# jacobstern/volume-viz

Measured on AMD Instinct MI355X. Metric: Msamples/s (rays x steps), 1024^3 f32 volume @1080p, higher is better.
Workload: dtype f32

## Files before the change

### include/volviz.h

```cpp
#ifndef VOLVIZ_H
#define VOLVIZ_H

#include <stddef.h>
#include <stdint.h>
#include <stdbool.h>

#ifdef __cplusplus
extern "C" {
#endif

#ifndef SLICE_NONE
#define SLICE_NONE      -1
#define SLICE_PLANE      0
#define SLICE_PLANE_CUT  1
#endif
#ifndef TRANSFER_PRESET_DEFAULT
#define TRANSFER_PRESET_DEFAULT -1
#define TRANSFER_PRESET_ENGINE   0
#define TRANSFER_PRESET_MRI      1
#endif

struct slice_params {
    int   type;
    float params[6];
// ... 120 lines not shown
int  vv_render_projection(vv_context *ctx, int width, int height,
                          const struct slice_params *slice,
                          const struct camera_params *camera,
                          const vv_ray_source *rays,
                          const vv_render_options *opts,
                          int mode,
                          uint8_t *rgba_out, uint8_t *index_out, uint32_t *stat_out, int out_on_device, void *stream);

int  vv_slice(vv_context *ctx, float *buffer, size_t height, size_t width,
              float dx, float dy, float dz, int orientation,
              const float scale[3], int legacy, int filter,
              int out_on_device, void *stream);
int  vv_slice_advanced(vv_context *ctx, float *buffer, size_t height, size_t width,
                       const float trans[16] ,
                       const float scale[3], int filter,
                       int out_on_device, void *stream);

typedef enum { VV_SLAB_MAX = 0, VV_SLAB_MIN = 1, VV_SLAB_MEAN = 2 } vv_slab_mode;
#define VV_SLAB_MAX_SAMPLES 1024
typedef struct vv_slab { int mode; int samples; float thickness; } vv_slab;
int  vv_slice_slab(vv_context *ctx, float *buffer, int32_t *aux , size_t height, size_t width,
                   float dx, float dy, float dz, int orientation, const float scale[3], int filter,
                   const vv_slab *slab, int out_on_device, void *stream);
int  vv_slice_advanced_slab(vv_context *ctx, float *buffer, int32_t *aux , size_t height, size_t width,
                            const float trans[16], const float scale[3], int filter,
                            const vv_slab *slab, int out_on_device, void *stream);

typedef struct vv_histogram {
    unsigned long long counts[256];
    unsigned long long voxels;
    unsigned long long nan_voxels;
    float vmin, vmax;
} vv_histogram;
int  vv_volume_histogram(vv_context *ctx, const int box_lo[3], const int box_hi[3],
                         vv_histogram *out, int out_on_device, void *stream);
int  vv_histogram_indices(vv_context *ctx, const uint8_t *index, size_t n,
                          unsigned long long counts[256], int on_device, void *stream);

int  vv_first_pass(vv_context *ctx, int img_w, int img_h, const struct camera_params *camera,
                   const vv_ray_source *rays, uint8_t *front_rgba, uint8_t *back_rgba,
                   int out_on_device, void *stream);

int  vv_cut_plane_canonical(int orientation, float displace, float point[3], float normal[3]);
int  vv_cut_plane_from_euler(float dx, float dy, float dz, float theta, float phi, float psi, float point[3], float normal[3]);
int  vv_cut_plane_to_slice_params(int slice_type, const float point[3], const float normal[3],
                                  int flip_cross_section, struct slice_params *out);

int  vv_camera_orbit_drag(const float position[3], int dx, int dy, float out_position[3], float out_look[3]);
int  vv_camera_zoom(const float position[3], const float look[3], int delta, float out_position[3]);
int  vv_cut_plane_from_drag(const float position[3], const float look[3], const float up[3], float aspect,
                            const float press[2], const float release[2],
                            float point[3], float normal[3], float plane_up[3], float plane_right[3]);
int  vv_cut_plane_drag(float point[3], const float plane_up[3], const float plane_right[3],
                       int dx, int dy, int width, int height);

int  vv_slice_to_bgra(const float *slice, size_t height, size_t width, uint8_t *bgra);

int  vv_slice_matrix(float dx, float dy, float dz, float theta, float phi, float psi,
                     float out[16]);

int  vv_generate_ellipsoids(vv_context *ctx, uint8_t *out, int out_on_device,
                            int nx, int ny, int nz, int n,
                            const float *centers , const float *axes ,
                            const uint8_t *colors , void *stream);
int  vv_draw_ellipsoid(vv_context *ctx, uint8_t *vol, int vol_on_device,
                       int nx, int ny, int nz, const float center[3], const float axes[3],
                       uint8_t color, void *stream);
int  vv_generate_default_brain(vv_context *ctx, uint8_t *out, int out_on_device,
                               int nx, int ny, int nz, void *stream);
int  vv_promote_u8_to_f32(vv_context *ctx, const uint8_t *dev_in, float *dev_out,
                          size_t n, void *stream);
int  vv_generate_noise_u8(vv_context *ctx, uint8_t *dev_out, int nx, int ny, int nz,
                          uint32_t seed, void *stream);

typedef enum { VV_TF_ENGINE = 0, VV_TF_HEAD = 1, VV_TF_MRI = 2 } vv_tf_preset;
int  vv_transfer_preset(int preset, float tf_out[1024]);

int  vv_dataset_preset(const char *path, int *tf_preset, float scale[3]);

int  vv_t3d_read_header(const char *path, int header, int *nx, int *ny, int *nz);
int  vv_t3d_read (const char *path, int header, uint8_t *dst, size_t capacity);
int  vv_t3d_write(const char *path, int header, const uint8_t *src, int nx, int ny, int nz);

enum { VV_LAYOUT_BRICKED = 1, VV_LAYOUT_ZPAIR = 2, VV_LAYOUT_ZFAST = 4, VV_LAYOUT_POLICY = 256 };
int  vv_prepare_layouts(vv_context *ctx, int which, void *stream);
int  vv_set_layout_policy(vv_context *ctx, unsigned long long budget_bytes , int build_in_render );
int  vv_layout_state(const vv_context *ctx, unsigned long long out[8]);
int  vv_device_bytes(const vv_context *ctx, unsigned long long out[4]);

float              vv_last_frame_ms(const vv_context *ctx);
int                vv_set_frame_timing(vv_context *ctx, int on);
unsigned long long vv_last_sample_count(vv_context *ctx);
int                vv_debug_last_launch(vv_context *ctx, int out[8]);
int                vv_debug_screen_rect(int width, int height, const struct camera_params *cam, const vv_ray_source *rays, double out[4]);
int                vv_debug_counters(vv_context *ctx, unsigned long long out[16]);
int                vv_reread_env(vv_context *ctx);
int                vv_volume_dims(const vv_context *ctx, int dims[3], int *voxel_type);

#ifdef __cplusplus
}
#endif
#endif
```

### volume-viz_amd/csrc/vv_api.cpp

```cpp
#include "../../include/volviz.h"
#include "vv_kernels.h"
#include "vv_gate.h"

#include <cassert>
#include <hip/hip_runtime.h>
#include <climits>
#include <cmath>
#include <cstdio>
#include <cstdlib>
#include <cstring>
#include <string>
#include <algorithm>
#include <vector>

using namespace vv;

struct vv_knobs {
    int tile_log2w = -1, xcd_band = -1, unroll = -1, lds_reserve = -1, lds_reserve_phong = -1;
    int bricked = -1, zpair = -1, zfast = -1, force_big = 0;
    int block_w = -1, tail = -1, rect = -1, lpt = -1, lpt_run = -1, phong_bricks = -1;
    int hist_blocks = -1;
    static int geti(const char *name, int dflt) { const char *e = getenv(name); return e ? atoi(e) : dflt; }
    void read()
    {
        tile_log2w = geti("VV_TILE_LOG2W", -1); xcd_band = geti("VV_XCD_BAND", -1); unroll = geti("VV_UNROLL", -1);
        lds_reserve = geti("VV_LDS_RESERVE", -1); lds_reserve_phong = geti("VV_LDS_RESERVE_PHONG", -1);
        bricked = geti("VV_BRICKED", -1); zpair = geti("VV_ZPAIR", -1);
        block_w = geti("VV_BLOCK_W", -1); tail = geti("VV_TAIL", -1);
        zfast = geti("VV_ZFAST", -1); force_big = getenv("VV_FORCE_BIG") != nullptr;
        rect = geti("VV_RECT", -1); lpt = geti("VV_LPT", -1); lpt_run = geti("VV_LPT_RUN", -1); phong_bricks = geti("VV_PHONG_BRICKS", -1);
        hist_blocks = geti("VV_HIST_BLOCKS", -1);
    }
};

enum { CP_BRICKS = 0, CP_ZPAIR = 1, CP_ZFAST = 2, CP_XPAIR = 3, CP_N = 4 };
struct layout_copy {
    void *ptr = nullptr; size_t bytes = 0;
    bool valid = false, failed = false;
    unsigned long long last_used = 0;
    uint32_t row = 0; uint64_t slab = 0;
};

struct vv_context {
    int device = 0;
    vv_knobs knobs;
    hipStream_t stream = nullptr;
    hipEvent_t ev0 = nullptr, ev1 = nullptr;
    hipEvent_t ev_count = nullptr;
    bool timed = false, time_frames = true;
    void *d_vol = nullptr; size_t vol_bytes = 0; int vtype = VV_VOXEL_U8; int nx = 0, ny = 0, nz = 0;
    size_t row_pitch = 0, slice_pitch = 0, alloc_bytes = 0;
    layout_copy copies[CP_N];
    size_t layout_budget_bytes = 0; bool build_in_render = true;
    unsigned long long frame_no = 0;
    unsigned long long builds_in_render = 0;
    float last_density = 1e9f;
    float4 *d_tf = nullptr; bool tf_gray = false; bool have_tf = false;
    bool tf_alpha_unit = false;
    float *d_rad = nullptr; size_t rad_cap = 0;
    uint32_t *d_order = nullptr; size_t order_cap = 0;
    uint8_t *d_frame = nullptr; size_t frame_cap = 0;
    uint8_t *d_index = nullptr; size_t index_cap = 0;
    uint8_t *d_hit = nullptr; size_t hit_cap = 0;
    uint8_t *d_stat = nullptr; size_t stat_cap = 0;
    float4 *d_tf_arg = nullptr;
    uint8_t *d_img = nullptr; size_t img_cap = 0;
    float *d_slice = nullptr; size_t slice_cap = 0;
    float *d_gen = nullptr; size_t gen_cap = 0;
    struct view_key_t { float cam[8]; const void *front, *back; int img_w, img_h, W, H; } view_key;
    bool view_key_valid = false, view_est_ok = false; float view_side[3] = {0, 0, 0}, view_px_cube = 0.f;
    std::vector<uint8_t> row_buf;
    int last_launch[8] = {0, 0, 0, 0, 0, 0, 0, 0};
    unsigned long long *d_counter = nullptr;
    unsigned long long *d_hist = nullptr;
    int n_cu = 0;
    bool counter_valid = false;
    hipStream_t copy_stream = nullptr, promo_stream = nullptr;
    void *pin[2] = {nullptr, nullptr}; hipEvent_t pin_ev[2] = {nullptr, nullptr}; int pin_next = 0;
    hipEvent_t src_ev[2] = {nullptr, nullptr}; int src_last = -1;
    uint8_t *d_stage[2] = {nullptr, nullptr};
    bool streaming = false;
    std::string err;
};

static std::string g_err;

static const size_t kHistResultOffset = kHistAccWords * sizeof(unsigned long long);
static const size_t kHistScratchBytes = kHistResultOffset + sizeof(vv_histogram);
static_assert(sizeof(vv_histogram) == 2072 && sizeof(unsigned long long) == 8, "vv_histogram layout (include/volviz.h)");

static int fail(vv_context *c, int code, const std::string &msg)
{
    if (c) c->err = msg; else g_err = msg;
    return code;
}
#define HIPCHK(c, expr) do { hipError_t e_ = (expr); if (e_ != hipSuccess) \
    return fail((c), VV_ERR_DEVICE, std::string(#expr) + ": " + hipGetErrorString(e_)); } while (0)

static inline hipStream_t pick_stream(const vv_context *c, void *stream)
{
    if (!stream) return c->stream;
    if (stream == VV_STREAM_DEFAULT_ASYNC) return (hipStream_t)0;
    return (hipStream_t)stream;
}

static void drop_copies(vv_context *c)
{
    for (layout_copy &cp : c->copies) {
        if (cp.ptr) (void)hipFree(cp.ptr);
        cp = layout_copy();
    }
    c->builds_in_render = 0;
    c->view_key_valid = false;
}

static int ensure(vv_context *c, void **p, size_t *cap, size_t need)
{
    if (*cap >= need && *p) return VV_OK;
    if (*p) { HIPCHK(c, hipFree(*p)); *p = nullptr; *cap = 0; }
    HIPCHK(c, hipMalloc(p, need));
    *cap = need;
    return VV_OK;
}

static int finalize_layout(vv_context *c, hipStream_t st);
static int camera_basis(vv_context *c, FrameParams &P, const camera_params *cam, const vv_ray_source *rays, int W, int H);
typedef vv_context::view_key_t vv_view_key;

static bool image_source_has_hint(const vv_ray_source *r)
{
    if (r->mode != VV_RAYS_IMAGES) return false;
    const float l2 = r->look[0] * r->look[0] + r->look[1] * r->look[1] + r->look[2] * r->look[2];
    const float cx = r->look[1] * r->up[2] - r->look[2] * r->up[1], cy = r->look[2] * r->up[0] - r->look[0] * r->up[2], cz = r->look[0] * r->up[1] - r->look[1] * r->up[0];
    return std::isfinite(l2) && l2 > 0.f && std::isfinite(cx + cy + cz) && (cx * cx + cy * cy + cz * cz) > 0.f;
}
static int clamp_row(long long t, int n) { return (int)(t < 0 ? 0 : (t > n - 1 ? n - 1 : t)); }
static vv_view_key view_key_of(const camera_params *cam, const vv_ray_source *r, int W, int H)
{
    vv_view_key k;
    memset(&k, 0, sizeof k);
    memcpy(k.cam, cam, sizeof(float) * 8);
    k.front = r->front; k.back = r->back; k.img_w = r->img_w; k.img_h = r->img_h; k.W = W; k.H = H;
    return k;
}
static bool estimate_view_from_images(const uint8_t *front, const uint8_t *back, int img_w, int img_h, int W, int H, float side[3], float *px_cube)
{
    if (!front || !back || img_w < 1 || img_h < 1 || W < 8 || H < 1) return false;
    const int y = H / 2;
    const int ty = clamp_row((long long)floorf((float)y / (float)H * (float)img_h), img_h);
    const uint8_t *fr = front + (size_t)ty * img_w * 4, *br = back + (size_t)ty * img_w * 4;
    auto texel = [&](int x) { return clamp_row((long long)floorf((float)x / (float)W * (float)img_w), img_w); };
    auto hit = [&](int x) { const int t = texel(x) * 4; return fr[t] != br[t] || fr[t + 1] != br[t + 1] || fr[t + 2] != br[t + 2]; };
    int xl = -1, xr = -1;
    for (int x = 0; x <= W - 2; ++x) if (hit(x)) { xl = x; break; }
    if (xl < 0) return false;
    for (int x = W - 2; x >= xl; --x) if (hit(x)) { xr = x; break; }
    if (xr - xl < 8) return false;
    const int a = (xl + xr) / 2 - (xr - xl) / 8, b = (xl + xr) / 2 + (xr - xl) / 8;
    float d[3], len2 = 0.f;
    for (int k = 0; k < 3; ++k) {
        const int ta = texel(a) * 4 + k, tb = texel(b) * 4 + k;
        d[k] = (((float)fr[tb] + (float)br[tb]) - ((float)fr[ta] + (float)br[ta])) / (2.f * 255.f);
        len2 += d[k] * d[k];
    }
    if (!(len2 > 0.f)) return false;
    const float len = sqrtf(len2);
    side[0] = d[0] / len; side[1] = d[1] / len; side[2] = d[2] / len;
    *px_cube = len / (float)(b - a);
    return true;
}

static size_t layout_budget(const vv_context *c)
{
    if (c->layout_budget_bytes) return c->layout_budget_bytes;
    return std::max<size_t>((size_t)8 << 30, c->alloc_bytes / 2 * 5);
}
static size_t copy_bytes(const vv_context *c, int k) { return c->copies[k].valid ? c->copies[k].bytes : 0; }
static void copy_drop(vv_context *c, int k)
{
    layout_copy &cp = c->copies[k];
    if (cp.ptr) (void)hipFree(cp.ptr);
    cp.ptr = nullptr; cp.valid = false; cp.bytes = 0;
}
static bool make_room(vv_context *c, size_t need, unsigned keep)
{
    const size_t budget = layout_budget(c);
    if (need > budget) return false;
    for (;;) {
        size_t used = 0;
        for (int k = 0; k < CP_N; ++k) used += copy_bytes(c, k);
        if (used + need <= budget) return true;
        int victim = -1;
        for (int k = 0; k < CP_N; ++k)
            if (c->copies[k].valid && !(keep & (1u << k)) && (victim < 0 || c->copies[k].last_used < c->copies[victim].last_used)) victim = k;
        if (victim < 0) return false;
        copy_drop(c, victim);
    }
}

static bool copy_refused(vv_context *c, int k)
{
    if (k != CP_ZPAIR) c->copies[k].failed = true;
    return false;
}

template <class Build>
static bool build_copy(vv_context *c, int k, size_t bytes, size_t pad, size_t zero_from, unsigned keep, hipStream_t st, Build build)
{
    layout_copy &cp = c->copies[k];
    size_t free_b = 0, total_b = 0;
    if (make_room(c, bytes, keep | (1u << k)) && hipMemGetInfo(&free_b, &total_b) == hipSuccess && free_b >= bytes + (512ull << 20) &&
        hipMalloc(&cp.ptr, bytes + pad) == hipSuccess) {
        if (hipMemsetAsync((char *)cp.ptr + zero_from, 0, bytes + pad - zero_from, st) == hipSuccess) {
            build(cp.ptr);
            if (hipGetLastError() == hipSuccess && hipStreamSynchronize(st) == hipSuccess) { cp.bytes = bytes; cp.valid = true; return true; }
        }
        (void)hipFree(cp.ptr);
    }
    (void)hipGetLastError();
    cp.ptr = nullptr;
    return copy_refused(c, k);
}

static bool ensure_bricks(vv_context *c, hipStream_t st)
{
    layout_copy &cp = c->copies[CP_BRICKS];
    if (cp.valid || cp.failed) return cp.valid;
    uint32_t sy = 0, sz64 = 0;
    const size_t bytes = brick_copy_bytes(c->vtype, c->nx, c->ny, c->nz, &sy, &sz64);
    if (sz64 >= (1u << 24) || sy >= (1u << 24)) return copy_refused(c, CP_BRICKS);
    cp.row = sy; cp.slab = sz64;
    return build_copy(c, CP_BRICKS, bytes, 16, bytes, 0, st, [&](void *p) {
        launch_build_bricks(c->vtype, c->d_vol, c->row_pitch, c->slice_pitch, p, c->nx, c->ny, c->nz, st); });
}

static bool ensure_zpair(vv_context *c, hipStream_t st)
{
    layout_copy &cp = c->copies[CP_ZPAIR];
    if (cp.valid) return true;
    uint32_t rb = 0, sb = 0;
    const size_t bytes = zpair_copy_bytes(c->vtype, c->nx, c->ny, c->nz, &rb, &sb);
    if ((size_t)(c->ny + 1) * ((size_t)c->nx + 1) * 8 >= (1ull << 32) || ((size_t)c->nx + 1) * 8 >= (1u << 24) ||
        (c->vtype == VV_VOXEL_U8 && bytes >= (1ull << 32)))
        return copy_refused(c, CP_ZPAIR);
    cp.row = rb; cp.slab = sb;
    return build_copy(c, CP_ZPAIR, bytes, 32, bytes, 0, st, [&](void *p) {
        launch_build_zpair(c->vtype, c->d_vol, c->row_pitch, c->slice_pitch, p, c->nx, c->ny, c->nz, st); });
}

static bool ensure_zfast(vv_context *c, hipStream_t st)
{
    layout_copy &cp = c->copies[CP_ZFAST];
    if (cp.valid || cp.failed) return cp.valid;
    const size_t vsz = c->vtype == VV_VOXEL_F32 ? 4 : 1;
    size_t row = (size_t)c->nz * vsz;
    if (row % 1024 == 0) row += 32;
    else if (vsz == 1) row = (row + 3) & ~(size_t)3;
    size_t rows = (size_t)c->ny;
    if (row % 1024 == 32 && (rows * row) % 4096 == 0) rows += 1;
    const size_t slice = rows * row, bytes = slice * ((size_t)c->nx + 1) + row + 16;
    if (c->ny > 65535 || (c->nz + 31) / 32 > 65535 || row >= (1u << 24) || slice >= (1ull << 32))
        return copy_refused(c, CP_ZFAST);
    cp.row = (uint32_t)row; cp.slab = slice;
    return build_copy(c, CP_ZFAST, bytes, 0, 0, 0, st, [&](void *p) {
        launch_build_zfast(c->vtype, c->d_vol, (uint32_t)c->row_pitch, (uint64_t)c->slice_pitch, p, (uint32_t)row, (uint64_t)slice, c->nx, c->ny, c->nz, st); });
}

static bool ensure_xpair(vv_context *c, hipStream_t st)
{
    layout_copy &cp = c->copies[CP_XPAIR];
    if (cp.valid || cp.failed) return cp.valid;
    if (!ensure_zfast(c, st)) return false;
    uint32_t rb = 0, sb = 0;
    const size_t bytes = zpair_copy_bytes(c->vtype, c->nz, c->ny, c->nx, &rb, &sb);
    if ((size_t)(c->ny + 1) * ((size_t)c->nz + 1) * 8 >= (1ull << 32) || ((size_t)c->nz + 1) * 8 >= (1u << 24) ||
        (c->vtype == VV_VOXEL_U8 && bytes >= (1ull << 32)))
        return copy_refused(c, CP_XPAIR);
    cp.row = rb; cp.slab = sb;
    const layout_copy &zf = c->copies[CP_ZFAST];
    return build_copy(c, CP_XPAIR, bytes, 32, bytes, 1u << CP_ZFAST, st, [&](void *p) {
        launch_build_xpair(c->vtype, zf.ptr, zf.row, zf.slab, p, c->nx, c->ny, c->nz, st); });
}

static bool (*const ensure_copy[CP_N])(vv_context *, hipStream_t) = {ensure_bricks, ensure_zpair, ensure_zfast, ensure_xpair};

static bool take_copy(vv_context *c, int k, hipStream_t st)
{
    if (!(c->build_in_render ? ensure_copy[k](c, st) : c->copies[k].valid)) return false;
    c->copies[k].last_used = c->frame_no;
    return true;
}

extern "C" {

const char *vv_last_error(const vv_context *ctx) { return ctx ? ctx->err.c_str() : g_err.c_str(); }

int vv_init(int device, vv_context **out)
{
    if (!out) return fail(nullptr, VV_ERR_INVALID, "vv_init: out_ctx is NULL");
    *out = nullptr;
    int count = 0;
    hipError_t e = hipGetDeviceCount(&count);
    if (e != hipSuccess || count == 0)
        return fail(nullptr, VV_ERR_DEVICE, "vv_init: no HIP device available (this library has no CPU path)");
    if (device < 0) { if (hipGetDevice(&device) != hipSuccess) device = 0; }
    if (device >= count) return fail(nullptr, VV_ERR_INVALID, "vv_init: device index out of range");
    vv_context *c = new vv_context();
    c->device = device;
    c->knobs.read();
    if (hipSetDevice(device) != hipSuccess || hipStreamCreate(&c->stream) != hipSuccess ||
        hipEventCreate(&c->ev0) != hipSuccess || hipEventCreate(&c->ev1) != hipSuccess || hipEventCreateWithFlags(&c->ev_count, hipEventDisableTiming) != hipSuccess ||
        hipMalloc((void **)&c->d_counter, 16 * sizeof(unsigned long long)) != hipSuccess ||
        hipMalloc((void **)&c->d_hist, kHistScratchBytes) != hipSuccess ||
        hipDeviceGetAttribute(&c->n_cu, hipDeviceAttributeMultiprocessorCount, device) != hipSuccess ||
        hipMalloc((void **)&c->d_tf, 256 * sizeof(float4)) != hipSuccess) {
        delete c;
        return fail(nullptr, VV_ERR_DEVICE, "vv_init: device set-up failed");
    }
    *out = c;
    return VV_OK;
}

int vv_shutdown(vv_context *c)
{
    if (!c) return VV_OK;
    hipSetDevice(c->device);
    hipStreamSynchronize(c->stream);
    if (c->d_vol) hipFree(c->d_vol);
    drop_copies(c);
    if (c->d_tf) hipFree(c->d_tf);
    if (c->d_rad) hipFree(c->d_rad);
    if (c->d_order) hipFree(c->d_order);
    if (c->d_frame) hipFree(c->d_frame);
    if (c->d_index) hipFree(c->d_index);
    if (c->d_hit) hipFree(c->d_hit);
    if (c->d_stat) hipFree(c->d_stat);
    if (c->d_tf_arg) hipFree(c->d_tf_arg);
    if (c->d_img) hipFree(c->d_img);
    if (c->d_slice) hipFree(c->d_slice);
    if (c->d_gen) hipFree(c->d_gen);
    if (c->d_counter) hipFree(c->d_counter);
    if (c->d_hist) hipFree(c->d_hist);
    for (int i = 0; i < 2; ++i) {
        if (c->pin[i]) hipHostFree(c->pin[i]);
        if (c->pin_ev[i]) hipEventDestroy(c->pin_ev[i]);
        if (c->src_ev[i]) hipEventDestroy(c->src_ev[i]);
        if (c->d_stage[i]) hipFree(c->d_stage[i]);
    }
    if (c->copy_stream) hipStreamDestroy(c->copy_stream);
    if (c->promo_stream) hipStreamDestroy(c->promo_stream);
    if (c->ev0) hipEventDestroy(c->ev0);
    if (c->ev1) hipEventDestroy(c->ev1);
    if (c->ev_count) hipEventDestroy(c->ev_count);
    if (c->stream) hipStreamDestroy(c->stream);
    delete c;
    return VV_OK;
}

int vv_set_transfer_function(vv_context *c, const float tf[1024])
{
    if (!c || !tf) return fail(c, VV_ERR_INVALID, "vv_set_transfer_function: NULL argument");
    HIPCHK(c, hipSetDevice(c->device));
    for (int i = 0; i < 1024; ++i)
        if (!std::isfinite(tf[i])) return fail(c, VV_ERR_INVALID, "vv_set_transfer_function: table entries must be finite");
    bool gray = true, unit = true;
    for (int i = 0; i < 256; ++i)
        if (!(tf[4*i] == tf[4*i+1] && tf[4*i] == tf[4*i+2])) { gray = false; break; }
    for (int i = 0; i < 256; ++i)
        if (!(tf[4*i+3] >= 0.f && tf[4*i+3] <= 1.f)) { unit = false; break; }
    HIPCHK(c, hipMemcpy(c->d_tf, tf, 1024 * sizeof(float), hipMemcpyHostToDevice));
    c->tf_gray = gray; c->tf_alpha_unit = unit; c->have_tf = true;
    return VV_OK;
}

static int install_volume(vv_context *c, const void *src, bool src_on_device, int vtype,
                          int nx, int ny, int nz, const float tf[1024], hipStream_t s)
{
    if (!c || !src) return fail(c, VV_ERR_INVALID, "load_volume: NULL argument");
    if (nx < 1 || ny < 1 || nz < 1) return fail(c, VV_ERR_INVALID, "load_volume: dims must be >= 1");
    if (vtype != VV_VOXEL_U8 && vtype != VV_VOXEL_F32) return fail(c, VV_ERR_INVALID, "load_volume: bad voxel type");
    const size_t vsz = vtype == VV_VOXEL_F32 ? 4 : 1;
    const size_t bytes = (size_t)nx * ny * nz * vsz;
    if ((size_t)nx * ny * vsz > 0xFFFFFFF0ull)
        return fail(c, VV_ERR_INVALID, "load_volume: one slice must stay below 4 GiB");
    if ((size_t)nx * vsz >= (1u << 24) || nx >= (1 << 24) || ny >= (1 << 24) || nz >= (1 << 24))
        return fail(c, VV_ERR_INVALID, "load_volume: a volume row must be below 16 MiB and each dimension below 2^24");
    HIPCHK(c, hipSetDevice(c->device));
    c->knobs.read();
    const size_t pad = (size_t)nx * ny * vsz + 2 * (size_t)nx * vsz + 4096;
    drop_copies(c);
    if (c->d_vol) { HIPCHK(c, hipFree(c->d_vol)); c->d_vol = nullptr; }
    HIPCHK(c, hipMalloc(&c->d_vol, bytes + pad));
    hipStream_t st = pick_stream(c, s);
    HIPCHK(c, hipMemsetAsync((char *)c->d_vol + bytes, 0, pad, st));
    if (src_on_device) HIPCHK(c, hipMemcpyAsync(c->d_vol, src, bytes, hipMemcpyDeviceToDevice, st));
    else { HIPCHK(c, hipMemcpyAsync(c->d_vol, src, bytes, hipMemcpyHostToDevice, st)); }
    c->vol_bytes = bytes; c->vtype = vtype; c->nx = nx; c->ny = ny; c->nz = nz;
    c->row_pitch = (size_t)nx * vsz; c->slice_pitch = c->row_pitch * ny; c->alloc_bytes = bytes + pad;
    { int rc = finalize_layout(c, st); if (rc) return rc; }
    if (!src_on_device || !s) HIPCHK(c, hipStreamSynchronize(st));
    if (tf) return vv_set_transfer_function(c, tf);
    return VV_OK;
}

int vv_load_volume_u8(vv_context *c, const uint8_t *texels, size_t size, int nx, int ny, int nz, const float tf[1024])
{
    if (size != (size_t)nx * ny * nz) return fail(c, VV_ERR_INVALID, "vv_load_volume_u8: size != nx*ny*nz");
    return install_volume(c, texels, false, VV_VOXEL_U8, nx, ny, nz, tf, nullptr);
}
int vv_load_volume_f32(vv_context *c, const float *texels, size_t size, int nx, int ny, int nz, const float tf[1024])
{
    if (size != (size_t)nx * ny * nz * 4) return fail(c, VV_ERR_INVALID, "vv_load_volume_f32: size != nx*ny*nz*4 bytes");
    return install_volume(c, texels, false, VV_VOXEL_F32, nx, ny, nz, tf, nullptr);
}
int vv_load_volume_device(vv_context *c, const void *dev, int vtype, int nx, int ny, int nz, const float tf[1024], void *stream)
{
    return install_volume(c, dev, true, vtype, nx, ny, nz, tf, (hipStream_t)stream);
}

int vv_prepare_layouts(vv_context *c, int which, void *stream)
{
    if (!c) return fail(nullptr, VV_ERR_INVALID, "vv_prepare_layouts: NULL context");
    if (!c->d_vol) return fail(c, VV_ERR_NO_VOLUME, "vv_prepare_layouts: no volume loaded");
    if (which & ~(VV_LAYOUT_BRICKED | VV_LAYOUT_ZPAIR | VV_LAYOUT_ZFAST | VV_LAYOUT_POLICY)) return fail(c, VV_ERR_INVALID, "vv_prepare_layouts: unknown layout bit");
    HIPCHK(c, hipSetDevice(c->device));
    hipStream_t st = pick_stream(c, stream);
    const bool pair_ok = c->vtype == VV_VOXEL_U8 || c->vol_bytes <= (512ull << 20);
    if (which & VV_LAYOUT_POLICY) {
        if ((size_t)c->nx * c->ny * c->nz >= (1ull << 21)) which |= VV_LAYOUT_BRICKED | VV_LAYOUT_ZFAST;
        if (pair_ok) which |= VV_LAYOUT_ZPAIR;
    }
    int built = 0;
    if (which & VV_LAYOUT_BRICKED) c->copies[CP_BRICKS].failed = false;
    if (which & VV_LAYOUT_ZFAST) c->copies[CP_ZFAST].failed = c->copies[CP_XPAIR].failed = false;
    auto prepare = [&](int k) {
        if (!ensure_copy[k](c, st)) return false;
        c->copies[k].last_used = ++c->frame_no;
        return true;
    };
    if ((which & VV_LAYOUT_BRICKED) && prepare(CP_BRICKS)) built |= VV_LAYOUT_BRICKED;
    if ((which & VV_LAYOUT_ZFAST) && prepare(CP_ZFAST)) {
        built |= VV_LAYOUT_ZFAST;
        if (pair_ok) prepare(CP_XPAIR);
    }
    if ((which & VV_LAYOUT_ZPAIR) && prepare(CP_ZPAIR)) built |= VV_LAYOUT_ZPAIR;
    return built;
}

int vv_reread_env(vv_context *c)
{
    if (!c) return VV_ERR_INVALID;
    c->knobs.read();
    return VV_OK;
}

int vv_set_layout_policy(vv_context *c, unsigned long long budget_bytes, int build_in_render)
{
    if (!c) return fail(nullptr, VV_ERR_INVALID, "vv_set_layout_policy: NULL context");
    c->layout_budget_bytes = (size_t)budget_bytes;
    c->build_in_render = build_in_render != 0;
    return VV_OK;
}

int vv_layout_state(const vv_context *c, unsigned long long out[8])
{
    if (!c || !out) return VV_ERR_INVALID;
    out[0] = c->d_vol ? c->alloc_bytes : 0;
    for (int k = 0; k < CP_N; ++k) out[1 + k] = copy_bytes(c, k);
    out[5] = c->d_vol ? layout_budget(c) : c->layout_budget_bytes;
    out[6] = c->builds_in_render;
    out[7] = c->build_in_render ? 1 : 0;
    return VV_OK;
}

int vv_device_bytes(const vv_context *c, unsigned long long out[4])
{
    if (!c || !out) return VV_ERR_INVALID;
    out[0] = c->d_vol ? c->alloc_bytes : 0;
    out[1] = copy_bytes(c, CP_BRICKS);
    out[2] = copy_bytes(c, CP_ZPAIR) + copy_bytes(c, CP_ZFAST) + copy_bytes(c, CP_XPAIR);
    out[3] = c->rad_cap + c->frame_cap + c->index_cap + c->hit_cap + c->stat_cap + (c->d_tf_arg ? 4096 : 0) + c->img_cap + c->slice_cap + 4096 + 8 * sizeof(unsigned long long) + kHistScratchBytes;
    return VV_OK;
}

int vv_debug_counters(vv_context *c, unsigned long long out[16])
{
    if (!c || !out || !c->counter_valid) return VV_ERR_INVALID;
    if (hipEventSynchronize(c->ev_count) != hipSuccess) return VV_ERR_DEVICE;
    if (hipMemcpy(out, c->d_counter, 16 * sizeof(unsigned long long), hipMemcpyDeviceToHost) != hipSuccess) return VV_ERR_DEVICE;
    return VV_OK;
}

static const size_t kStageBytes = 64u << 20;

int vv_load_volume_stream_begin(vv_context *c, int vtype, int nx, int ny, int nz, const float tf[1024])
{
    if (!c) return fail(nullptr, VV_ERR_INVALID, "stream_begin: NULL context");
    if (nx < 1 || ny < 1 || nz < 1 || (vtype != VV_VOXEL_U8 && vtype != VV_VOXEL_F32))
        return fail(c, VV_ERR_INVALID, "stream_begin: bad dims / voxel type");
    const size_t vsz = vtype == VV_VOXEL_F32 ? 4 : 1;
    if ((size_t)nx * ny * vsz > 0xFFFFFFF0ull) return fail(c, VV_ERR_INVALID, "stream_begin: one slice must stay below 4 GiB");
    if ((size_t)nx * vsz >= (1u << 24) || ny >= (1 << 24) || nz >= (1 << 24))
        return fail(c, VV_ERR_INVALID, "stream_begin: a volume row must be below 16 MiB and each dimension below 2^24");
    HIPCHK(c, hipSetDevice(c->device));
    c->knobs.read();
    const size_t bytes = (size_t)nx * ny * nz * vsz, pad = (size_t)nx * ny * vsz + 2 * (size_t)nx * vsz + 4096;
    drop_copies(c);
    if (c->d_vol) { HIPCHK(c, hipFree(c->d_vol)); c->d_vol = nullptr; }
    HIPCHK(c, hipMalloc(&c->d_vol, bytes + pad));
    if (!c->copy_stream) HIPCHK(c, hipStreamCreate(&c->copy_stream));
    if (!c->promo_stream) HIPCHK(c, hipStreamCreate(&c->promo_stream));
    HIPCHK(c, hipMemsetAsync((char *)c->d_vol + bytes, 0, pad, c->copy_stream));
    c->src_last = -1;
    c->vol_bytes = bytes; c->vtype = vtype; c->nx = nx; c->ny = ny; c->nz = nz;
    c->row_pitch = (size_t)nx * vsz; c->slice_pitch = c->row_pitch * ny; c->alloc_bytes = bytes + pad;
    c->streaming = true;
    if (tf) return vv_set_transfer_function(c, tf);
    return VV_OK;
}

int vv_load_volume_stream_slices_async(vv_context *c, const void *src, int src_type, int z0, int nslices)
{
    if (!c || !c->streaming) return fail(c, VV_ERR_INVALID, "stream_slices: no stream_begin");
    if (!src || z0 < 0 || nslices < 1 || z0 + nslices > c->nz) return fail(c, VV_ERR_INVALID, "stream_slices: bad slice range");
    if (src_type != c->vtype && !(src_type == VV_VOXEL_U8 && c->vtype == VV_VOXEL_F32))
        return fail(c, VV_ERR_INVALID, "stream_slices: source type must match the volume (or be u8 for an f32 volume)");
    HIPCHK(c, hipSetDevice(c->device));
    const size_t ssz = src_type == VV_VOXEL_F32 ? 4 : 1, dsz = c->vtype == VV_VOXEL_F32 ? 4 : 1;
    const size_t slice_vox = (size_t)c->nx * c->ny;
    const bool promote = src_type != c->vtype;
    hipPointerAttribute_t attr;
    bool pinned = hipPointerGetAttributes(&attr, src) == hipSuccess && attr.type == hipMemoryTypeHost;
    (void)hipGetLastError();
    size_t total_vox = slice_vox * (size_t)nslices, done = 0;
    const size_t piece_vox_max = ((kStageBytes / ssz) / 16) * 16;
    while (done < total_vox) {
        const size_t nv = std::min(piece_vox_max, total_vox - done);
        const int b = c->pin_next; c->pin_next ^= 1;
        if (!c->pin_ev[b]) HIPCHK(c, hipEventCreate(&c->pin_ev[b]));
        if (!c->src_ev[b]) HIPCHK(c, hipEventCreate(&c->src_ev[b]));
        HIPCHK(c, hipEventSynchronize(c->pin_ev[b]));
        const char *hsrc = (const char *)src + done * ssz;
        if (!pinned) {
            if (!c->pin[b]) HIPCHK(c, hipHostMalloc(&c->pin[b], kStageBytes, hipHostMallocDefault));
            memcpy(c->pin[b], hsrc, nv * ssz);
            hsrc = (const char *)c->pin[b];
        }
        char *dst = (char *)c->d_vol + ((size_t)z0 * slice_vox + done) * dsz;
        if (!promote) {
            HIPCHK(c, hipMemcpyAsync(dst, hsrc, nv * ssz, hipMemcpyHostToDevice, c->copy_stream));
            HIPCHK(c, hipEventRecord(c->src_ev[b], c->copy_stream));
            HIPCHK(c, hipEventRecord(c->pin_ev[b], c->copy_stream));
        } else {
            if (!c->d_stage[b]) HIPCHK(c, hipMalloc((void **)&c->d_stage[b], kStageBytes));
// ... 73 lines not shown
        return rc ? rc : r3;
    }
    return VV_OK;
}

int vv_volume_dims(const vv_context *c, int dims[3], int *vtype)
{
    if (!c || !c->d_vol) return VV_ERR_NO_VOLUME;
    if (dims) { dims[0] = c->nx; dims[1] = c->ny; dims[2] = c->nz; }
    if (vtype) *vtype = c->vtype;
    return VV_OK;
}

static int finalize_layout(vv_context *c, hipStream_t st)
{
    size_t pad_bytes = 32;
    if (const char *e = getenv("VV_PITCH_PAD")) { int t = atoi(e); if (t <= 0) return VV_OK; if (t >= 16 && t <= 4096 && t % 16 == 0) pad_bytes = (size_t)t; }
    const size_t dense_row = c->row_pitch;
    if (dense_row % 1024 != 0 && !getenv("VV_PITCH_FORCE")) return VV_OK;
    if (dense_row % 16 != 0) return VV_OK;
    const size_t row = dense_row + pad_bytes;
    size_t rows = (size_t)c->ny;
    if ((rows * row) % 4096 == 0) rows += 1;
    if (const char *e = getenv("VV_PITCH_ROWS")) { int t = atoi(e); if (t >= 0 && t <= 64) rows = (size_t)c->ny + (size_t)t; }
    const size_t slice = rows * row;
    if (slice > 0xFFFFFFF0ull || row >= (1u << 24)) return VV_OK;
    const size_t bytes = slice * (size_t)c->nz, pad = slice + 2 * row + 4096;
    size_t free_b = 0, total_b = 0;
    void *nv = nullptr;
    if (hipMemGetInfo(&free_b, &total_b) != hipSuccess || free_b < bytes + pad + (512ull << 20) ||
        hipMalloc(&nv, bytes + pad) != hipSuccess) { (void)hipGetLastError(); return VV_OK; }
    HIPCHK(c, hipMemsetAsync(nv, 0, bytes + pad, st));
    launch_repitch(c->d_vol, nv, dense_row, (size_t)c->ny, (size_t)c->nz, row, slice, st);
    HIPCHK(c, hipGetLastError());
    HIPCHK(c, hipStreamSynchronize(st));
    HIPCHK(c, hipFree(c->d_vol));
    c->d_vol = nv; c->row_pitch = row; c->slice_pitch = slice; c->alloc_bytes = bytes + pad;
    return VV_OK;
}

static VolumeView view_of(const vv_context *c, MarchBuild b)
{
    VolumeView V = {};
    V.data = c->d_vol; V.nx = c->nx; V.ny = c->ny; V.nz = c->nz;
    V.row_bytes = (uint32_t)c->row_pitch;
    V.slice_bytes = (uint32_t)c->slice_pitch;
    V.big = c->slice_pitch * (size_t)c->nz > (1ull << 32) || V.slice_bytes >= (1u << 24) || c->knobs.force_big;
    const layout_copy *cp = c->copies;
    if (b == MB_BRICKED || b == MB_BRICKED_CACHED) { V.bricks = cp[CP_BRICKS].ptr; V.b_sy = cp[CP_BRICKS].row; V.b_sz64 = (uint32_t)cp[CP_BRICKS].slab; }
    if (b == MB_ZFAST || b == MB_XPAIR) { V.zfast = cp[CP_ZFAST].ptr; V.zf_row_bytes = cp[CP_ZFAST].row; V.zf_slice_bytes = cp[CP_ZFAST].slab; }
    const layout_copy &pc = cp[b == MB_XPAIR ? CP_XPAIR : CP_ZPAIR];
    if (b == MB_ZPAIR || b == MB_XPAIR) { V.zpair = pc.ptr; V.zp_row_bytes = pc.row; V.zp_slab_bytes = (uint32_t)pc.slab; }
    return V;
}

static inline float vlen_h(float x, float y, float z) { return sqrtf(x * x + y * y + z * z); }

static int camera_basis(vv_context *c, FrameParams &P, const camera_params *cam, const vv_ray_source *rays, int W, int H)
{
    float lx = rays->look[0], ly = rays->look[1], lz = rays->look[2];
    float ll = vlen_h(lx, ly, lz);
    if (!(ll > 0.f)) return fail(c, VV_ERR_INVALID, "vv_render: look vector is zero");
    lx /= ll; ly /= ll; lz /= ll;
    float ux = rays->up[0], uy = rays->up[1], uz = rays->up[2];
    float sx = ly * uz - lz * uy, sy = lz * ux - lx * uz, sz = lx * uy - ly * ux;
    float sl = vlen_h(sx, sy, sz);
    if (!(sl > 0.f)) return fail(c, VV_ERR_INVALID, "vv_render: up vector is parallel to look");
    sx /= sl; sy /= sl; sz /= sl;
    float vx = sy * lz - sz * ly, vy = sz * lx - sx * lz, vz = sx * ly - sy * lx;
    float vl = vlen_h(vx, vy, vz);
    vx /= vl; vy /= vl; vz /= vl;
    P.look[0] = lx; P.look[1] = ly; P.look[2] = lz;
    P.side[0] = sx; P.side[1] = sy; P.side[2] = sz;
    P.up[0] = vx; P.up[1] = vy; P.up[2] = vz;
    float aspect = rays->aspect > 0.f ? rays->aspect : (float)W / (float)H;
    float th = (float)tan((double)cam->fovY * M_PI / 360.0);
    P.tan_half_x = th * aspect; P.tan_half_y = th;
    return VV_OK;
}


}

static bool choose_launch(vv_context *c, MarchArgs &A, const camera_params *cam, const vv_ray_source *rays, const shading_params *shading,
                          bool have_basis, float density, int H, hipStream_t st)
{
    FrameParams &P = A.P;
    A.V_type = c->vtype;
    A.strips.tile_log2w = 3;
    if (have_basis) {
        const float ax = fabsf(P.side[0]) , ay = fabsf(P.side[1]), az = fabsf(P.side[2]);
        if (ax >= 0.97f * sqrtf(ax * ax + ay * ay + az * az)) A.strips.tile_log2w = 5;
    }
    const vv_knobs &K = c->knobs;
    if ((rays->mode == VV_RAYS_ANALYTIC || image_source_has_hint(rays)) && have_basis && H > 0) {
        const float dist = vlen_h(cam->origin[0], cam->origin[1], cam->origin[2]);
        const float vpw = cbrtf(((float)c->nx / (2.f * P.scale[0])) * ((float)c->ny / (2.f * P.scale[1])) * ((float)c->nz / (2.f * P.scale[2])));
        const float px_vox = 2.f * P.tan_half_y * dist / (float)H * vpw;
        const float step_vox = fmaxf(P.step[0] * c->nx, fmaxf(P.step[1] * c->ny, P.step[2] * c->nz));
        if (std::isfinite(px_vox) && std::isfinite(step_vox) && px_vox > 0.f && step_vox > 0.f) density = step_vox * px_vox * px_vox;
    }
    bool use_zfast = false;
    if (have_basis && A.strips.tile_log2w == 3) {
        const float ax = fabsf(P.side[0]) , ay = fabsf(P.side[1]), az = fabsf(P.side[2]);
        use_zfast = az >= 0.97f * sqrtf(ax * ax + ay * ay + az * az) && (size_t)c->nx * c->ny * c->nz >= (1ull << 21);
        if (K.zfast >= 0) use_zfast = K.zfast != 0;
    }
    const bool phong_bricks_fit = K.phong_bricks > 0 || (density > 3.5f && density <= 8.f && c->vol_bytes > (2ull << 30) && c->vol_bytes <= (8ull << 30));
    const bool phong_bricks = phong_bricks_fit && shading->phongShading && c->vol_bytes > (1ull << 30) && c->vtype == VV_VOXEL_F32 && K.bricked != 0 && K.phong_bricks != 0 &&
                              (c->copies[CP_BRICKS].valid || (c->build_in_render && !c->copies[CP_BRICKS].failed));
    if (phong_bricks && K.zfast < 0) use_zfast = false;
    ++c->frame_no;
    auto copies_valid = [c] { int n = 0; for (const layout_copy &cp : c->copies) n += cp.valid; return n; };
    const int valid_before = copies_valid();
    if (use_zfast) use_zfast = take_copy(c, CP_ZFAST, st);
    if (use_zfast) A.strips.tile_log2w = 5;
    if (K.tile_log2w >= 3 && K.tile_log2w <= 5 && !use_zfast) A.strips.tile_log2w = K.tile_log2w;
    A.strips.xcd_band = 1;
    if (K.xcd_band >= 0 && K.xcd_band <= 64) A.strips.xcd_band = K.xcd_band;
    const bool beyond_caches = c->vol_bytes > (1ull << 30);
    const int big_reserve = density > 3.5f ? 76000 : (density > 1.8f ? 49000 : 36000);
    A.unroll = (A.strips.tile_log2w == 5 || beyond_caches) ? 3 : 2;
    A.lds_reserve = !beyond_caches ? 36000 : (A.strips.tile_log2w == 5 ? big_reserve : 155000);
    A.strips.blk_log2w = 5;
    A.strips.tail_batch = K.tail == 0 ? 0 : 1;
    const int rows_px_8 = A.strips.n_strips * 8;
    int block_w = A.strips.tile_log2w == 3 ? 16 : ((A.strips.tile_log2w == 5 && c->vol_bytes >= (1ull << 30) && density > 3.5f) ? 64 : 32);
    if (K.block_w >= 8 && K.block_w <= 128 && (K.block_w & (K.block_w - 1)) == 0) block_w = K.block_w;
    {
        int lw = 3; while ((1 << lw) < block_w) ++lw;
        const int h = 256 >> lw;
        if (lw != 5 && lw >= A.strips.tile_log2w && h >= (64 >> A.strips.tile_log2w)) {
            A.strips.blk_log2w = lw;
            if (A.strips.strips_per_band < (1 << 26)) {
                const int band_px = A.strips.strips_per_band * 8, spb = (band_px + h - 1) / h;
                A.strips.n_strips = (rows_px_8 / band_px) * spb; A.strips.strips_per_band = spb;
            } else A.strips.n_strips = (rows_px_8 + h - 1) / h;
        }
    }
    const bool k_unroll = K.unroll >= 1 && K.unroll <= 3, k_reserve = K.lds_reserve >= 0 && K.lds_reserve <= 155 * 1024;
    if (k_unroll) A.unroll = K.unroll;
    if (k_reserve) A.lds_reserve = K.lds_reserve;
    bool use_bricks = (A.strips.tile_log2w == 3 || phong_bricks) && (size_t)c->nx * c->ny * c->nz >= (1ull << 21);
    if (K.bricked >= 0) use_bricks = K.bricked != 0;
    if (use_zfast) use_bricks = false;
    if (use_bricks) use_bricks = take_copy(c, CP_BRICKS, st);
    if (use_bricks) {
        if (!k_unroll) A.unroll = 2;
        if (!k_reserve) A.lds_reserve = beyond_caches ? big_reserve : 36000;
    }
    bool use_zpair = !use_bricks && A.strips.tile_log2w == 5 && !shading->phongShading &&
                     (c->vtype == VV_VOXEL_U8 || c->vol_bytes <= (512ull << 20));
    if (K.zpair >= 0) use_zpair = K.zpair != 0 && !use_bricks;
    if (use_zfast) use_zpair = false;
    if (use_zpair) use_zpair = take_copy(c, CP_ZPAIR, st);
    const bool use_xpair = use_zfast && !shading->phongShading && K.zpair != 0 && (c->vtype == VV_VOXEL_U8 || c->vol_bytes <= (512ull << 20)) &&
                           take_copy(c, CP_XPAIR, st);
    const int valid_after = copies_valid();
    if (valid_after > valid_before) c->builds_in_render += valid_after - valid_before;
    A.build = use_xpair ? MB_XPAIR : use_zfast ? MB_ZFAST : use_bricks ? (beyond_caches ? MB_BRICKED : MB_BRICKED_CACHED) : use_zpair ? MB_ZPAIR :
              (view_of(c, MB_LINEAR).big || (shading->phongShading && beyond_caches)) ? MB_LINEAR_BIG : MB_LINEAR;
    A.V = view_of(c, A.build);
    A.lds_reserve_phong = c->vol_bytes > (8ull << 30) ? 40000 : ((beyond_caches && density > 3.5f && !use_bricks) ? 30000 : 13000);
    if (K.lds_reserve_phong >= 0 && K.lds_reserve_phong <= 146 * 1024) A.lds_reserve_phong = K.lds_reserve_phong;
    c->last_density = density;
    return beyond_caches;
}

static bool screen_rect(const MarchArgs &A, int W, int H, double *xmin, double *xmax, double *ymin, double *ymax)
{
    const FrameParams &P = A.P;
    double lo[2] = {INFINITY, INFINITY}, hi[2] = {-INFINITY, -INFINITY}, dmin = INFINITY, ext = 0.0;
    for (int a = 0; a < 3; ++a) ext = std::max(ext, (double)fabsf(P.cam_pos[a]) + (double)P.scale[a]);
    for (int k = 0; k < 8; ++k) {
        const double v[3] = {((k & 1) ? P.scale[0] : -P.scale[0]) - (double)P.cam_pos[0], ((k & 2) ? P.scale[1] : -P.scale[1]) - (double)P.cam_pos[1],
                             ((k & 4) ? P.scale[2] : -P.scale[2]) - (double)P.cam_pos[2]};
        const double depth = v[0] * P.look[0] + v[1] * P.look[1] + v[2] * P.look[2];
        if (!(depth > 1e-3 * ext)) return false;
        dmin = std::min(dmin, depth);
        const double sx = (v[0] * P.side[0] + v[1] * P.side[1] + v[2] * P.side[2]) / depth, sy = (v[0] * P.up[0] + v[1] * P.up[1] + v[2] * P.up[2]) / depth;
        const double px = (sx / P.tan_half_x + 1.0) * 0.5 * W - 0.5, py = (sy / P.tan_half_y + 1.0) * 0.5 * H - 0.5;
        lo[0] = std::min(lo[0], px); hi[0] = std::max(hi[0], px); lo[1] = std::min(lo[1], py); hi[1] = std::max(hi[1], py);
    }
    const double ang = 1e-4 * ext / dmin;
    const double mx = 1.0 + ang / (2.0 * P.tan_half_x / W), my = 1.0 + ang / (2.0 * P.tan_half_y / H);
    if (!std::isfinite(lo[0] + hi[0] + lo[1] + hi[1] + mx + my) || mx > W || my > H) return false;
    *xmin = lo[0] - mx; *xmax = hi[0] + mx; *ymin = lo[1] - my; *ymax = hi[1] + my;
    return true;
}

static void launch_build(FrameKind kind, const MarchArgs &A, hipStream_t st) { assert(A.build < MB_COUNT); kLaunch[frame_row(kind)][A.build](A, st); }

struct FrameImage {
    void *host;
    size_t px_bytes;
    uint8_t **scratch; size_t *cap;
    unsigned align;
    const char *misaligned;
    uint8_t *dev;
};

struct Frame {
    MarchArgs A;
    FrameKind kind; int W, H; hipStream_t st;
    bool have_basis; float density;
    bool beyond_caches;
    bool rect_limits; PixelRect fill_rect;
    bool whole;
    FrameImage img[4];
};

static int check_frame_args(vv_context *c, int W, int H, const slice_params *slice, const camera_params *cam, const vv_ray_source *rays)
{
    if (W < 1 || H < 1) return fail(c, VV_ERR_INVALID, "vv_render: width/height must be >= 1");
    if (!c->d_vol || !c->have_tf) return fail(c, VV_ERR_NO_VOLUME, "vv_render: no volume / transfer function loaded");
    if (slice->type != SLICE_NONE && slice->type != SLICE_PLANE && slice->type != SLICE_PLANE_CUT)
        return fail(c, VV_ERR_INVALID, "vv_render: slice type must be SLICE_NONE/PLANE/PLANE_CUT");
    if (rays->mode == VV_RAYS_IMAGES && (!rays->front || !rays->back || rays->img_w < 1 || rays->img_h < 1))
        return fail(c, VV_ERR_INVALID, "vv_render: image ray source needs front/back images");
    if (rays->mode != VV_RAYS_IMAGES && rays->mode != VV_RAYS_ANALYTIC)
        return fail(c, VV_ERR_INVALID, "vv_render: bad ray source mode");
    for (int a = 0; a < 3; ++a)
        if (!(cam->scale[a] > 0.f) || !std::isfinite(cam->scale[a]))
            return fail(c, VV_ERR_INVALID, "vv_render: camera scale must be finite and > 0");
    return VV_OK;
}

static int frame_params(vv_context *c, Frame &F, const slice_params *slice, const camera_params *cam, const vv_ray_source *rays, const vv_render_options *opts)
{
    MarchArgs &A = F.A;
    FrameParams &P = A.P;
    const int W = F.W, H = F.H;
    const bool reducer = F.kind != FRAME_COMPOSITE;
    P.W = W; P.H = H;
    P.nbx = W / kSlab + ((W % kSlab) ? 1 : 0);
    P.nby = H / kSlab + ((H % kSlab) ? 1 : 0);
    P.conflict_x = (W >= 2 && W - 1 == (P.nbx - 1) * kSlab);
    P.conflict_y = (H >= 2 && H - 1 == (P.nby - 1) * kSlab);
    int rb = 0, re = P.nby;
    int s_count = 1, s_index = 0, s_band = 4;
    P.step[0] = 1.f / (float)c->nx; P.step[1] = 1.f / (float)c->ny; P.step[2] = 1.f / (float)c->nz;
    P.ert_thr = .95f; P.ert_true = 0; P.alpha_unit = c->tf_alpha_unit;
    A.tex8 = true; A.instr = false;
    if (opts) {
        if (opts->step[0] > 0.f || opts->step[1] > 0.f || opts->step[2] > 0.f) {
// ... 164 lines not shown
}

static int tile_order(vv_context *c, Frame &F, const vv_ray_source *rays)
{
    MarchArgs &A = F.A;
    const int W = F.W, H = F.H;
    const bool beyond_caches = F.beyond_caches;
    A.strips.order = nullptr; A.order_out = nullptr;
    const int wr = A.strips.wr, ns = A.strips.s1 - A.strips.s0;
    A.strips.order_run = wr > 0 ? (wr + (wr + 15) / 16 - 1) / ((wr + 15) / 16) : 1;
    if (c->knobs.lpt_run > 0 && c->knobs.lpt_run <= 256) A.strips.order_run = c->knobs.lpt_run;
    const int units = wr > 0 ? order_units(A.strips) : 0;
    const bool want = c->knobs.lpt > 0 ? true : (A.strips.tile_log2w == 5 && !beyond_caches && (long long)wr * ns >= 1024);
    if (c->knobs.lpt != 0 && want && !A.phong && rays->mode == VV_RAYS_ANALYTIC && W >= 2 && H >= 2 && units >= 8 && units <= 1024 && (long long)(wr + 1) * (ns + 1) <= 24576) {
        const int rc = ensure(c, (void **)&c->d_order, &c->order_cap, std::max((size_t)order_words(A.strips), (size_t)65536) * sizeof(uint32_t));
        if (rc) return rc;
        A.strips.order = c->d_order; A.order_out = c->d_order;
    } else A.strips.order_run = 1;
    return VV_OK;
}

static int stage_images(vv_context *c, Frame &F, int out_on_device)
{
    const size_t npx = (size_t)F.W * F.H;
    for (FrameImage &im : F.img) {
        im.dev = (uint8_t *)im.host;
        if (out_on_device || !im.host) continue;
        int rc = ensure(c, (void **)im.scratch, im.cap, npx * im.px_bytes);
        if (rc) return rc;
        im.dev = *im.scratch;
        if (!F.whole) HIPCHK(c, hipMemcpyAsync(im.dev, im.host, npx * im.px_bytes, hipMemcpyHostToDevice, F.st));
    }
    for (const FrameImage &im : F.img)
        if (((uintptr_t)im.dev & (im.align - 1)) != 0) return fail(c, VV_ERR_INVALID, im.misaligned);
    return VV_OK;
}

static void launch_kernels(Frame &F)
{
    MarchArgs &A = F.A;
    hipStream_t st = F.st;
    if (A.phong) {
        if (A.fill_outside) { A.rad_out = nullptr; launch_rad(A, st); }
        launch_build(F.kind, A, st);
    } else if (A.strips.n_strips > 0) {
        if (F.W >= 2 && F.H >= 2) launch_rad(A, st);
        if (F.kind != FRAME_COMPOSITE && F.rect_limits) launch_fill(A, F.fill_rect, st);
        launch_build(F.kind, A, st);
    }
}

static int read_back(vv_context *c, const Frame &F, int out_on_device, void *stream)
{
    const size_t W = (size_t)F.W, H = (size_t)F.H;
    if (!out_on_device) {
        for (const FrameImage &im : F.img) {
            if (!im.host) continue;
            const size_t pitch = W * im.px_bytes;
            if (F.whole) HIPCHK(c, hipMemcpy2DAsync(im.host, pitch, im.dev, pitch, (W - 1) * im.px_bytes, H - 1, hipMemcpyDeviceToHost, F.st));
            else HIPCHK(c, hipMemcpyAsync(im.host, im.dev, pitch * H, hipMemcpyDeviceToHost, F.st));
        }
        HIPCHK(c, hipStreamSynchronize(F.st));
    } else if (!stream) {
        HIPCHK(c, hipStreamSynchronize(F.st));
    }
    return VV_OK;
}

static int render_frame(vv_context *c, int W, int H, const slice_params *slice, const camera_params *cam,
                        const shading_params *shading, const vv_ray_source *rays, const vv_render_options *opts,
                        uint8_t *rgba_out, uint8_t *index_out, float *hit_out, uint32_t *stat_out, FrameKind kind, int level, int out_on_device, void *stream)
{
    int rc = check_frame_args(c, W, H, slice, cam, rays);
    if (rc) return rc;
    HIPCHK(c, hipSetDevice(c->device));
    Frame F;
    memset(&F, 0, sizeof F);
    F.kind = kind; F.W = W; F.H = H; F.st = pick_stream(c, stream);
    MarchArgs &A = F.A;
    const FrameParams &P = A.P;
    hipStream_t st = F.st;
    if ((rc = frame_params(c, F, slice, cam, rays, opts)) != VV_OK) return rc;
    if ((rc = view_knowledge(c, F, cam, rays, stream)) != VV_OK) return rc;
    F.beyond_caches = choose_launch(c, A, cam, rays, shading, F.have_basis, F.density, H, st);
    F.density = c->last_density;
    A.gray = c->tf_gray; A.phong = shading->phongShading;
    tiles_under_rect(c, F, rays);
    A.tf = c->d_tf; A.fill_tf = kind == FRAME_ISO ? nullptr : A.tf;
    if ((rc = ensure(c, (void **)&c->d_rad, &c->rad_cap, (size_t)P.nbx * P.nby * sizeof(float))) != VV_OK) return rc;
    if ((rc = tile_order(c, F, rays)) != VV_OK) return rc;
    A.rad = c->d_rad; A.rad_out = c->d_rad;
    A.counter = c->d_counter;

    F.whole = P.count <= 1 && P.rb == 0 && P.re == P.nby && W >= 2 && H >= 2;
    const FrameImage images[4] = {
        {rgba_out,  4,  &c->d_frame, &c->frame_cap, 4,  "vv_render: output buffer must be 4-byte aligned", nullptr},
        {index_out, 1,  &c->d_index, &c->index_cap, 1,  "", nullptr},
        {hit_out,   16, &c->d_hit,   &c->hit_cap,   16, "vv_render_iso: a device hit_out must be 16-byte aligned", nullptr},
        {stat_out,  8,  &c->d_stat,  &c->stat_cap,  8,  "vv_render_projection: a device stat_out must be 8-byte aligned", nullptr},
    };
    memcpy(F.img, images, sizeof images);
    if ((rc = stage_images(c, F, out_on_device)) != VV_OK) return rc;
    A.pixels = (uint32_t *)F.img[0].dev; A.index = F.img[1].dev; A.hit = (float4 *)F.img[2].dev; A.stat = (uint2 *)F.img[3].dev;
    A.proj_mode = kind == FRAME_PROJ ? level : 0;
    if (kind == FRAME_ISO) {
        A.iso.level = level;
        const int dims[3] = {c->nx, c->ny, c->nz};
        for (int a = 0; a < 3; ++a) { A.iso.n[a] = (float)dims[a]; A.iso.h[a] = 1.0f / (float)dims[a]; }
    }

    if (A.instr) HIPCHK(c, hipMemsetAsync(c->d_counter, 0, 16 * sizeof(unsigned long long), st));
#ifdef VV_TIMELINE
    { const char *e = getenv("VV_TIMELINE_PTR"); A.I.timeline = e ? (unsigned long long *)strtoull(e, nullptr, 0) : nullptr; }
#endif
    c->counter_valid = A.instr;
    {
        static const int layout_code[] = {0, 1, 2, 2, 3, 4, 5};
        const int v[8] = {A.strips.tile_log2w, A.strips.blk_log2w, A.unroll, A.phong ? A.lds_reserve_phong : A.lds_reserve, layout_code[A.build],
                          F.have_basis ? 1 : 0, (int)fminf(F.density * 1000.f, 2e9f), kind != FRAME_COMPOSITE ? (int)kind : (A.phong ? 1 : 0)};
        memcpy(c->last_launch, v, sizeof v);
    }
    if (c->time_frames) HIPCHK(c, hipEventRecord(c->ev0, st));
    launch_kernels(F);
    if (c->time_frames) HIPCHK(c, hipEventRecord(c->ev1, st));
    if (A.instr) HIPCHK(c, hipEventRecord(c->ev_count, st));
    HIPCHK(c, hipGetLastError());
    c->timed = c->time_frames;
    return read_back(c, F, out_on_device, stream);
}

static shading_params unshaded()
{
    shading_params s;
    memset(&s, 0, sizeof s);
    s.transferPreset = -1; s.phongShading = false;
    return s;
}

extern "C" {

int vv_render(vv_context *c, int W, int H, const slice_params *slice, const camera_params *cam,
              const shading_params *shading, const vv_ray_source *rays, const vv_render_options *opts,
              uint8_t *rgba_out, int out_on_device, void *stream)
{
    if (!c) return fail(nullptr, VV_ERR_INVALID, "vv_render: NULL context");
    if (!slice || !cam || !shading || !rays || !rgba_out) return fail(c, VV_ERR_INVALID, "vv_render: NULL argument");
    return render_frame(c, W, H, slice, cam, shading, rays, opts, rgba_out, nullptr, nullptr, nullptr, FRAME_COMPOSITE, 0, out_on_device, stream);
}

int vv_render_mip(vv_context *c, int W, int H, const slice_params *slice, const camera_params *cam,
                  const vv_ray_source *rays, const vv_render_options *opts,
                  uint8_t *rgba_out, uint8_t *index_out, int out_on_device, void *stream)
{
    if (!c) return fail(nullptr, VV_ERR_INVALID, "vv_render_mip: NULL context");
    if (!slice || !cam || !rays) return fail(c, VV_ERR_INVALID, "vv_render_mip: NULL argument");
    if (!rgba_out && !index_out) return fail(c, VV_ERR_INVALID, "vv_render_mip: rgba_out and index_out are both NULL");
    const shading_params none = unshaded();
    return render_frame(c, W, H, slice, cam, &none, rays, opts, rgba_out, index_out, nullptr, nullptr, FRAME_MIP, 0, out_on_device, stream);
}

int vv_render_iso(vv_context *c, int W, int H, const slice_params *slice, const camera_params *cam,
                  const vv_ray_source *rays, const vv_render_options *opts, int level,
                  uint8_t *rgba_out, uint8_t *index_out, float *hit_out, int out_on_device, void *stream)
{
    if (!c) return fail(nullptr, VV_ERR_INVALID, "vv_render_iso: NULL context");
    if (!slice || !cam || !rays) return fail(c, VV_ERR_INVALID, "vv_render_iso: NULL argument");
    if (!rgba_out && !index_out && !hit_out) return fail(c, VV_ERR_INVALID, "vv_render_iso: rgba_out, index_out and hit_out are all NULL");
// ... 418 lines not shown
```

### volume-viz_amd/csrc/vv_aux.hip

```cpp
#include <atomic>
#include "vv_device.h"
#include "vv_kernels.h"
#include <cstdlib>

namespace vv {

__device__ __forceinline__ void vv_wave_lds_order()
{
    __builtin_amdgcn_fence(__ATOMIC_RELEASE, "wavefront");
    __builtin_amdgcn_wave_barrier();
    __builtin_amdgcn_fence(__ATOMIC_ACQUIRE, "wavefront");
}


template <int VOXEL, bool TEX8>
__global__ __launch_bounds__(256) void slice_kernel(SliceArgs A)
{
#pragma clang fp contract(off)
    const size_t i = threadIdx.x + (size_t)blockIdx.x * 16;
    const size_t j = threadIdx.y + (size_t)blockIdx.y * 16;
    if (!(j < A.height && i < A.width)) return;
    const size_t offset = j * A.height + i;
    if (offset >= A.height * A.width) return;
    if (i >= A.height && j + 1 < A.height) return;
// ... 531 lines not shown
void launch_promote_u8_f32(const uint8_t *in, float *out, size_t n, hipStream_t s)
{
    size_t blocks = (n / 4 + 255) / 256;
    if (blocks > 256 * 32) blocks = 256 * 32;
    if (blocks == 0) blocks = 1;
    hipLaunchKernelGGL(promote_kernel, dim3((unsigned)blocks), dim3(256), 0, s, in, out, n);
}

size_t brick_copy_bytes(int vtype, int nx, int ny, int nz, uint32_t *sy, uint32_t *sz64)
{
    const size_t brick = vtype == VV_VOXEL_F32 ? BrickGeom<VV_VOXEL_F32>::brick : BrickGeom<VV_VOXEL_U8>::brick;
    const size_t bxv = vtype == VV_VOXEL_F32 ? BrickGeom<VV_VOXEL_F32>::bx : BrickGeom<VV_VOXEL_U8>::bx;
    const bool xcol = vtype == VV_VOXEL_F32 && BrickGeom<VV_VOXEL_F32>::halo == 0;
    const size_t bzv = vtype == VV_VOXEL_F32 ? BrickGeom<VV_VOXEL_F32>::bz : BrickGeom<VV_VOXEL_U8>::bz;
    const size_t nbx = xcol ? (size_t)nx / bxv + 1 : ((size_t)nx + bxv - 1) / bxv, nby = (size_t)ny / 4 + 1, nbz = (size_t)nz / bzv + 1;
    size_t row = nbx * brick;
    size_t pad = (vtype == VV_VOXEL_F32 && row % 4096 == 0) ? (BrickGeom<VV_VOXEL_F32>::brick % 128 == 0 ? 128 : 64) : 0;
    if (const char *e = getenv("VV_BRICK_PAD")) { int t = atoi(e); if (t >= 0 && t <= 4096 && t % 64 == 0) pad = (size_t)t; }
    if (nx >= (1 << 20)) { if (sy) *sy = 0xFFFFFFFFu; if (sz64) *sz64 = 0xFFFFFFFFu; return ~(size_t)0 >> 1; }
    row += pad;
    const size_t layer = nby * row;
    if (sy) *sy = (uint32_t)row;
    if (sz64) *sz64 = (uint32_t)(layer >> 6);
    return nbz * layer;
}

template <typename T, int E, int BX, int BZ, int BRICK_ELEMS>
__global__ __launch_bounds__(256) void brick_kernel(const T *__restrict__ in, size_t row_pitch, size_t slice_pitch, T *__restrict__ out,
                                                    int nx, int ny, int nz, size_t nbx, size_t nby, size_t total,
                                                    size_t brow , size_t blayer )
{
    for (size_t t = blockIdx.x * (size_t)blockDim.x + threadIdx.x; t < total; t += (size_t)gridDim.x * blockDim.x) {
        constexpr int R = 4 * BZ;
        const int e = (int)(t % E), r = (int)((t / E) % R);
        const size_t b = t / (E * R);
        const size_t bx = b % nbx, by = (b / nbx) % nby, bz = b / (nbx * nby);
        const int x = min((int)bx * BX + e, nx - 1), y = min((int)by * 4 + (r & 3), ny - 1), z = min((int)bz * BZ + (r >> 2), nz - 1);
        out[bz * blayer + by * brow + bx * (size_t)BRICK_ELEMS + (size_t)(r * E + e)] =
            e <= BX ? ((const T *)((const char *)in + (size_t)z * slice_pitch + (size_t)y * row_pitch))[x] : T(0);
    }
}

void launch_build_bricks(int vtype, const void *linear, size_t row_pitch, size_t slice_pitch, void *bricks, int nx, int ny, int nz, hipStream_t s)
{
    constexpr int FBX = BrickGeom<VV_VOXEL_F32>::bx;
    const size_t bxv = vtype == VV_VOXEL_F32 ? FBX : 4;
    constexpr int FH = BrickGeom<VV_VOXEL_F32>::halo;
    const bool xcol = vtype == VV_VOXEL_F32 && FH == 0;
    constexpr int FBZ = BrickGeom<VV_VOXEL_F32>::bz;
    const size_t bzv = vtype == VV_VOXEL_F32 ? FBZ : 4;
    const size_t nbx = xcol ? (size_t)nx / bxv + 1 : ((size_t)nx + bxv - 1) / bxv, nby = (size_t)ny / 4 + 1, nbz = (size_t)nz / bzv + 1;
    const size_t per_brick = vtype == VV_VOXEL_F32 ? 4 * FBZ * (FBX + FH) : 128;
    const size_t total = nbx * nby * nbz * per_brick;
    uint32_t sy = 0, sz64 = 0;
    brick_copy_bytes(vtype, nx, ny, nz, &sy, &sz64);
    const size_t esz = vtype == VV_VOXEL_F32 ? 4 : 1, brow = sy / esz, blayer = ((size_t)sz64 << 6) / esz;
    size_t blocks = (total + 255) / 256;
    if (blocks > 256 * 64) blocks = 256 * 64;
    if (vtype == VV_VOXEL_F32)
        hipLaunchKernelGGL((brick_kernel<float, FBX + FH, FBX, FBZ, BrickGeom<VV_VOXEL_F32>::brick / 4>), dim3((unsigned)blocks), dim3(256), 0, s, (const float *)linear, row_pitch, slice_pitch, (float *)bricks, nx, ny, nz, nbx, nby, total, brow, blayer);
    else
        hipLaunchKernelGGL((brick_kernel<uint8_t, 8, 4, 4, 128>), dim3((unsigned)blocks), dim3(256), 0, s, (const uint8_t *)linear, row_pitch, slice_pitch, (uint8_t *)bricks, nx, ny, nz, nbx, nby, total, brow, blayer);
}

__global__ __launch_bounds__(256) void repitch_kernel(const uint4 *__restrict__ in, char *__restrict__ out, size_t row16, size_t ny,
                                                      size_t row_pitch, size_t slice_pitch, size_t total)
{
    for (size_t t = blockIdx.x * (size_t)blockDim.x + threadIdx.x; t < total; t += (size_t)gridDim.x * blockDim.x) {
        const size_t x = t % row16, r = t / row16, y = r % ny, z = r / ny;
        *(uint4 *)(out + z * slice_pitch + y * row_pitch + x * 16) = in[t];
    }
}

void launch_repitch(const void *dense, void *pitched, size_t row_bytes, size_t ny, size_t nz,
                    size_t row_pitch, size_t slice_pitch, hipStream_t s)
{
    const size_t row16 = row_bytes / 16, total = row16 * ny * nz;
    size_t blocks = (total + 255) / 256;
    if (blocks > 256 * 64) blocks = 256 * 64;
    if (blocks == 0) return;
    hipLaunchKernelGGL(repitch_kernel, dim3((unsigned)blocks), dim3(256), 0, s, (const uint4 *)dense, (char *)pitched, row16, ny, row_pitch, slice_pitch, total);
}

size_t zpair_copy_bytes(int vtype, int nx, int ny, int nz, uint32_t *row_bytes, uint32_t *slab_bytes)
{
    const size_t rec = vtype == VV_VOXEL_F32 ? 8 : 2;
    size_t row = (((size_t)nx + 1) * rec + 3) & ~(size_t)3;
    if (const char *e = getenv("VV_ZPAIR_PAD")) { int t = atoi(e); if (t > 0 && t <= 4096 && t % 8 == 0) row += (size_t)t; }
    const size_t slab = ((size_t)ny + 1) * row;
    if (row_bytes) *row_bytes = (uint32_t)row;
    if (slab_bytes) *slab_bytes = (uint32_t)slab;
    return slab * (size_t)nz;
}

template <typename T, typename T2>
__global__ __launch_bounds__(256) void zpair_kernel(const T *__restrict__ in, size_t row_pitch, size_t slice_pitch, T2 *__restrict__ out,
                                                    int nx, int ny, int nz, size_t row_recs, size_t total)
{
    const size_t ry = (size_t)ny + 1;
    for (size_t t = blockIdx.x * (size_t)blockDim.x + threadIdx.x; t < total; t += (size_t)gridDim.x * blockDim.x) {
        const int x = min((int)(t % row_recs), nx - 1);
        const size_t row = t / row_recs;
        const int y = min((int)(row % ry), ny - 1), z = (int)(row / ry);
        const char *rowp = (const char *)in + (size_t)y * row_pitch;
        T2 r;
        r.x = ((const T *)(rowp + (size_t)z * slice_pitch))[x];
        r.y = ((const T *)(rowp + (size_t)min(z + 1, nz - 1) * slice_pitch))[x];
        out[t] = r;
    }
}

void launch_build_zpair(int vtype, const void *linear, size_t row_pitch, size_t slice_pitch, void *zpair, int nx, int ny, int nz, hipStream_t s)
{
    uint32_t rb = 0, sb = 0;
    zpair_copy_bytes(vtype, nx, ny, nz, &rb, &sb);
    const size_t row_recs = rb / (vtype == VV_VOXEL_F32 ? 8 : 2);
    const size_t total = row_recs * ((size_t)ny + 1) * (size_t)nz;
    size_t blocks = (total + 255) / 256;
    if (blocks > 256 * 64) blocks = 256 * 64;
    if (vtype == VV_VOXEL_F32)
        hipLaunchKernelGGL((zpair_kernel<float, float2>), dim3((unsigned)blocks), dim3(256), 0, s, (const float *)linear, row_pitch, slice_pitch, (float2 *)zpair, nx, ny, nz, row_recs, total);
    else
        hipLaunchKernelGGL((zpair_kernel<uint8_t, uchar2>), dim3((unsigned)blocks), dim3(256), 0, s, (const uint8_t *)linear, row_pitch, slice_pitch, (uchar2 *)zpair, nx, ny, nz, row_recs, total);
}

template <typename T>
__global__ __launch_bounds__(256) void zfast_kernel(const T *__restrict__ in, uint32_t row_pitch, uint64_t slice_pitch, T *__restrict__ out,
                                                    uint32_t zf_row_bytes, uint64_t zf_slice_bytes, int nx, int ny, int nz)
{
    __shared__ T tile[32][33];
    const int tx = threadIdx.x & 31, ty = threadIdx.x >> 5;
    const int x0 = blockIdx.x * 32, z0 = blockIdx.y * 32, y = blockIdx.z;
    for (int r = ty; r < 32; r += 8) {
        const int z = z0 + r, x = x0 + tx;
        tile[r][tx] = (z < nz && x < nx) ? ((const T *)((const char *)in + (uint64_t)z * slice_pitch + (uint64_t)y * row_pitch))[x] : T(0);
    }
    __syncthreads();
    for (int r = ty; r < 32; r += 8) {
        const int x = x0 + r, z = z0 + tx;
        if (x < nx && z < nz) ((T *)((char *)out + (uint64_t)x * zf_slice_bytes + (uint64_t)y * zf_row_bytes))[z] = tile[tx][r];
    }
}

void launch_build_zfast(int vtype, const void *vol, uint32_t row_pitch, uint64_t slice_pitch, void *out, uint32_t zf_row_bytes, uint64_t zf_slice_bytes, int nx, int ny, int nz, hipStream_t s)
{
    if (ny > 65535 || (nz + 31) / 32 > 65535) return;
    const dim3 grid((unsigned)((nx + 31) / 32), (unsigned)((nz + 31) / 32), (unsigned)ny);
    if (vtype == VV_VOXEL_F32)
        hipLaunchKernelGGL(zfast_kernel<float>, grid, dim3(256), 0, s, (const float *)vol, row_pitch, slice_pitch, (float *)out, zf_row_bytes, zf_slice_bytes, nx, ny, nz);
    else
        hipLaunchKernelGGL(zfast_kernel<uint8_t>, grid, dim3(256), 0, s, (const uint8_t *)vol, row_pitch, slice_pitch, (uint8_t *)out, zf_row_bytes, zf_slice_bytes, nx, ny, nz);
}

template <typename T, typename T2>
__global__ __launch_bounds__(256) void xpair_kernel(const T *__restrict__ zf, uint32_t zf_row_bytes, uint64_t zf_slice_bytes, T2 *__restrict__ out,
                                                    int nx, int ny, int nz, size_t row_recs, size_t total)
{
    const size_t ry = (size_t)ny + 1;
    for (size_t t = blockIdx.x * (size_t)blockDim.x + threadIdx.x; t < total; t += (size_t)gridDim.x * blockDim.x) {
        const int z = min((int)(t % row_recs), nz - 1);
        const size_t row = t / row_recs;
        const int y = min((int)(row % ry), ny - 1), x = (int)(row / ry);
        const char *rowp = (const char *)zf + (size_t)y * zf_row_bytes;
        T2 r;
        r.x = ((const T *)(rowp + (size_t)x * zf_slice_bytes))[z];
        r.y = ((const T *)(rowp + (size_t)min(x + 1, nx - 1) * zf_slice_bytes))[z];
// ... 52 lines not shown
```

### volume-viz_amd/csrc/vv_device.h

```cpp
#pragma once
#include <hip/hip_runtime.h>
#include <stdint.h>
#include "../../include/volviz.h"

namespace vv {

constexpr int   kCacheDepth = 32;
constexpr float kChunkSteps = 30.f;
constexpr int   kSlab = 14;
constexpr int   kBlock = 16;
constexpr float kSqrt3 = 1.73205081f;
constexpr float kEps = 1e-6f;

struct f3 { float x, y, z; };
__device__ __forceinline__ f3 mk3(float x, float y, float z) { return f3{x, y, z}; }

struct VolumeView {
    const void *data;
    int nx, ny, nz;
    uint32_t row_bytes;
    uint32_t slice_bytes;
    int big;
    const void *bricks;
    uint32_t b_sy;
    uint32_t b_sz64;
    const void *zpair;
    uint32_t zp_row_bytes;
    uint32_t zp_slab_bytes;
    const void *zfast;
    uint32_t zf_row_bytes;
    uint64_t zf_slice_bytes;
};
template <int VOXEL> struct BrickGeom;
#ifndef VV_BRICK_XLOG2
#define VV_BRICK_XLOG2 2
#endif
#ifndef VV_BRICK_HALO
#define VV_BRICK_HALO 1
#endif
#ifndef VV_BRICK_ZLOG2
#define VV_BRICK_ZLOG2 2
#endif
#ifndef VV_BRICK_X7
#define VV_BRICK_X7 0
#endif
#ifndef VV_BRICK_EXTRA
#define VV_BRICK_EXTRA 0
#endif
#if VV_BRICK_X7
template <> struct BrickGeom<VV_VOXEL_F32> { static constexpr uint32_t xlog2 = 0, bx = 7, halo = 1, row = 32,
                                             zlog2 = VV_BRICK_ZLOG2, bz = 1u << zlog2, rows = 4 * bz, brick = rows * row + VV_BRICK_EXTRA; };
#else
template <> struct BrickGeom<VV_VOXEL_F32> { static constexpr uint32_t xlog2 = VV_BRICK_XLOG2, bx = 1u << xlog2, halo = VV_BRICK_HALO, row = (bx + halo) * 4,
                                             zlog2 = VV_BRICK_ZLOG2, bz = 1u << zlog2, rows = 4 * bz, brick = rows * row; };
#endif
template <int VOXEL>
__device__ __forceinline__ uint32_t brick_x_offset(uint32_t ix)
{
    using G = BrickGeom<VOXEL>;
    if constexpr (VOXEL == VV_VOXEL_F32 && G::bx == 7) {
        const uint32_t q = (uint32_t)((float)ix * 0.142857149f);
        return __umul24(q, G::brick - 28u) + (ix << 2);
    } else if constexpr (VOXEL == VV_VOXEL_F32) {
        return __umul24(ix >> G::xlog2, G::brick) + ((ix & (G::bx - 1u)) << 2);
    } else {
        return (ix >> 2) * G::brick;
    }
}
template <> struct BrickGeom<VV_VOXEL_U8>  { static constexpr uint32_t xlog2 = 2, bx = 4, halo = 1, row = 8, zlog2 = 2, bz = 4, rows = 16, brick = 128; };
enum { LAYOUT_LINEAR = 0, LAYOUT_LINEAR_BIG = 1, LAYOUT_BRICKED = 2, LAYOUT_ZPAIR = 3, LAYOUT_ZFAST = 4 };

struct FrameParams {
    int W, H;
    int nbx, nby;
    int conflict_x, conflict_y;
    int rb, re, band, count, index;
    int slice_type;
    float slice_point[3], slice_normal[3];
    float cam_pos[3], scale[3], inv_scale[3];
    float step[3];
    float tan_fov_x, tan_fov_y;
    float ert_thr;
    int   ert_true;
    int   alpha_unit;
    int   max_chunks;
    int   safe_div;
    int ray_mode, quantize8;
    const uint8_t *front_img, *back_img; int img_w, img_h;
    float side[3], up[3], look[3];
    float tan_half_x, tan_half_y;
};

__device__ __forceinline__ int wave_min_i(int v) { for (int o = 32; o > 0; o >>= 1) v = min(v, __shfl_xor(v, o)); return v; }
__device__ __forceinline__ int wave_max_i(int v) { for (int o = 32; o > 0; o >>= 1) v = max(v, __shfl_xor(v, o)); return v; }

#pragma clang fp contract(off)
__device__ __forceinline__ float vlen3(float x, float y, float z)
{
#pragma clang fp contract(off)
    return sqrtf(x * x + y * y + z * z);
}
__device__ __forceinline__ float dot3s(f3 a, f3 b)
{
#pragma clang fp contract(off)
    return a.x * b.x + a.y * b.y + a.z * b.z;
}

__device__ __forceinline__ void ray_endpoints(const FrameParams &P, int x, int y, f3 &front, f3 &back)
{
#pragma clang fp contract(off)
    if (P.ray_mode == VV_RAYS_IMAGES) {
        float u = (float)x / (float)P.W, v = (float)y / (float)P.H;
        int tx = (int)floorf(u * (float)P.img_w), ty = (int)floorf(v * (float)P.img_h);
        tx = max(0, min(tx, P.img_w - 1)); ty = max(0, min(ty, P.img_h - 1));
        const size_t t = (size_t)ty * P.img_w + tx;
        const uint32_t f = ((const uint32_t *)P.front_img)[t], b = ((const uint32_t *)P.back_img)[t];
        front = mk3((float)(f & 255u) / 255.f, (float)((f >> 8) & 255u) / 255.f, (float)((f >> 16) & 255u) / 255.f);
        back  = mk3((float)(b & 255u) / 255.f, (float)((b >> 8) & 255u) / 255.f, (float)((b >> 16) & 255u) / 255.f);
        return;
    }
    float ndx = (2.0f * ((float)x + 0.5f)) / (float)P.W - 1.0f;
    float ndy = (2.0f * ((float)y + 0.5f)) / (float)P.H - 1.0f;
    float sx = ndx * P.tan_half_x, sy = ndy * P.tan_half_y;
    float d[3], o[3] = {P.cam_pos[0], P.cam_pos[1], P.cam_pos[2]};
    for (int a = 0; a < 3; a++) d[a] = (P.side[a] * sx + P.up[a] * sy) + P.look[a];
    float tmin = -INFINITY, tmax = INFINITY;
    bool miss = false;
    for (int a = 0; a < 3; a++) {
        float s = P.scale[a];
        if (d[a] != 0.0f) {
            float t1 = (-s - o[a]) / d[a], t2 = (s - o[a]) / d[a];
            tmin = fmaxf(tmin, fminf(t1, t2)); tmax = fminf(tmax, fmaxf(t1, t2));
        } else if (o[a] < -s || o[a] > s) miss = true;
    }
    front = mk3(0.f, 0.f, 0.f); back = mk3(0.f, 0.f, 0.f);
    if (miss || !(tmin <= tmax) || !(tmax > 0.0f)) return;
    back = mk3((o[0] + d[0] * tmax) * 0.5f + 0.5f, (o[1] + d[1] * tmax) * 0.5f + 0.5f,
               (o[2] + d[2] * tmax) * 0.5f + 0.5f);
    if (tmin > 0.0f)
        front = mk3((o[0] + d[0] * tmin) * 0.5f + 0.5f, (o[1] + d[1] * tmin) * 0.5f + 0.5f,
                    (o[2] + d[2] * tmin) * 0.5f + 0.5f);
    if (P.quantize8) {
        float *p[6] = {&front.x, &front.y, &front.z, &back.x, &back.y, &back.z};
        for (int i = 0; i < 6; i++) {
            float c = fmaxf(0.f, fminf(*p[i], 1.f));
            *p[i] = floorf(c * 255.0f + 0.5f) / 255.f;
        }
    }
}

__device__ __host__ __forceinline__ int slab_lo(int b) { int v = b * kSlab - 1; return v < 0 ? 0 : v; }
__device__ __host__ __forceinline__ int slab_up(int b, int n) { int v = (b + 1) * kSlab + 1; return v > n - 1 ? n - 1 : v; }
// ... 20 lines not shown
    f3 cam = mk3(P.cam_pos[0], P.cam_pos[1], P.cam_pos[2]);
    float dx = back.x - front.x, dy = back.y - front.y, dz = back.z - front.z;
    float length = vlen3(dx, dy, dz);
    f3 ray = mk3(dx / length, dy / length, dz / length);
    f3 pos = front;
    {
        f3 l = mk3(ray.x * -1.f, ray.y * -1.f, ray.z * -1.f);
        f3 l0p0 = mk3(front.x - cam.x, front.y - cam.y, front.z - cam.z);
        float b = dot3s(l, l0p0);
        float c = dot3s(l0p0, l0p0) - rad * rad;
        float disc = b * b - c;
        if (disc >= 0.f) {
            float t = b * -1.f - sqrtf(disc);
            if (t >= -kEps) pos = mk3(pos.x - ray.x * t, pos.y - ray.y * t, pos.z - ray.z * t);
        }
    }
    float upper = fminf(kSqrt3, vlen3(back.x - pos.x, back.y - pos.y, back.z - pos.z));
    r.origin = pos; r.dir = ray;
    r.sdir = mk3(ray.x * P.step[0], ray.y * P.step[1], ray.z * P.step[2]);
    r.sstep = vlen3(r.sdir.x, r.sdir.y, r.sdir.z);
    r.dist0 = 0.f; r.cut_return = false;
    if (P.slice_type == SLICE_PLANE_CUT) {
        f3 p0 = mk3(P.slice_point[0], P.slice_point[1], P.slice_point[2]);
        f3 n  = mk3(P.slice_normal[0], P.slice_normal[1], P.slice_normal[2]);
        f3 bk = mk3(pos.x + ray.x * upper, pos.y + ray.y * upper, pos.z + ray.z * upper);
        float sf = dot3s(n, mk3(pos.x - p0.x, pos.y - p0.y, pos.z - p0.z));
        float sb = dot3s(n, mk3(bk.x - p0.x, bk.y - p0.y, bk.z - p0.z));
        if (sf <= kEps && sb <= kEps) {
            r.cut_return = true;
        } else {
            float denom = dot3s(n, ray);
            bool hit = false;
            if (denom > kEps) {
                float t = dot3s(mk3(p0.x - pos.x, p0.y - pos.y, p0.z - pos.z), n) / denom;
                if (t >= 0.f) { r.dist0 = t; hit = true; }
            }
            if (!hit) {
                f3 nr = mk3(ray.x * -1.f, ray.y * -1.f, ray.z * -1.f);
                float den2 = dot3s(n, nr);
                if (den2 > kEps) {
                    float t = dot3s(mk3(p0.x - bk.x, p0.y - bk.y, p0.z - bk.z), n) / den2;
                    if (t >= 0.f) upper -= t;
                }
            }
        }
    }
    r.upper = upper;
}

__device__ __forceinline__ int chunk_count(float dist, float upper, float sstep)
{
#pragma clang fp contract(off)
    if (!(dist < upper)) return 0;
    float est = (upper - dist) / sstep;
    int n = est >= 30.f ? 30 : (est > 0.f ? (int)est : 0);
    while (n < 30 && !((float)(n + 1) * sstep + dist > upper)) ++n;
    while (n > 0 && ((float)n * sstep + dist > upper)) --n;
    if (sstep != sstep) n = 30;
    return n;
}
#pragma clang fp contract(fast)

typedef float  __attribute__((ext_vector_type(2), aligned(4))) float2u;
typedef unsigned short __attribute__((aligned(1))) ushort_u;

template <bool TEX8>
__device__ __forceinline__ float axis_coord(float x, float n, float nm1, uint32_t &i)
{
    float xb = __builtin_fmaf(x, n, -0.5f);
    xb = __builtin_amdgcn_fmed3f(xb, 0.0f, nm1);
    i = (uint32_t)xb;
    float a = __builtin_amdgcn_fractf(xb);
    if (TEX8) {
        const float magic = 49152.0f;
        float t = a + magic;
        a = t - magic;
    }
    return a;
}

template <int VOXEL> struct Corners;
template <> struct Corners<VV_VOXEL_F32> { float2u a, b, c, d; float wx, wy, wz; };
template <> struct Corners<VV_VOXEL_U8>  { uint32_t a0, a1, b0, b1, c0, c1, d0, d1, sh; float wx, wy, wz; };

template <int VOXEL>
__device__ __forceinline__ void load_rows(const char *b00, uint32_t row_bytes, uint32_t slice_bytes, uint32_t ix,
                                          uint32_t yz, Corners<VOXEL> &C)
{
    const char *b10 = b00 + row_bytes;
    const char *b01 = b00 + slice_bytes;
    const char *b11 = b01 + row_bytes;
    if constexpr (VOXEL == VV_VOXEL_F32) {
        const uint32_t off = ix * 4u + yz;
        C.a = *(const float2u *)(b00 + off); C.b = *(const float2u *)(b10 + off);
        C.c = *(const float2u *)(b01 + off); C.d = *(const float2u *)(b11 + off);
    } else {
        const uint32_t off = (ix & ~3u) + yz;
        C.sh = ix & 3u;
        C.a0 = *(const uint32_t *)(b00 + off); C.a1 = *(const uint32_t *)(b00 + off + 4);
        C.b0 = *(const uint32_t *)(b10 + off); C.b1 = *(const uint32_t *)(b10 + off + 4);
        C.c0 = *(const uint32_t *)(b01 + off); C.c1 = *(const uint32_t *)(b01 + off + 4);
        C.d0 = *(const uint32_t *)(b11 + off); C.d1 = *(const uint32_t *)(b11 + off + 4);
    }
}

template <int VOXEL, bool TEX8, int LAYOUT = LAYOUT_LINEAR>
__device__ __forceinline__ void fetch_corners(const VolumeView &V, float px, float py, float pz, Corners<VOXEL> &C)
{
    uint32_t ix, iy, iz;
    C.wx = axis_coord<TEX8>(px, (float)V.nx, (float)(V.nx - 1), ix);
    C.wy = axis_coord<TEX8>(py, (float)V.ny, (float)(V.ny - 1), iy);
    C.wz = axis_coord<TEX8>(pz, (float)V.nz, (float)(V.nz - 1), iz);
    if constexpr (LAYOUT == LAYOUT_LINEAR) {
        load_rows<VOXEL>((const char *)V.data, V.row_bytes, V.slice_bytes, ix,
                         __umul24(iy, V.row_bytes) + __umul24(iz, V.slice_bytes), C);
    } else if constexpr (LAYOUT == LAYOUT_LINEAR_BIG) {
        const uint32_t vsz = VOXEL == VV_VOXEL_F32 ? 4u : 1u;
        const char *zb = (const char *)V.data + (uint64_t)iz * V.slice_bytes + (__umul24(iy, V.row_bytes) + ix * vsz);
        if constexpr (VOXEL == VV_VOXEL_F32) load_rows<VOXEL>(zb, V.row_bytes, V.slice_bytes, 0u, 0u, C);
        else {
            const char *zr = (const char *)V.data + (uint64_t)iz * V.slice_bytes;
            load_rows<VOXEL>(zr, V.row_bytes, V.slice_bytes, ix, __umul24(iy, V.row_bytes), C);
        }
    } else if constexpr (LAYOUT == LAYOUT_ZFAST) {
        const char *xb = (const char *)V.zfast + (uint64_t)ix * V.zf_slice_bytes;
        if constexpr (VOXEL == VV_VOXEL_F32) {
            Corners<VOXEL> T;
            load_rows<VOXEL>(xb + (__umul24(iy, V.zf_row_bytes) + iz * 4u), V.zf_row_bytes, (uint32_t)V.zf_slice_bytes, 0u, 0u, T);
            C.a.x = T.a.x; C.a.y = T.c.x; C.b.x = T.b.x; C.b.y = T.d.x;
            C.c.x = T.a.y; C.c.y = T.c.y; C.d.x = T.b.y; C.d.y = T.d.y;
        } else {
            load_rows<VOXEL>(xb, V.zf_row_bytes, (uint32_t)V.zf_slice_bytes, iz, __umul24(iy, V.zf_row_bytes), C);
        }
    } else {
        using G = BrickGeom<VOXEL>;
        const uint32_t ya = iy & 3u, za = iz & (G::bz - 1u);
        const uint32_t oy0 = __umul24(iy >> 2, V.b_sy) + __umul24(ya, G::row);
        const uint32_t oy1 = oy0 + (ya == 3u ? V.b_sy - 3u * G::row : G::row);
        const uint32_t m0  = __umul24(iz >> G::zlog2, V.b_sz64);
        const uint32_t m1  = m0 + (za == G::bz - 1u ? V.b_sz64 : 0u);
        const uint32_t zi0 = __umul24(za, 4u * G::row), zi1 = za == G::bz - 1u ? 0u : zi0 + 4u * G::row;
        const char *L0 = (const char *)V.bricks + ((uint64_t)m0 << 6);
        const char *L1 = (const char *)V.bricks + ((uint64_t)m1 << 6);
        if constexpr (VOXEL == VV_VOXEL_F32) {
            const uint32_t ox = brick_x_offset<VOXEL>(ix);
            const uint32_t o0 = ox + oy0, o1 = ox + oy1;
            if constexpr (G::halo != 0) {
                C.a = *(const float2u *)(L0 + (o0 + zi0)); C.b = *(const float2u *)(L0 + (o1 + zi0));
                C.c = *(const float2u *)(L1 + (o0 + zi1)); C.d = *(const float2u *)(L1 + (o1 + zi1));
            } else {
                const uint32_t dx = (ix & (G::bx - 1u)) == G::bx - 1u ? G::brick - (G::bx - 1u) * 4u : 4u;
                const char *pa = L0 + (o0 + zi0), *pb = L0 + (o1 + zi0), *pc = L1 + (o0 + zi1), *pd = L1 + (o1 + zi1);
                const float a0 = *(const float *)pa, b0 = *(const float *)pb, c0 = *(const float *)pc, d0 = *(const float *)pd;
                const float a1 = *(const float *)(pa + dx), b1 = *(const float *)(pb + dx), c1 = *(const float *)(pc + dx), d1 = *(const float *)(pd + dx);
                C.a = {a0, a1}; C.b = {b0, b1}; C.c = {c0, c1}; C.d = {d0, d1};
            }
        } else {
            const uint32_t ox = (ix >> 2) * G::brick;
            const uint32_t o0 = ox + oy0, o1 = ox + oy1;
            C.sh = ix & 3u;
            const uint2 ra = *(const uint2 *)(L0 + (o0 + zi0)), rb = *(const uint2 *)(L0 + (o1 + zi0));
            const uint2 rc = *(const uint2 *)(L1 + (o0 + zi1)), rd = *(const uint2 *)(L1 + (o1 + zi1));
            C.a0 = ra.x; C.a1 = ra.y; C.b0 = rb.x; C.b1 = rb.y; C.c0 = rc.x; C.c1 = rc.y; C.d0 = rd.x; C.d1 = rd.y;
        }
    }
}

typedef float __attribute__((ext_vector_type(4), aligned(8))) float4u;
typedef float __attribute__((ext_vector_type(2))) float2v;
struct CornersZ { float wx, c000, c001, c100, c101, wy, c010, c011, c110, c111, wz; };

template <bool TEX8>
__device__ __forceinline__ void fetch_corners_zpair(const VolumeView &V, float px, float py, float pz, CornersZ &C)
{
    uint32_t ix, iy, iz;
    C.wx = axis_coord<TEX8>(px, (float)V.nx, (float)(V.nx - 1), ix);
    C.wy = axis_coord<TEX8>(py, (float)V.ny, (float)(V.ny - 1), iy);
    C.wz = axis_coord<TEX8>(pz, (float)V.nz, (float)(V.nz - 1), iz);
#ifdef VV_XPAIR
    const char *zb = (const char *)V.zpair + (uint64_t)ix * V.zp_slab_bytes;
    const uint32_t off = __umul24(iy, V.zp_row_bytes) + (iz << 3);
    const float4u r0 = *(const float4u *)(zb + off);
    const float4u r1 = *(const float4u *)(zb + off + V.zp_row_bytes);
    C.c000 = r0.x; C.c100 = r0.y; C.c001 = r0.z; C.c101 = r0.w;
    C.c010 = r1.x; C.c110 = r1.y; C.c011 = r1.z; C.c111 = r1.w;
#else
    const char *zb = (const char *)V.zpair + (uint64_t)iz * V.zp_slab_bytes;
    const uint32_t off = __umul24(iy, V.zp_row_bytes) + (ix << 3);
    const float4u r0 = *(const float4u *)(zb + off);
    const float4u r1 = *(const float4u *)(zb + off + V.zp_row_bytes);
    C.c000 = r0.x; C.c001 = r0.y; C.c100 = r0.z; C.c101 = r0.w;
    C.c010 = r1.x; C.c011 = r1.y; C.c110 = r1.z; C.c111 = r1.w;
#endif
}

struct CornersZ8 { float wx; uint32_t r0; float wy; uint32_t r1; float wz; };
typedef uint32_t __attribute__((aligned(2))) uint32_a2;

template <bool TEX8>
__device__ __forceinline__ void fetch_corners_zpair(const VolumeView &V, float px, float py, float pz, CornersZ8 &C)
{
    uint32_t ix, iy, iz;
    C.wx = axis_coord<TEX8>(px, (float)V.nx, (float)(V.nx - 1), ix);
    C.wy = axis_coord<TEX8>(py, (float)V.ny, (float)(V.ny - 1), iy);
    C.wz = axis_coord<TEX8>(pz, (float)V.nz, (float)(V.nz - 1), iz);
    const char *b0 = (const char *)V.zpair, *b1 = b0 + V.zp_row_bytes;
#ifdef VV_XPAIR
    const uint32_t off = ix * V.zp_slab_bytes + __umul24(iy, V.zp_row_bytes) + (iz << 1);
#else
    const uint32_t off = iz * V.zp_slab_bytes + __umul24(iy, V.zp_row_bytes) + (ix << 1);
#endif
    C.r0 = *(const uint32_a2 *)(b0 + off);
    C.r1 = *(const uint32_a2 *)(b1 + off);
}

__device__ __forceinline__ float finish_corners(const CornersZ8 &C)
{
#ifdef VV_XPAIR
    const float c000 = (float)(C.r0 & 0xffu), c100 = (float)((C.r0 >> 8) & 0xffu), c001 = (float)((C.r0 >> 16) & 0xffu), c101 = (float)(C.r0 >> 24);
    const float c010 = (float)(C.r1 & 0xffu), c110 = (float)((C.r1 >> 8) & 0xffu), c011 = (float)((C.r1 >> 16) & 0xffu), c111 = (float)(C.r1 >> 24);
#else
    const float c000 = (float)(C.r0 & 0xffu), c001 = (float)((C.r0 >> 8) & 0xffu), c100 = (float)((C.r0 >> 16) & 0xffu), c101 = (float)(C.r0 >> 24);
    const float c010 = (float)(C.r1 & 0xffu), c011 = (float)((C.r1 >> 8) & 0xffu), c110 = (float)((C.r1 >> 16) & 0xffu), c111 = (float)(C.r1 >> 24);
#endif
    const float c00 = __builtin_fmaf(C.wx, c100 - c000, c000);
    const float c10 = __builtin_fmaf(C.wx, c110 - c010, c010);
    const float c01 = __builtin_fmaf(C.wx, c101 - c001, c001);
    const float c11 = __builtin_fmaf(C.wx, c111 - c011, c011);
    const float c0 = __builtin_fmaf(C.wy, c10 - c00, c00);
    const float c1 = __builtin_fmaf(C.wy, c11 - c01, c01);
    return __builtin_fmaf(C.wz, c1 - c0, c0);
}

__device__ __forceinline__ float finish_corners(const CornersZ &C)
{
    const float2v lo0 = {C.c000, C.c001}, hi0 = {C.c100, C.c101}, lo1 = {C.c010, C.c011}, hi1 = {C.c110, C.c111};
    const float2v wx = {C.wx, C.wx}, wy = {C.wy, C.wy};
    const float2v cy0 = __builtin_elementwise_fma(wx, hi0 - lo0, lo0);
    const float2v cy1 = __builtin_elementwise_fma(wx, hi1 - lo1, lo1);
    const float2v cz  = __builtin_elementwise_fma(wy, cy1 - cy0, cy0);
    return __builtin_fmaf(C.wz, cz.y - cz.x, cz.x);
}

template <int VOXEL>
__device__ __forceinline__ float finish_corners(const Corners<VOXEL> &C)
{
    float c000, c100, c010, c110, c001, c101, c011, c111;
    if constexpr (VOXEL == VV_VOXEL_F32) {
        c000 = C.a.x; c100 = C.a.y; c010 = C.b.x; c110 = C.b.y; c001 = C.c.x; c101 = C.c.y; c011 = C.d.x; c111 = C.d.y;
    } else {
        const uint32_t a = __builtin_amdgcn_alignbyte(C.a1, C.a0, C.sh), b = __builtin_amdgcn_alignbyte(C.b1, C.b0, C.sh);
        const uint32_t c = __builtin_amdgcn_alignbyte(C.c1, C.c0, C.sh), d = __builtin_amdgcn_alignbyte(C.d1, C.d0, C.sh);
#ifdef VV_ZFAST
        c000 = (float)(a & 0xffu); c001 = (float)((a >> 8) & 0xffu); c010 = (float)(b & 0xffu); c011 = (float)((b >> 8) & 0xffu);
        c100 = (float)(c & 0xffu); c101 = (float)((c >> 8) & 0xffu); c110 = (float)(d & 0xffu); c111 = (float)((d >> 8) & 0xffu);
#else
        c000 = (float)(a & 0xffu); c100 = (float)((a >> 8) & 0xffu); c010 = (float)(b & 0xffu); c110 = (float)((b >> 8) & 0xffu);
        c001 = (float)(c & 0xffu); c101 = (float)((c >> 8) & 0xffu); c011 = (float)(d & 0xffu); c111 = (float)((d >> 8) & 0xffu);
#endif
    }
    float c00 = __builtin_fmaf(C.wx, c100 - c000, c000);
    float c10 = __builtin_fmaf(C.wx, c110 - c010, c010);
    float c01 = __builtin_fmaf(C.wx, c101 - c001, c001);
    float c11 = __builtin_fmaf(C.wx, c111 - c011, c011);
    float c0 = __builtin_fmaf(C.wy, c10 - c00, c00);
    float c1 = __builtin_fmaf(C.wy, c11 - c01, c01);
    return __builtin_fmaf(C.wz, c1 - c0, c0);
}

template <int VOXEL, bool TEX8, bool BIG = false>
__device__ __forceinline__ float tex3d_raw(const VolumeView &V, float px, float py, float pz)
{
    Corners<VOXEL> C;
    fetch_corners<VOXEL, TEX8, BIG ? LAYOUT_LINEAR_BIG : LAYOUT_LINEAR>(V, px, py, pz, C);
    return finish_corners<VOXEL>(C);
}

__device__ __forceinline__ bool bounds_check(float x, float y, float z)
{
    uint32_t m = max(max(__float_as_uint(x), __float_as_uint(y)), __float_as_uint(z));
    return m < 0x3F800000u;
}

template <int VOXEL> __device__ __forceinline__ float corner_value(const Corners<VOXEL> &C) { return finish_corners<VOXEL>(C); }
template <int VOXEL> __device__ __forceinline__ float corner_value(const CornersZ &C) { return finish_corners(C); }
template <int VOXEL> __device__ __forceinline__ float corner_value(const CornersZ8 &C) { return finish_corners(C); }

template <int VOXEL>
__device__ __forceinline__ uint32_t index_of(float L)
{
    float s = (VOXEL == VV_VOXEL_F32) ? L * 255.0f : L;
    return min((uint32_t)s, 255u);
}
template <int VOXEL, class CT>
__device__ __forceinline__ uint32_t classify_raw(const CT &C)
{
    return index_of<VOXEL>(corner_value<VOXEL>(C));
}
template <int VOXEL, class CT>
__device__ __forceinline__ uint32_t classify_index(const CT &C, float px, float py, float pz)
{
    uint32_t idx = index_of<VOXEL>(corner_value<VOXEL>(C));
    return bounds_check(px, py, pz) ? idx : 0u;
}
template <int VOXEL, bool TEX8, bool BIG = false>
__device__ __forceinline__ uint32_t sample_index(const VolumeView &V, float px, float py, float pz)
{
    Corners<VOXEL> C;
    fetch_corners<VOXEL, TEX8, BIG ? LAYOUT_LINEAR_BIG : LAYOUT_LINEAR>(V, px, py, pz, C);
    return classify_index<VOXEL>(C, px, py, pz);
}

__device__ __forceinline__ uint32_t pack_rgba(float r, float g, float b, float a)
{
    uint32_t R = (uint32_t)(fmaxf(0.f, fminf(r, 1.f)) * 255.0f);
    uint32_t G = (uint32_t)(fmaxf(0.f, fminf(g, 1.f)) * 255.0f);
    uint32_t B = (uint32_t)(fmaxf(0.f, fminf(b, 1.f)) * 255.0f);
    uint32_t A = (uint32_t)(fmaxf(0.f, fminf(a, 1.f)) * 255.0f);
    return R | (G << 8) | (B << 16) | (A << 24);
}

__device__ __forceinline__ float ph_div_core(float n, float d)
{
    const float y0 = __builtin_amdgcn_rcpf(d);
    const float e = __builtin_fmaf(-d, y0, 1.0f);
    const float y = __builtin_fmaf(e, y0, y0);
    const float q0 = n * y;
    const float r0 = __builtin_fmaf(-d, q0, n);
    const float q1 = __builtin_fmaf(r0, y, q0);
    const float r1 = __builtin_fmaf(-d, q1, n);
    return __builtin_fmaf(r1, y, q1);
}
__device__ __forceinline__ float ph_sqrt_core(float x)
{
    const float s0 = __builtin_amdgcn_sqrtf(x);
    const float sm = __uint_as_float(__float_as_uint(s0) - 1u), sp = __uint_as_float(__float_as_uint(s0) + 1u);
    const float t1 = __builtin_fmaf(-sm, s0, x);
    float s = (0.f >= t1) ? sm : s0;
    const float t2 = __builtin_fmaf(-sp, s0, x);
    s = (0.f < t2) ? sp : s;
    return s;
}

struct InstrArgs {
    uint32_t *bricks;
    uint32_t *lines;
    uint64_t  line_bits;
    int       lines_all;
    unsigned long long *pairs;
    uint32_t  pairs_log2;
#ifdef VV_TIMELINE
    unsigned long long *timeline;
#endif
};
__device__ __forceinline__ void mark_line_range(const InstrArgs &I, uint64_t off, uint32_t bytes)
{
    for (uint64_t l = off >> 7; l <= (off + bytes - 1u) >> 7; ++l) {
        if (I.lines && l < I.line_bits) {
            const uint32_t bit = 1u << (l & 31);
            if (!(I.lines[l >> 5] & bit)) atomicOr(&I.lines[l >> 5], bit);
        }
        if (I.pairs) {
            const unsigned long long key = ((unsigned long long)(blockIdx.x + 1u) << 36) | (l & 0xFFFFFFFFFull);
            const unsigned long long mask = (1ull << I.pairs_log2) - 1ull;
            unsigned long long h = (key * 0x9E3779B97F4A7C15ull) >> (64u - I.pairs_log2);
            for (int probe = 0; probe < (1 << 14); ++probe, h = (h + 1ull) & mask) {
                const unsigned long long seen = I.pairs[h];
                if (seen == key) break;
                if (seen == 0ull) { const unsigned long long old = atomicCAS(&I.pairs[h], 0ull, key); if (old == 0ull || old == key) break; }
            }
        }
    }
}

// ... 33 lines not shown
```

### volume-viz_amd/csrc/vv_kernels.h

```cpp
#pragma once
#include <hip/hip_runtime.h>
#include "vv_device.h"
#include "vv_tiles.h"

namespace vv {

struct PixelRect { int x0, x1, y0, y1; };

struct SlabMap  { int r0, band, band_stride, n_regular;
                  int gx0, wg, gs0, gs1; };

#define VV_FOR_EACH_BUILD(X, K) X(K, MB_LINEAR) X(K, MB_LINEAR_BIG) X(K, MB_BRICKED) X(K, MB_BRICKED_CACHED) X(K, MB_ZPAIR) X(K, MB_ZFAST) X(K, MB_XPAIR)
#define VV_X(K, B) B,
enum MarchBuild : uint8_t { VV_FOR_EACH_BUILD(VV_X, ) MB_COUNT };
#undef VV_X

enum FrameKind { FRAME_COMPOSITE = 0, FRAME_MIP = 2, FRAME_ISO = 3, FRAME_PROJ = 4 };
#define VV_FOR_EACH_KIND(X) X(FRAME_COMPOSITE) X(FRAME_MIP) X(FRAME_ISO) X(FRAME_PROJ)
#define VV_X(K) K,
constexpr FrameKind kFrameKinds[] = { VV_FOR_EACH_KIND(VV_X) };
#undef VV_X
constexpr int kFrameKindCount = sizeof(kFrameKinds) / sizeof(kFrameKinds[0]);
constexpr int frame_row(FrameKind k) { int r = 0; while (r < kFrameKindCount - 1 && kFrameKinds[r] != k) ++r; return r; }

struct IsoParams { int level; float h[3]; float n[3]; };

struct MarchArgs {
    FrameParams P;
    VolumeView  V;
    int V_type;
    bool tex8, gray, phong, instr;
    MarchBuild build;
    int lds_reserve;
    int unroll;
    int lds_reserve_phong;
    StripMap strips;
    PixelRect rect;
    bool fill_outside;
    uint32_t *order_out;
    SlabMap slabs;
    const float4 *tf;
    const float *rad;
    float *rad_out;
    const float4 *fill_tf;
    uint32_t *pixels;
    uint8_t *index;
    float4 *hit;
    IsoParams iso;
    uint2 *stat;
    int proj_mode;
    unsigned long long *counter;
    InstrArgs I;
};

template <int KIND, MarchBuild B> void launch_frame(const MarchArgs &a, hipStream_t s);
#define VV_X(K, B) template <> void launch_frame<K, B>(const MarchArgs &, hipStream_t);
#define VV_ROW(K) VV_FOR_EACH_BUILD(VV_X, K)
VV_FOR_EACH_KIND(VV_ROW)
#undef VV_ROW
#undef VV_X
using MarchLauncher = void (*)(const MarchArgs &, hipStream_t);
#define VV_X(K, B) launch_frame<K, B>,
#define VV_ROW(K) { VV_FOR_EACH_BUILD(VV_X, K) },
constexpr MarchLauncher kLaunch[][MB_COUNT] = { VV_FOR_EACH_KIND(VV_ROW) };
#undef VV_ROW
#undef VV_X
static_assert(sizeof(kLaunch) == sizeof(MarchLauncher) * kFrameKindCount * MB_COUNT, "one launcher per frame kind and build");
void launch_rad(const MarchArgs &a, hipStream_t s);
constexpr int kMipTableBytes = 4096;
void launch_fill(const MarchArgs &a, const PixelRect &rect, hipStream_t s);
void launch_mip_classify(const uint8_t *index, size_t n, const float4 *tf, uint32_t *pixels, hipStream_t s);
void launch_build_xpair(int vtype, const void *zfast, uint32_t zf_row_bytes, uint64_t zf_slice_bytes, void *xpair, int nx, int ny, int nz, hipStream_t s);
void launch_build_zfast(int vtype, const void *vol, uint32_t row_pitch, uint64_t slice_pitch, void *out, uint32_t zf_row_bytes, uint64_t zf_slice_bytes, int nx, int ny, int nz, hipStream_t s);
size_t zpair_copy_bytes(int vtype, int nx, int ny, int nz, uint32_t *row_bytes, uint32_t *slab_bytes);
void launch_build_zpair(int vtype, const void *linear, size_t row_pitch, size_t slice_pitch, void *zpair, int nx, int ny, int nz, hipStream_t s);
void launch_repitch(const void *dense, void *pitched, size_t row_bytes , size_t ny, size_t nz,
                    size_t row_pitch, size_t slice_pitch, hipStream_t s);
size_t brick_copy_bytes(int vtype, int nx, int ny, int nz, uint32_t *sy, uint32_t *sz64);
void launch_build_bricks(int vtype, const void *linear, size_t row_pitch, size_t slice_pitch, void *bricks, int nx, int ny, int nz, hipStream_t s);
struct SliceArgs {
    VolumeView V; int V_type; bool tex8;
    float *buffer; size_t height, width;
    float dx, dy, dz; int orientation; int legacy;
    float scale[3];
    float trans[16]; int advanced;
};
void launch_slice(const SliceArgs &a, hipStream_t s);
struct SlabArgs {
    VolumeView V; int V_type; bool tex8;
    float *buffer; int32_t *aux; size_t height, width;
    float dx, dy, dz; int orientation;
    float scale[3];
    float trans[16]; int advanced;
    int mode, samples; float thickness;
};
void launch_slab(const SlabArgs &a, hipStream_t s);
struct HistRuns {
    const void *data0; int vtype; int tight;
    uint64_t run_voxels, row_step, slice_step;
    uint32_t rps, n_slices;
};
constexpr int kHistAccNan = 256, kHistAccKeys = 257, kHistAccWords = 258;
void launch_hist(const HistRuns &r, int n_cu, int max_blocks , unsigned long long *acc, hipStream_t s);
void launch_hist_finish(const unsigned long long *acc, int vtype, unsigned long long voxels, vv_histogram *out, unsigned long long *counts ,
                        hipStream_t s);
void launch_first_pass(const FrameParams &P, uint32_t *front, uint32_t *back, hipStream_t s);

size_t generate_scratch_floats(int nx, int ny, int nz, int n);
void launch_generate_ellipsoids(uint8_t *out, int nx, int ny, int nz, int n,
                                const float *centers, const float *axes, const uint8_t *colors,
                                int in_place, float *scratch , hipStream_t s);
void launch_promote_u8_f32(const uint8_t *in, float *out, size_t n, hipStream_t s);
void launch_noise_u8(uint8_t *out, int nx, int ny, int nz, uint32_t seed, hipStream_t s);

constexpr int kMaxEllipsoids = 64;

}
```

### volume-viz_amd/csrc/vv_layout.h

```cpp
#pragma once
#include <type_traits>
#include "vv_device.h"
#include "vv_kernels.h"

#if defined(VV_ZPAIR) && defined(VV_XPAIR)
#define VV_BIG_NS xpair
constexpr vv::MarchBuild kBuild = vv::MB_XPAIR;
constexpr int kLayout = vv::LAYOUT_ZPAIR;
#elif defined(VV_ZPAIR)
#define VV_BIG_NS zpair
constexpr vv::MarchBuild kBuild = vv::MB_ZPAIR;
constexpr int kLayout = vv::LAYOUT_ZPAIR;
#elif defined(VV_BRICKED) && defined(VV_BRICKED_CACHED)
#define VV_BIG_NS brickc
constexpr vv::MarchBuild kBuild = vv::MB_BRICKED_CACHED;
constexpr int kLayout = vv::LAYOUT_BRICKED;
#elif defined(VV_BRICKED)
#define VV_BIG_NS brick
constexpr vv::MarchBuild kBuild = vv::MB_BRICKED;
constexpr int kLayout = vv::LAYOUT_BRICKED;
#elif defined(VV_ZFAST)
#define VV_BIG_NS zfast
constexpr vv::MarchBuild kBuild = vv::MB_ZFAST;
constexpr int kLayout = vv::LAYOUT_ZFAST;
#elif defined(VV_BIG_VOLUME)
#define VV_BIG_NS big
constexpr vv::MarchBuild kBuild = vv::MB_LINEAR_BIG;
constexpr int kLayout = vv::LAYOUT_LINEAR_BIG;
#else
#define VV_BIG_NS small
#define VV_BUILD_LINEAR
constexpr vv::MarchBuild kBuild = vv::MB_LINEAR;
constexpr int kLayout = vv::LAYOUT_LINEAR;
#endif

namespace vv {
namespace VV_BIG_NS {

template <int VOXEL> struct CornerSel { using type = Corners<VOXEL>; };
#ifdef VV_ZPAIR
template <> struct CornerSel<VV_VOXEL_F32> { using type = CornersZ; };
template <> struct CornerSel<VV_VOXEL_U8>  { using type = CornersZ8; };
#endif
template <int VOXEL, bool TEX8, class CT>
__device__ __forceinline__ void fetch_any(const VolumeView &V, float px, float py, float pz, CT &C)
{
#ifdef VV_ZPAIR
    fetch_corners_zpair<TEX8>(V, px, py, pz, C);
#else
    fetch_corners<VOXEL, TEX8, kLayout>(V, px, py, pz, C);
#endif
}

template <int VOXEL, bool TEX8>
__device__ __noinline__ void mark_sample_lines(const InstrArgs &I, const VolumeView &V, float px, float py, float pz)
{
    uint32_t ix, iy, iz;
    (void)axis_coord<TEX8>(px, (float)V.nx, (float)(V.nx - 1), ix);
    (void)axis_coord<TEX8>(py, (float)V.ny, (float)(V.ny - 1), iy);
    (void)axis_coord<TEX8>(pz, (float)V.nz, (float)(V.nz - 1), iz);
    constexpr bool F = VOXEL == VV_VOXEL_F32;
#if defined(VV_ZPAIR)
    const uint32_t rec = F ? 8u : 2u, bytes = F ? 16u : 4u;
#ifdef VV_XPAIR
    const uint64_t off = (uint64_t)ix * V.zp_slab_bytes + (uint64_t)iy * V.zp_row_bytes + (uint64_t)iz * rec;
#else
    const uint64_t off = (uint64_t)iz * V.zp_slab_bytes + (uint64_t)iy * V.zp_row_bytes + (uint64_t)ix * rec;
#endif
    mark_line_range(I, off, bytes); mark_line_range(I, off + V.zp_row_bytes, bytes);
#else
    if constexpr (kLayout == LAYOUT_LINEAR || kLayout == LAYOUT_LINEAR_BIG) {
        const uint64_t o = (uint64_t)iz * V.slice_bytes + (uint64_t)iy * V.row_bytes + (F ? ix * 4u : (ix & ~3u));
        mark_line_range(I, o, 8); mark_line_range(I, o + V.row_bytes, 8);
        mark_line_range(I, o + V.slice_bytes, 8); mark_line_range(I, o + V.slice_bytes + V.row_bytes, 8);
    } else if constexpr (kLayout == LAYOUT_ZFAST) {
        const uint64_t o = (uint64_t)ix * V.zf_slice_bytes + (uint64_t)iy * V.zf_row_bytes + (F ? iz * 4u : (iz & ~3u));
        mark_line_range(I, o, 8); mark_line_range(I, o + V.zf_row_bytes, 8);
        mark_line_range(I, o + V.zf_slice_bytes, 8); mark_line_range(I, o + V.zf_slice_bytes + V.zf_row_bytes, 8);
    } else {
        using G = BrickGeom<VOXEL>;
        uint64_t a[4];
        brick_offsets<VOXEL>(V, ix, iy, iz, a);
        if constexpr (F && G::halo == 0) {
            const uint32_t dx = (ix & (G::bx - 1u)) == G::bx - 1u ? G::brick - (G::bx - 1u) * 4u : 4u;
            for (int k = 0; k < 4; ++k) { mark_line_range(I, a[k], 4); mark_line_range(I, a[k] + dx, 4); }
        } else {
            for (int k = 0; k < 4; ++k) mark_line_range(I, a[k], 8);
        }
    }
#endif
}

template <int VOXEL, bool TEX8>
__device__ __forceinline__ void instrument_sample(const InstrArgs &I, const VolumeView &V, float tx, float ty, float tz, bool live, unsigned long long &executed)
{
    const bool inv = bounds_check(tx, ty, tz);
    if (live) {
        executed++;
        if (I.bricks && inv) mark_bricks(I.bricks, V, tx, ty, tz);
    }
    if ((I.lines || I.pairs) && (I.lines_all || (live && inv))) mark_sample_lines<VOXEL, TEX8>(I, V, tx, ty, tz);
}

__device__ __forceinline__ void flush_counters(unsigned long long *__restrict__ counter, unsigned long long executed, unsigned long long slots)
{
    const bool first = (threadIdx.x & 63) == 0;
    for (int o = 32; o > 0; o >>= 1) executed += __shfl_down(executed, o);
    if (first && executed) atomicAdd(counter, executed);
    if (first && slots) atomicAdd(counter + 1, slots);
    if (kLayout == LAYOUT_BRICKED && first && executed) atomicAdd(counter + 2, 1ull);
    if (kLayout == LAYOUT_ZPAIR && first && executed) atomicAdd(counter + 3, 1ull);
}

template <int N> using int_c = std::integral_constant<int, N>;
template <class F> static void with_bool(bool b, F &&f) { if (b) f(std::true_type{}); else f(std::false_type{}); }
template <class F> static void for_sampler(const MarchArgs &a, F &&f)
{
    with_bool(a.instr, [&](auto instr) { with_bool(a.V_type == VV_VOXEL_F32, [&](auto f32) { with_bool(a.tex8, [&](auto tex8) {
        f(int_c<decltype(f32)::value ? VV_VOXEL_F32 : VV_VOXEL_U8>{}, tex8, instr);
    }); }); });
}
template <class F> static void for_unroll(const MarchArgs &a, F &&f) { if (a.unroll == 3) f(int_c<3>{}); else f(int_c<2>{}); }
template <class F> static void for_variant(const MarchArgs &a, F &&f)
{
    for_sampler(a, [&](auto VOXEL, auto TEX8, auto INSTR) { for_unroll(a, [&](auto U) { f(VOXEL, TEX8, INSTR, U); }); });
}

static inline size_t reducer_lds(const MarchArgs &a) { return (size_t)a.lds_reserve + kMipTableBytes; }

}
}
```

### volume-viz_amd/csrc/vv_raymarch.hip

```cpp
#include "vv_device.h"
#include "vv_kernels.h"

#include "vv_layout.h"

namespace vv {
namespace VV_BIG_NS {

__device__ __forceinline__ int point_life_class(const FrameParams &P, const StripMap &M, int gx, int gy)
{
    const float x = (float)((M.tx0 + gx) << M.blk_log2w) - 0.5f, y = (float)strip_row(M, M.s0 + gy) - 0.5f;
    const float sx = ((2.0f * (x + 0.5f)) / (float)P.W - 1.0f) * P.tan_half_x, sy = ((2.0f * (y + 0.5f)) / (float)P.H - 1.0f) * P.tan_half_y;
    float tmin = 0.f, tmax = INFINITY, d2 = 0.f, s2 = 0.f;
    bool miss = false;
    for (int a = 0; a < 3; a++) {
        const float d = P.side[a] * sx + P.up[a] * sy + P.look[a], o = P.cam_pos[a], sc = P.scale[a];
        d2 += d * d; s2 += sc * sc;
        if (d != 0.0f) { const float t1 = (-sc - o) / d, t2 = (sc - o) / d; tmin = fmaxf(tmin, fminf(t1, t2)); tmax = fminf(tmax, fmaxf(t1, t2)); }
        else if (o < -sc || o > sc) miss = true;
    }
    float len = (miss || !(tmin <= tmax)) ? 0.f : (tmax - tmin) * sqrtf(d2);
    const float cls = len / (2.0f * sqrtf(s2)) * 64.f;
    const int k = cls >= 63.f ? 63 : (cls > 0.f ? (int)cls : 0);
    return 63 - k;
}

constexpr int kMaxUnits = 1024, kMaxPoints = 24576;
__global__ __launch_bounds__(256) void rad_kernel(FrameParams P, float *__restrict__ rad, PixelRect R, uint32_t *__restrict__ pixels,
                                                  StripMap M, uint32_t *__restrict__ order)
{
    if (order && blockIdx.x == gridDim.x - 1) {
        __shared__ uint32_t w[kMaxUnits];
        __shared__ uint8_t pts[kMaxPoints];
        const int cols = M.wr, rows = M.s1 - M.s0, run = M.order_run, nseg = order_units_per_row(M), U = order_units(M), n = cols * rows;
        for (int i = threadIdx.x; i < U; i += 256) w[i] = 0;
        for (int i = threadIdx.x; i < order_words(M); i += 256) order[i] = ~0u;
        __syncthreads();
        {
            const int gw = cols + 1, np = gw * (rows + 1);
            for (int i = threadIdx.x; i < np; i += 256) pts[i] = (uint8_t)point_life_class(P, M, i % gw, i / gw);
            __syncthreads();
            for (int t = threadIdx.x; t < n; t += 256) {
                const int tx = t % cols, ty = t / cols;
                const int c = min(min((int)pts[ty * gw + tx], (int)pts[ty * gw + tx + 1]), min((int)pts[(ty + 1) * gw + tx], (int)pts[(ty + 1) * gw + tx + 1]));
                atomicAdd(&w[ty * nseg + tx / run], 64u - (uint32_t)c);
            }
        }
        __syncthreads();
        for (int u = threadIdx.x; u < U; u += 256) {
            const uint32_t wu = w[u];
            int rank = 0;
            for (int v = 0; v < U; ++v) { const uint32_t wv = w[v]; rank += (wv > wu || (wv == wu && v < u)) ? 1 : 0; }
            const int c = rank & 7, r = rank >> 3, xcd = (r & 1) ? 7 - c : c;
            const int row = u / nseg, x0 = (u % nseg) * run, size = min(run, cols - x0);
            uint32_t *dst = order + order_slot(M, r, xcd, 0);
            for (int i = 0; i < size; ++i) dst[i] = (uint32_t)(row * cols + x0 + i);
        }
        return;
    }
    const int slab = blockIdx.x * 4 + (threadIdx.x >> 6), lane = threadIdx.x & 63;
    if (slab >= P.nbx * P.nby) return;
    const int bx = slab % P.nbx, by = slab / P.nbx;
    if (!row_owned(P, by * kSlab) && !(P.conflict_y && by == P.nby - 1)) return;
    const int sx0 = bx * kSlab, sy0 = by * kSlab;
    const bool meets = sx0 < R.x1 && sx0 + kSlab > R.x0 && sy0 < R.y1 && sy0 + kSlab > R.y0;
    const bool inside = sx0 >= R.x0 && sx0 + kSlab <= R.x1 && sy0 >= R.y0 && sy0 + kSlab <= R.y1;
    if (!inside && row_owned(P, sy0)) {
#pragma unroll
        for (int q = 0; q < 4; ++q) {
            const int t = lane + 64 * q, tx = t % kSlab, ty = t / kSlab;
            const int x = sx0 + tx, y = sy0 + ty;
            if (t < kSlab * kSlab && x <= P.W - 2 && y <= P.H - 2 && !(x >= R.x0 && x < R.x1 && y >= R.y0 && y < R.y1)) pixels[(size_t)y * P.W + x] = 0u;
        }
    }
    if (!rad || (!meets && !(P.conflict_x && bx == P.nbx - 1) && !(P.conflict_y && by == P.nby - 1))) return;
    const int lox = slab_lo(bx), upx = slab_up(bx, P.W) - 1, loy = slab_lo(by), upy = slab_up(by, P.H) - 1;
    float m = 0.f;
#pragma unroll
    for (int q = 0; q < 4; ++q) {
        const int t = lane + 64 * q, tx = t & 15, ty = t >> 4;
        int x = bx * kSlab + tx - 1, y = by * kSlab + ty - 1;
        x = max(lox, min(x, upx));
        y = max(loy, min(y, upy));
// ... 381 lines not shown
                float cr = e.x, cg = e.y, cb = e.z, ca = e.w;
                if (ca > kEps) {
                    const uint32_t qf = s_before, qa = s_next;
                    const uint32_t ql = cache[i][nl], qr = cache[i][nr], qt = cache[i][nt], qb = cache[i][nb];
                    float direct = 0.f;
                    if (!(qr == ql && qt == qb && qa == qf)) {
                        float f = q255[qf], a = q255[qa], l = q255[ql], rr = q255[qr], t = q255[qt], b = q255[qb];
                        float gx, gy, gz;
                        if (P.safe_div) {
                            gx = ph_div_core(rr - l, P.tan_fov_x * vd); gy = ph_div_core(t - b, P.tan_fov_y * vd); gz = ph_div_core(a - f, r.sstep * 2.f);
                            if (gx != 0.f && gy != 0.f && gz != 0.f) {
                                float inv = ph_div_core(1.0f, ph_sqrt_core(gx * gx + gy * gy + gz * gz));
                                gx *= inv; gy *= inv; gz *= inv;
                            }
                        } else {
                            gx = (rr - l) / (P.tan_fov_x * vd); gy = (t - b) / (P.tan_fov_y * vd); gz = (a - f) / (r.sstep * 2.f);
                            if (gx != 0.f && gy != 0.f && gz != 0.f) {
                                float inv = 1.0f / sqrtf(gx * gx + gy * gy + gz * gz);
                                gx *= inv; gy *= inv; gz *= inv;
                            }
                        }
                        direct = (gx * -1.f + gy * -1.f + gz * 1.f) * 0.3f;
                        direct = fmaxf(0.f, fminf(direct, 0.3f));
                    }
                    cr = cr * 0.7f + direct; cg = cg * 0.7f + direct; cb = cb * 0.7f + direct;
                }
                if (SLICE == SLICE_PLANE) {
                    float vx = r.origin.x + r.dir.x * vd, vy = r.origin.y + r.dir.y * vd, vz = r.origin.z + r.dir.z * vd;
                    float d = fabsf(sn.x * (vx - sp.x) + sn.y * (vy - sp.y) + sn.z * (vz - sp.z));
                    if (d < .01f) cr = fmaxf(0.f, fminf(cr + (.01f - d) * 100.f, 1.f));
                }
                if (ca > kEps) {
                    float bf = ca * (1.f - res_a);
                    res_r = res_r + cr * bf; res_g = res_g + cg * bf; res_b = res_b + cb * bf; res_a = res_a + bf;
                }
                if (res_a > P.ert_thr) { if (P.ert_true) ert_done = true; break; }
            }
        }
        {
#pragma clang fp contract(off)
            dist += r.sstep * kChunkSteps;
        }
        if (chunk + 1 < P.max_chunks) post_need((chunk + 1) & 1);
        __syncthreads();
    }

    if (writer)
        pixels[(size_t)y * P.W + x] = skip ? 0u : pack_rgba(res_r, res_g, res_b, res_a);
#ifdef VV_TIMELINE
    if (I.timeline && threadIdx.x == 0) {
        unsigned long long *t = I.timeline + 4ull * blockIdx.x;
        t[0] = tl0; t[1] = wall_clock64(); t[2] = ((unsigned long long)by << 16) | (unsigned)bx;
        t[3] = (__builtin_amdgcn_s_getreg((3 << 11) | 20) & 15u) | 256u | ((unsigned long long)__builtin_amdgcn_s_getreg((31 << 11) | 4) << 16);
    }
#endif
    if (INSTR) flush_counters(counter, executed, 0ull);
}

template <int SLICE, int VOXEL, bool TEX8, bool GRAY, bool INSTR>
static void launch_march(const MarchArgs &a, hipStream_t s)
{
    const unsigned nblocks = grid_blocks(a.strips);
    if (!nblocks) return;
    dim3 grid(nblocks);
    if (a.unroll == 3)
        hipLaunchKernelGGL((march_kernel<SLICE, VOXEL, TEX8, GRAY, INSTR, 3>), grid, dim3(256), (size_t)a.lds_reserve, s,
                           a.P, a.V, a.tf, a.rad, a.pixels, a.counter, a.I, a.strips);
    else
        hipLaunchKernelGGL((march_kernel<SLICE, VOXEL, TEX8, GRAY, INSTR, 2>), grid, dim3(256), (size_t)a.lds_reserve, s,
                           a.P, a.V, a.tf, a.rad, a.pixels, a.counter, a.I, a.strips);
}
template <int SLICE, int VOXEL, bool TEX8, bool INSTR>
static void launch_phong(const MarchArgs &a, hipStream_t s)
{
    const int rows = a.slabs.gs1 - a.slabs.gs0 + 1;
    constexpr int BAND = VV_PHONG_BAND;
    if (a.slabs.wg <= 0) return;
    dim3 grid((unsigned)(((rows + 8 * BAND - 1) / (8 * BAND)) * 8 * BAND * a.slabs.wg));
    hipLaunchKernelGGL((march_phong_kernel<SLICE, VOXEL, TEX8, INSTR>), grid, dim3(256), (size_t)a.lds_reserve_phong, s,
                       a.P, a.V, a.tf, a.slabs, a.pixels, a.counter, a.I);
}

template <int SLICE, int VOXEL, bool TEX8>
static void dispatch3(const MarchArgs &a, hipStream_t s)
{
    if (a.phong) {
        if (a.instr) launch_phong<SLICE, VOXEL, TEX8, true>(a, s); else launch_phong<SLICE, VOXEL, TEX8, false>(a, s);
        return;
    }
    const bool gray = a.gray && SLICE != SLICE_PLANE;
    if (gray) { if (a.instr) launch_march<SLICE, VOXEL, TEX8, true, true>(a, s); else launch_march<SLICE, VOXEL, TEX8, true, false>(a, s); }
    else      { if (a.instr) launch_march<SLICE, VOXEL, TEX8, false, true>(a, s); else launch_march<SLICE, VOXEL, TEX8, false, false>(a, s); }
}
template <int SLICE>
static void dispatch2(const MarchArgs &a, hipStream_t s)
{
    if (a.V_type == VV_VOXEL_F32) { if (a.tex8) dispatch3<SLICE, VV_VOXEL_F32, true>(a, s); else dispatch3<SLICE, VV_VOXEL_F32, false>(a, s); }
    else                          { if (a.tex8) dispatch3<SLICE, VV_VOXEL_U8,  true>(a, s); else dispatch3<SLICE, VV_VOXEL_U8,  false>(a, s); }
}

static void launch_rad_impl(const MarchArgs &a, hipStream_t s)
{
    dim3 grid((unsigned)((a.P.nbx * a.P.nby + 3) / 4) + (a.order_out ? 1u : 0u));
    hipLaunchKernelGGL(rad_kernel, grid, dim3(256), 0, s, a.P, a.rad_out, a.rect, a.pixels, a.strips, a.order_out);
}

static void launch_raymarch_impl(const MarchArgs &a, hipStream_t s)
{
    switch (a.P.slice_type) {
    case SLICE_PLANE:     dispatch2<SLICE_PLANE>(a, s); break;
    case SLICE_PLANE_CUT: dispatch2<SLICE_PLANE_CUT>(a, s); break;
    default:              dispatch2<SLICE_NONE>(a, s); break;
    }
}

}

template <> void launch_frame<FRAME_COMPOSITE, kBuild>(const MarchArgs &a, hipStream_t s) { VV_BIG_NS::launch_raymarch_impl(a, s); }
#ifdef VV_BUILD_LINEAR
void launch_rad(const MarchArgs &a, hipStream_t s) { small::launch_rad_impl(a, s); }
#endif

}
```

### volume-viz_amd/host/device_math_check.hip

```cpp
#include <hip/hip_runtime.h>
#include <algorithm>
#include <cmath>
#include <cstdio>
#include <cstdlib>
#include <cstring>
#include <string>
#include <vector>
#include "../csrc/vv_device.h"
#include "../csrc/vv_gate.h"

using namespace vv;

#define HIP_OK(e) do { hipError_t e_ = (e); if (e_ != hipSuccess) { fprintf(stderr, "device_math_check: %s: %s\n", #e, hipGetErrorString(e_)); exit(2); } } while (0)

struct Record {
    unsigned long long mismatches;
    unsigned int noted, pad;
    unsigned int ops[8][4];
};
__device__ __forceinline__ void note(Record *R, uint32_t a, uint32_t b, uint32_t c, uint32_t d)
{
    if (*(volatile unsigned int *)&R->noted < 8u) {
        const unsigned int s = atomicAdd(&R->noted, 1u);
        if (s < 8u) { R->ops[s][0] = a; R->ops[s][1] = b; R->ops[s][2] = c; R->ops[s][3] = d; }
    }
}
__device__ __forceinline__ void tally(Record *R, unsigned long long bad) { if (bad) atomicAdd(&R->mismatches, bad); }
__device__ __forceinline__ double wide(float v) { double w = (double)v; asm volatile("" : "+v"(w)); return w; }
__device__ __forceinline__ unsigned long long thread_index() { return (unsigned long long)blockIdx.x * blockDim.x + threadIdx.x; }

struct DenSpec { int lo, hi; };
__host__ __device__ inline unsigned long long den_count(const DenSpec &S) { return (unsigned long long)(S.hi - S.lo + 1) << 23; }
__device__ __forceinline__ float den_of(const DenSpec &S, unsigned long long idx) { return __uint_as_float((uint32_t)(((unsigned long long)(127 + S.lo) << 23) + idx)); }
template <int TWIN>
__device__ __forceinline__ float twin_div(float n, float d)
{
    const float y0 = __builtin_amdgcn_rcpf(d);
    const float e = __builtin_fmaf(-d, y0, 1.0f);
    const float y = __builtin_fmaf(e, y0, y0);
    const float q0 = n * y;
    if (TWIN == 1) return q0;
    const float r0 = __builtin_fmaf(-d, q0, n);
    return __builtin_fmaf(r0, y, q0);
}
template <int TWIN>
__global__ __launch_bounds__(256) void div_kernel(const float *__restrict__ nums, int n_nums, DenSpec S, Record *R)
{
    const unsigned long long idx = thread_index();
    if (idx >= den_count(S)) return;
    const float d = den_of(S, idx);
    const double dd = wide(d);
    unsigned long long bad = 0;
    for (int j = 0; j < n_nums; ++j) {
        const float n = nums[j];
        const float got = TWIN ? twin_div<TWIN>(n, d) : ph_div_core(n, d);
        const float want = (float)(wide(n) / dd);
        if (__float_as_uint(got) != __float_as_uint(want)) { ++bad; note(R, __float_as_uint(n), __float_as_uint(d), __float_as_uint(got), __float_as_uint(want)); }
    }
    tally(R, bad);
}

constexpr int kSqrtLo = -52, kSqrtHi = 86;
constexpr unsigned long long kSqrtCount = (unsigned long long)(kSqrtHi - kSqrtLo + 1) << 23;
template <int TWIN> __device__ __forceinline__ float twin_sqrt(float x)
{
    const float s0 = __builtin_amdgcn_sqrtf(x);
    const float sm = __uint_as_float(__float_as_uint(s0) - 1u), sp = __uint_as_float(__float_as_uint(s0) + 1u);
    float s = s0;
    if (TWIN != 2) { const float t1 = __builtin_fmaf(-sm, s0, x); s = (0.f >= t1) ? sm : s0; }
    if (TWIN != 1) { const float t2 = __builtin_fmaf(-sp, s0, x); s = (0.f < t2) ? sp : s; }
    return s;
}
template <int TWIN>
__global__ __launch_bounds__(256) void sqrt_kernel(Record *R, Record *Rinv)
{
    unsigned long long bad = 0, bad_inv = 0;
    for (unsigned long long idx = thread_index(); idx < kSqrtCount; idx += (unsigned long long)gridDim.x * blockDim.x) {
        const float x = __uint_as_float((uint32_t)(((unsigned long long)(127 + kSqrtLo) << 23) + idx));
        const float s = TWIN ? twin_sqrt<TWIN>(x) : ph_sqrt_core(x);
        const float want = (float)sqrt(wide(x));
        if (__float_as_uint(s) != __float_as_uint(want)) { ++bad; note(R, __float_as_uint(x), 0u, __float_as_uint(s), __float_as_uint(want)); }
        if (!TWIN) {
            const float inv = ph_div_core(1.0f, s), want_inv = (float)(1.0 / wide(s));
            if (__float_as_uint(inv) != __float_as_uint(want_inv)) { ++bad_inv; note(Rinv, __float_as_uint(1.0f), __float_as_uint(s), __float_as_uint(inv), __float_as_uint(want_inv)); }
        }
    }
    tally(R, bad); if (!TWIN) tally(Rinv, bad_inv);
}

constexpr int kAxisSizes = 12;
__constant__ uint32_t c_axis_sizes[kAxisSizes] = {1u, 2u, 3u, 5u, 7u, 16u, 255u, 256u, 257u, 1024u, 2048u, (1u << 24) - 1u};
constexpr uint32_t kUnitPatterns = 0x3F800000u;
// ... 91 lines not shown
    float s = (VOXEL == VV_VOXEL_F32) ? L * 255.0f : L;
    return min((uint32_t)(s + 0.5f), 255u);
}
template <int TWIN>
__global__ __launch_bounds__(256) void convert_kernel(Record *R)
{
    unsigned long long bad = 0;
    for (unsigned long long idx = thread_index(); idx < (1ull << 32); idx += (unsigned long long)gridDim.x * blockDim.x) {
        const float v = __uint_as_float((uint32_t)idx);
        const uint32_t g8 = TWIN ? twin_index_of<VV_VOXEL_U8>(v) : index_of<VV_VOXEL_U8>(v), w8 = ref_convert(v);
        const uint32_t gf = TWIN ? twin_index_of<VV_VOXEL_F32>(v) : index_of<VV_VOXEL_F32>(v), wf = ref_convert(ref_times255(v));
        const float c = (v != v) ? 1.0f : (v < 0.0f ? 0.0f : (v > 1.0f ? 1.0f : v));
        const uint32_t gp = pack_rgba(v, 0.f, 0.f, 0.f), wp = ref_convert(ref_times255(c));
        if (g8 != w8) { ++bad; note(R, (uint32_t)idx, 0u, g8, w8); }
        if (gf != wf) { ++bad; note(R, (uint32_t)idx, 1u, gf, wf); }
        if (gp != wp) { ++bad; note(R, (uint32_t)idx, 2u, gp, wp); }
    }
    tally(R, bad);
}

constexpr unsigned long long kChunkRandom = 1ull << 28, kChunkPairs = 1ull << 20, kChunkPerPair = 32 * 5, kChunkNan = 1024, kChunkBehind = 1024;
constexpr unsigned long long kChunkCount = kChunkRandom + kChunkPairs * kChunkPerPair + kChunkNan + kChunkBehind;
struct ChunkSpec { float sstep_lo, sstep_hi, log2_lo, log2_hi; };
__device__ __forceinline__ unsigned long long mix64(unsigned long long z)
{
    z += 0x9E3779B97F4A7C15ull; z = (z ^ (z >> 30)) * 0xBF58476D1CE4E5B9ull; z = (z ^ (z >> 27)) * 0x94D049BB133111EBull; return z ^ (z >> 31);
}
__device__ __forceinline__ float ulp_move(float f, int by)
{
    const uint32_t b = __float_as_uint(f);
    long long o = (b & 0x80000000u) ? -(long long)(b & 0x7FFFFFFFu) : (long long)b;
    o += by;
    return __uint_as_float(o < 0 ? (0x80000000u | (uint32_t)(-o)) : (uint32_t)o);
}
__device__ __forceinline__ int ref_chunks(float dist, float upper, float sstep)
{
#pragma clang fp contract(off)
    if (!(dist < upper)) return 0;
    int n = 0;
    for (int i = 1; i <= 30; ++i) {
        const float vd = (float)i * sstep + dist;
        if (vd > upper) break;
        ++n;
    }
    return n;
}
__device__ __forceinline__ int twin_chunks(float dist, float upper, float sstep)
{
#pragma clang fp contract(off)
    if (!(dist < upper)) return 0;
    float est = (upper - dist) / sstep;
    int n = est >= 30.f ? 30 : (est > 0.f ? (int)est : 0);
    while (n < 30 && !((float)(n + 1) * sstep + dist >= upper)) ++n;
    while (n > 0 && ((float)n * sstep + dist >= upper)) --n;
    if (sstep != sstep) n = 30;
    return n;
}
template <int TWIN>
__global__ __launch_bounds__(256) void chunks_kernel(ChunkSpec S, Record *R)
{
#pragma clang fp contract(off)
    unsigned long long bad = 0;
    for (unsigned long long idx = thread_index(); idx < kChunkCount; idx += (unsigned long long)gridDim.x * blockDim.x) {
        unsigned long long j = idx, key;
        int kind;
        if (j < kChunkRandom) { kind = 0; key = j; }
        else if ((j -= kChunkRandom) < kChunkPairs * kChunkPerPair) { kind = 1; key = (1ull << 40) + j / kChunkPerPair; }
        else if ((j -= kChunkPairs * kChunkPerPair) < kChunkNan) { kind = 2; key = (2ull << 40) + j; }
        else { j -= kChunkNan; kind = 3; key = (3ull << 40) + j; }
        const unsigned long long h0 = mix64(key ^ 0x20251018ull), h1 = mix64(h0);
        const float u0 = (float)(h0 & 0xFFFFFFu) * 0x1p-24f, u1 = (float)((h0 >> 24) & 0xFFFFFFu) * 0x1p-24f, u2 = (float)(h1 & 0xFFFFFFu) * 0x1p-24f;
        float sstep = fminf(S.sstep_hi, fmaxf(S.sstep_lo, exp2f(S.log2_lo + u0 * (S.log2_hi - S.log2_lo))));
        float dist = u1 * kSqrt3, upper;
        if (kind == 0) upper = (h1 >> 63) ? u2 * kSqrt3 : dist + u2 * 32.f * sstep;
        else if (kind == 1) { const int r = (int)(j % kChunkPerPair); upper = ulp_move((float)(r / 5) * sstep + dist, r % 5 - 2); }
        else if (kind == 2) { upper = u2 * kSqrt3 * 1.5f; sstep = __uint_as_float((j & 1) ? 0x7FC00000u : 0xFFC00001u); }
        else { upper = dist * u2; if (!(upper < dist)) upper = dist - 1.0f; }
        const int got = TWIN ? twin_chunks(dist, upper, sstep) : chunk_count(dist, upper, sstep), want = ref_chunks(dist, upper, sstep);
        if (got != want) { ++bad; note(R, __float_as_uint(dist), __float_as_uint(upper), __float_as_uint(sstep), ((uint32_t)got << 8) | (uint32_t)want); }
    }
    tally(R, bad);
}

static const char *kNames[] = {"div", "sqrt", "axis", "bounds", "convert", "chunks"};
constexpr int kSweeps = 6;

struct Result { unsigned long long visited = 0; Record rec = {}; float seconds = 0.f; };

struct Timer {
    hipEvent_t a, b;
    Timer() { HIP_OK(hipEventCreate(&a)); HIP_OK(hipEventCreate(&b)); HIP_OK(hipEventRecord(a, 0)); }
    float stop() { float ms = 0.f; HIP_OK(hipEventRecord(b, 0)); HIP_OK(hipEventSynchronize(b)); HIP_OK(hipEventElapsedTime(&ms, a, b)); (void)hipEventDestroy(a); (void)hipEventDestroy(b); return ms * 1e-3f; }
};
static Record *new_record() { Record *r; HIP_OK(hipMalloc(&r, sizeof(Record))); HIP_OK(hipMemset(r, 0, sizeof(Record))); return r; }
static Record take(Record *d) { Record h; HIP_OK(hipDeviceSynchronize()); HIP_OK(hipMemcpy(&h, d, sizeof h, hipMemcpyDeviceToHost)); HIP_OK(hipFree(d)); return h; }
static unsigned blocks_for(unsigned long long n) { return (unsigned)((n + 255) / 256); }
constexpr unsigned kStrideBlocks = 1u << 16;

struct Ranges { double sstep_lo, sstep_hi, den_lo, den_hi; int derived_lo, derived_hi, lo, hi; double nmin; };
static std::vector<float> numerators()
{
    float q[256];
    for (int i = 0; i < 256; ++i) q[i] = (float)i / 255.f;
    std::vector<uint32_t> bits;
    for (int i = 0; i < 256; ++i) for (int j = 0; j < 256; ++j) { volatile float n = q[i] - q[j]; float v = n; uint32_t b; memcpy(&b, &v, 4); bits.push_back(b); }
    std::sort(bits.begin(), bits.end()); bits.erase(std::unique(bits.begin(), bits.end()), bits.end());
    std::vector<float> out(bits.size());
    for (size_t k = 0; k < bits.size(); ++k) memcpy(&out[k], &bits[k], 4);
    return out;
}
static Ranges ranges(const std::vector<float> &nums)
{
    Ranges r;
    const double few = 0x1p-20;
    r.sstep_lo = (double)kStepMin * (1.0 - few); r.sstep_hi = (double)kSafeDivStepMax * (1.0 + few);
    const double vd_lo = r.sstep_lo, vd_hi = (double)kSqrt3 + 30.0 * r.sstep_hi;
    r.den_lo = std::min((double)kSafeDivTanLo * vd_lo, 2.0 * r.sstep_lo);
    r.den_hi = std::max((double)kSafeDivTanHi * vd_hi, 2.0 * r.sstep_hi);
    r.derived_lo = ilogb(r.den_lo); r.derived_hi = ilogb(r.den_hi);
    r.nmin = 1.0;
    for (float n : nums) if (n != 0.f) r.nmin = std::min(r.nmin, (double)fabsf(n));
    r.lo = std::min(r.derived_lo, ilogb(1.0 / 0x1p42)); r.hi = std::max(r.derived_hi, ilogb(r.nmin / 0x1p-26));
    return r;
}
static void guard(bool ok, const char *what) { if (!ok) { fprintf(stderr, "device_math_check: range guard failed: %s\n", what); exit(3); } }

template <int TWIN> static Result run_div()
{
    const std::vector<float> nums = numerators();
    const Ranges g = ranges(nums);
    guard(g.lo <= g.derived_lo && g.hi >= g.derived_hi, "swept binades contain the derived ones");
    guard(1.0 / ldexp(1.0, g.lo) >= 0x1p42 && g.nmin / ldexp(1.0, g.hi + 1) <= 0x1p-26, "swept quotients contain [2^-26, 2^42]");
    DenSpec S = {g.lo, g.hi};
    float *d_nums; HIP_OK(hipMalloc(&d_nums, nums.size() * 4)); HIP_OK(hipMemcpy(d_nums, nums.data(), nums.size() * 4, hipMemcpyHostToDevice));
    Record *R = new_record();
    Result out; Timer t;
    div_kernel<TWIN><<<blocks_for(den_count(S)), 256>>>(d_nums, (int)nums.size(), S, R);
    HIP_OK(hipGetLastError());
    out.seconds = t.stop(); out.rec = take(R); out.visited = den_count(S) * nums.size();
    HIP_OK(hipFree(d_nums));
    return out;
}
template <int TWIN> static Result run_sqrt(Result *inv)
{
    const std::vector<float> nums = numerators();
    const Ranges g = ranges(nums);
    const double qmin = g.nmin / g.den_hi, qmax = 1.0 / g.den_lo;
    guard(qmin * qmin >= ldexp(1.0, kSqrtLo) && 3.0 * qmax * qmax * (1.0 + 0x1p-20) < ldexp(1.0, kSqrtHi + 1), "swept radicands contain the derived ones");
    guard(kSqrtLo <= -52 && kSqrtHi >= 86, "swept radicands contain [2^-52, 2^86]");
    Record *R = new_record(), *Ri = new_record();
    Result out; Timer t;
    sqrt_kernel<TWIN><<<kStrideBlocks, 256>>>(R, Ri);
    HIP_OK(hipGetLastError());
    out.seconds = t.stop(); out.rec = take(R); out.visited = kSqrtCount;
    Record ri = take(Ri);
    if (inv) { inv->rec = ri; inv->visited = kSqrtCount; }
    return out;
}
template <int TWIN> static Result run_axis()
{
    Record *R = new_record(); Result out; Timer t;
    const unsigned long long n = (unsigned long long)kUnitPatterns + kAxisExtras;
    axis_kernel<TWIN><<<blocks_for(n), 256>>>(R);
    HIP_OK(hipGetLastError());
    out.seconds = t.stop(); out.rec = take(R); out.visited = n * kAxisSizes * 2;
    return out;
}
template <int TWIN> static Result run_bounds()
{
    Record *R = new_record(); Result out; Timer t;
    bounds_kernel<TWIN><<<kStrideBlocks, 256>>>(R);
    HIP_OK(hipGetLastError());
    out.seconds = t.stop(); out.rec = take(R); out.visited = 3ull << 32;
    return out;
}
template <int TWIN> static Result run_convert()
{
    Record *R = new_record(); Result out; Timer t;
    convert_kernel<TWIN><<<kStrideBlocks, 256>>>(R);
    HIP_OK(hipGetLastError());
    out.seconds = t.stop(); out.rec = take(R); out.visited = 3ull << 32;
    return out;
}
template <int TWIN> static Result run_chunks()
{
    const Ranges g = ranges(numerators());
    ChunkSpec S = {(float)g.sstep_lo, (float)g.sstep_hi, (float)log2(g.sstep_lo), (float)log2(g.sstep_hi)};
    Record *R = new_record(); Result out; Timer t;
    chunks_kernel<TWIN><<<kStrideBlocks, 256>>>(S, R);
    HIP_OK(hipGetLastError());
    out.seconds = t.stop(); out.rec = take(R); out.visited = kChunkCount;
    return out;
}

static std::string first_json(const Record &r)
{
    std::string s = "[";
    const unsigned n = r.noted < 8u ? r.noted : 8u;
    char buf[96];
    for (unsigned k = 0; k < n; ++k) {
        snprintf(buf, sizeof buf, "%s[\"0x%08x\", \"0x%08x\", \"0x%08x\", \"0x%08x\"]", k ? ", " : "", r.ops[k][0], r.ops[k][1], r.ops[k][2], r.ops[k][3]);
        s += buf;
    }
    return s + "]";
}

int main(int argc, char **argv)
{
    bool self_test = false, want[kSweeps] = {}, any = false;
    for (int a = 1; a < argc; ++a) {
        if (!strcmp(argv[a], "--list")) { for (const char *n : kNames) printf("%s\n", n); return 0; }
        if (!strcmp(argv[a], "--self-test")) { self_test = true; continue; }
        int k = 0;
        while (k < kSweeps && strcmp(argv[a], kNames[k])) ++k;
        if (k == kSweeps) { fprintf(stderr, "usage: device_math_check [--list] [--self-test] [div|sqrt|axis|bounds|convert|chunks ...]\n"); return 2; }
        want[k] = any = true;
    }
    int rc = 0;
    for (int k = 0; k < kSweeps; ++k) {
        if (any && !want[k]) continue;
        Result r, inv, twin, twin2;
        std::string extra;
        char buf[256];
        bool clean;
        switch (k) {
        case 0: {
            r = run_div<0>(); if (self_test) { twin = run_div<1>(); twin2 = run_div<2>(); }
            const std::vector<float> nums = numerators(); const Ranges g = ranges(nums);
            snprintf(buf, sizeof buf, ", \"numerators\": %zu, \"binade_lo\": %d, \"binade_hi\": %d, \"derived_lo\": %d, \"derived_hi\": %d, \"mantissas_per_binade\": %d",
                     nums.size(), g.lo, g.hi, g.derived_lo, g.derived_hi, 1 << 23);
            extra = buf;
            if (self_test) { snprintf(buf, sizeof buf, ", \"self_test_without_last_step\": %llu", twin2.rec.mismatches); extra += buf; }
            clean = r.rec.mismatches == 0; break; }
        case 1:
            r = run_sqrt<0>(&inv); if (self_test) { twin = run_sqrt<1>(nullptr); twin2 = run_sqrt<2>(nullptr); }
            snprintf(buf, sizeof buf, ", \"binade_lo\": %d, \"binade_hi\": %d, \"root_mismatches\": %llu, \"reciprocal_mismatches\": %llu, \"first_reciprocal\": ", kSqrtLo, kSqrtHi,
                     r.rec.mismatches, inv.rec.mismatches);
            extra = buf + first_json(inv.rec);
            if (self_test) { snprintf(buf, sizeof buf, ", \"self_test_without_lower_test\": %llu", twin2.rec.mismatches); extra += buf; }
            r.rec.mismatches += inv.rec.mismatches;
            clean = r.rec.mismatches == 0; break;
        case 2: r = run_axis<0>(); if (self_test) twin = run_axis<1>(); clean = r.rec.mismatches == 0; break;
        case 3: {
            r = run_bounds<0>(); if (self_test) twin = run_bounds<1>();
            bool seen[3] = {};
            clean = r.rec.mismatches == 3 && r.rec.noted == 3;
            for (unsigned m = 0; clean && m < 3; ++m) {
                if (r.rec.ops[m][0] != 0x80000000u || r.rec.ops[m][1] > 2u || seen[r.rec.ops[m][1]]) clean = false; else seen[r.rec.ops[m][1]] = true;
            }
            std::string set = "[";
            std::vector<uint32_t> pats;
            for (unsigned m = 0; m < std::min(r.rec.noted, 8u); ++m) pats.push_back(r.rec.ops[m][0]);
            std::sort(pats.begin(), pats.end()); pats.erase(std::unique(pats.begin(), pats.end()), pats.end());
            for (size_t m = 0; m < pats.size(); ++m) { snprintf(buf, sizeof buf, "%s\"0x%08x\"", m ? ", " : "", pats[m]); set += buf; }
            extra = ", \"disagreeing_patterns\": " + set + "]";
            break; }
        case 4: r = run_convert<0>(); if (self_test) twin = run_convert<1>(); clean = r.rec.mismatches == 0; break;
        default: r = run_chunks<0>(); if (self_test) twin = run_chunks<1>(); clean = r.rec.mismatches == 0; break;
        }
        if (!clean) rc = 1;
        std::string st;
        if (self_test) {
            snprintf(buf, sizeof buf, ", \"self_test_mismatches\": %llu, \"self_test_seconds\": %.3f", twin.rec.mismatches, twin.seconds);
            st = buf;
            if (twin.rec.mismatches == 0) rc = 1;
        }
        printf("{\"sweep\": \"%s\", \"visited\": %llu, \"mismatches\": %llu, \"first\": %s, \"seconds\": %.3f%s%s}\n", kNames[k], r.visited, r.rec.mismatches,
               first_json(r.rec).c_str(), r.seconds, extra.c_str(), st.c_str());
        fflush(stdout);
    }
    return rc;
}
```

### volume-viz_amd/python/volviz_amd/__init__.py

```python
from __future__ import annotations

import ctypes as C
import os
from dataclasses import dataclass, field
from typing import Optional, Sequence

import numpy as np

_HERE = os.path.dirname(os.path.abspath(__file__))
PKG_ROOT = os.path.normpath(os.path.join(_HERE, "..", ".."))
REPO_ROOT = os.path.normpath(os.path.join(PKG_ROOT, ".."))
LIB_PATH = os.environ.get("VV_LIB", os.path.join(PKG_ROOT, "lib", "libvolviz_hip.so"))

SLICE_NONE, SLICE_PLANE, SLICE_PLANE_CUT = -1, 0, 1
HORIZONTAL, SAGITTAL, CORONAL, FREE_FORM = 0, 1, 2, 4
VOXEL_U8, VOXEL_F32 = 0, 1
LAYOUT_BRICKED, LAYOUT_ZPAIR, LAYOUT_ZFAST, LAYOUT_POLICY = 1, 2, 4, 256
FILTER_TEX8, FILTER_EXACT = 0, 1
ERT_REFERENCE, ERT_TRUE = 0, 1
SLAB_MAX, SLAB_MIN, SLAB_MEAN = 0, 1, 2
SLAB_MAX_SAMPLES = 1024
PROJ_MAX, PROJ_MIN, PROJ_MEAN = 0, 1, 2
RAYS_IMAGES, RAYS_ANALYTIC = 0, 1
TF_ENGINE, TF_HEAD, TF_MRI = 0, 1, 2
STREAM_DEFAULT_ASYNC = 1


def stream_handle(torch_stream) -> int:
    h = int(torch_stream.cuda_stream)
    return h if h != 0 else STREAM_DEFAULT_ASYNC


class slice_params(C.Structure):
    _fields_ = [("type", C.c_int), ("params", C.c_float * 6)]


class camera_params(C.Structure):
    _fields_ = [("origin", C.c_float * 3), ("fovX", C.c_float), ("fovY", C.c_float),
                ("scale", C.c_float * 3)]


class shading_params(C.Structure):
    _fields_ = [("transferPreset", C.c_int), ("phongShading", C.c_bool)]


class vv_ray_source(C.Structure):
    _fields_ = [("mode", C.c_int), ("front", C.c_void_p), ("back", C.c_void_p),
                ("img_w", C.c_int), ("img_h", C.c_int), ("images_on_device", C.c_int),
                ("look", C.c_float * 3), ("up", C.c_float * 3), ("aspect", C.c_float),
                ("quantize8", C.c_int)]


class vv_render_options(C.Structure):
    _fields_ = [("step", C.c_float * 3), ("ert_threshold", C.c_float), ("filter", C.c_int),
                ("ert_mode", C.c_int), ("slab_row_begin", C.c_int), ("slab_row_end", C.c_int),
                ("shard_band", C.c_int), ("shard_count", C.c_int), ("shard_index", C.c_int),
                ("count_samples", C.c_int), ("touched_bricks", C.c_void_p),
                ("touched_lines", C.c_void_p), ("touched_line_bits", C.c_ulonglong), ("touched_lines_all", C.c_int),
                ("touched_block_lines", C.c_void_p), ("touched_block_lines_log2", C.c_int)]


class vv_slab(C.Structure):
    _fields_ = [("mode", C.c_int), ("samples", C.c_int), ("thickness", C.c_float)]


class vv_histogram(C.Structure):
    _fields_ = [("counts", C.c_ulonglong * 256), ("voxels", C.c_ulonglong), ("nan_voxels", C.c_ulonglong),
                ("vmin", C.c_float), ("vmax", C.c_float)]


@dataclass
class Histogram:
    counts: np.ndarray
    voxels: int
    nan_voxels: int
    vmin: np.float32
    vmax: np.float32

    @staticmethod
    def from_bytes(raw) -> "Histogram":
        raw = np.frombuffer(bytes(raw), np.uint8, C.sizeof(vv_histogram))
        q = raw[:258 * 8].view(np.uint64)
        f = raw[258 * 8:].view(np.float32)
        return Histogram(q[:256].copy(), int(q[256]), int(q[257]), f[0], f[1])


EXPORTS = [
    "vv_init", "vv_shutdown", "vv_last_error", "vv_load_volume_u8", "vv_load_volume_f32",
    "vv_load_volume_device", "vv_set_transfer_function", "vv_render", "vv_slice",
    "vv_slice_advanced", "vv_generate_ellipsoids", "vv_generate_default_brain",
    "vv_promote_u8_to_f32", "vv_generate_noise_u8", "vv_transfer_preset",
    "vv_t3d_read_header", "vv_t3d_read", "vv_t3d_write", "vv_last_frame_ms",
    "vv_last_sample_count", "vv_volume_dims", "vv_slice_matrix", "vv_draw_ellipsoid", "vv_debug_counters",
    "vv_first_pass", "vv_cut_plane_canonical", "vv_cut_plane_from_euler", "vv_cut_plane_to_slice_params", "vv_slice_to_bgra",
    "vv_camera_orbit_drag", "vv_camera_zoom", "vv_cut_plane_from_drag", "vv_cut_plane_drag",
    "vv_prepare_layouts", "vv_set_layout_policy", "vv_layout_state", "vv_device_bytes", "vv_reread_env",
    "vv_load_volume_stream_begin", "vv_load_volume_stream_slices", "vv_load_volume_stream_end", "vv_load_volume_t3d",
    "vv_load_volume_stream_slices_async", "vv_load_volume_stream_wait_source", "vv_dataset_preset", "vv_debug_last_launch", "vv_set_frame_timing", "vv_debug_screen_rect",
    "vv_render_mip", "vv_classify_indices", "vv_render_iso", "vv_slice_slab", "vv_slice_advanced_slab",
    "vv_volume_histogram", "vv_histogram_indices", "vv_render_projection",
]
_NEWER_EXPORTS = ("vv_render_mip", "vv_classify_indices", "vv_render_iso", "vv_slice_slab", "vv_slice_advanced_slab",
                  "vv_volume_histogram", "vv_histogram_indices", "vv_render_projection")

_lib = None
_libs = {}


def load_library(path: Optional[str] = None) -> C.CDLL:
    global _lib
    if _lib is not None and path is None:
        return _lib
    if path is not None and path in _libs:
        return _libs[path]
    p = path or LIB_PATH
    if not os.path.exists(p):
        raise RuntimeError(f"{p} not found: build it with `make -C {PKG_ROOT}` "
                           "(python __graft_entry__.py does). There is no fallback path.")
    lib = C.CDLL(p)
    vp, i, f, sz = C.c_void_p, C.c_int, C.c_float, C.c_size_t
    lib.vv_init.argtypes = [i, C.POINTER(vp)]
    lib.vv_shutdown.argtypes = [vp]
    lib.vv_last_error.argtypes = [vp]; lib.vv_last_error.restype = C.c_char_p
    lib.vv_load_volume_u8.argtypes = [vp, vp, sz, i, i, i, vp]
    lib.vv_load_volume_f32.argtypes = [vp, vp, sz, i, i, i, vp]
    lib.vv_load_volume_device.argtypes = [vp, vp, i, i, i, i, vp, vp]
    lib.vv_set_transfer_function.argtypes = [vp, vp]
    lib.vv_load_volume_stream_begin.argtypes = [vp, i, i, i, i, vp]
    lib.vv_load_volume_stream_slices.argtypes = [vp, vp, i, i, i]
    lib.vv_load_volume_stream_slices_async.argtypes = [vp, vp, i, i, i]
    lib.vv_load_volume_stream_wait_source.argtypes = [vp]
    lib.vv_load_volume_stream_end.argtypes = [vp]
    lib.vv_load_volume_t3d.argtypes = [vp, C.c_char_p, i, i, vp]
    lib.vv_render.argtypes = [vp, i, i, C.POINTER(slice_params), C.POINTER(camera_params),
                              C.POINTER(shading_params), C.POINTER(vv_ray_source),
                              C.POINTER(vv_render_options), vp, i, vp]
    if hasattr(lib, "vv_render_mip"):
        lib.vv_render_mip.argtypes = [vp, i, i, C.POINTER(slice_params), C.POINTER(camera_params), C.POINTER(vv_ray_source),
                                      C.POINTER(vv_render_options), vp, vp, i, vp]
        lib.vv_classify_indices.argtypes = [vp, vp, sz, vp, vp, i, vp]
    if hasattr(lib, "vv_render_iso"):
        lib.vv_render_iso.argtypes = [vp, i, i, C.POINTER(slice_params), C.POINTER(camera_params), C.POINTER(vv_ray_source),
                                      C.POINTER(vv_render_options), i, vp, vp, vp, i, vp]
    if hasattr(lib, "vv_render_projection"):
        lib.vv_render_projection.argtypes = [vp, i, i, C.POINTER(slice_params), C.POINTER(camera_params), C.POINTER(vv_ray_source),
                                             C.POINTER(vv_render_options), i, vp, vp, vp, i, vp]
    lib.vv_slice.argtypes = [vp, vp, sz, sz, f, f, f, i, C.POINTER(f * 3), i, i, i, vp]
    lib.vv_slice_advanced.argtypes = [vp, vp, sz, sz, C.POINTER(f * 16), C.POINTER(f * 3), i, i, vp]
    if hasattr(lib, "vv_slice_slab"):
        lib.vv_slice_slab.argtypes = [vp, vp, vp, sz, sz, f, f, f, i, C.POINTER(f * 3), i, C.POINTER(vv_slab), i, vp]
        lib.vv_slice_advanced_slab.argtypes = [vp, vp, vp, sz, sz, C.POINTER(f * 16), C.POINTER(f * 3), i, C.POINTER(vv_slab), i, vp]
    if hasattr(lib, "vv_volume_histogram"):
        lib.vv_volume_histogram.argtypes = [vp, C.POINTER(i * 3), C.POINTER(i * 3), vp, i, vp]
        lib.vv_histogram_indices.argtypes = [vp, vp, sz, vp, i, vp]
    lib.vv_generate_ellipsoids.argtypes = [vp, vp, i, i, i, i, i, vp, vp, vp, vp]
    lib.vv_generate_default_brain.argtypes = [vp, vp, i, i, i, i, vp]
    lib.vv_draw_ellipsoid.argtypes = [vp, vp, i, i, i, i, vp, vp, C.c_uint8, vp]
    lib.vv_promote_u8_to_f32.argtypes = [vp, vp, vp, sz, vp]
    lib.vv_generate_noise_u8.argtypes = [vp, vp, i, i, i, C.c_uint32, vp]
    lib.vv_transfer_preset.argtypes = [i, vp]
    lib.vv_dataset_preset.argtypes = [C.c_char_p, vp, vp]
    lib.vv_t3d_read_header.argtypes = [C.c_char_p, i, C.POINTER(i), C.POINTER(i), C.POINTER(i)]
    lib.vv_t3d_read.argtypes = [C.c_char_p, i, vp, sz]
    lib.vv_t3d_write.argtypes = [C.c_char_p, i, vp, i, i, i]
    lib.vv_last_frame_ms.argtypes = [vp]; lib.vv_last_frame_ms.restype = f
    lib.vv_last_sample_count.argtypes = [vp]; lib.vv_last_sample_count.restype = C.c_ulonglong
    lib.vv_slice_matrix.argtypes = [f, f, f, f, f, f, vp]
    lib.vv_first_pass.argtypes = [vp, i, i, C.POINTER(camera_params), C.POINTER(vv_ray_source), vp, vp, i, vp]
    lib.vv_cut_plane_canonical.argtypes = [i, f, vp, vp]
    lib.vv_cut_plane_from_euler.argtypes = [f, f, f, f, f, f, vp, vp]
    lib.vv_cut_plane_to_slice_params.argtypes = [i, vp, vp, i, C.POINTER(slice_params)]
    lib.vv_slice_to_bgra.argtypes = [vp, sz, sz, vp]
    lib.vv_camera_orbit_drag.argtypes = [vp, i, i, vp, vp]
    lib.vv_camera_zoom.argtypes = [vp, vp, i, vp]
    lib.vv_cut_plane_from_drag.argtypes = [vp, vp, vp, f, vp, vp, vp, vp, vp, vp]
    lib.vv_cut_plane_drag.argtypes = [vp, vp, vp, i, i, i, i]
    lib.vv_debug_counters.argtypes = [vp, vp]
    lib.vv_debug_last_launch.argtypes = [vp, vp]
    lib.vv_set_frame_timing.argtypes = [vp, i]
    lib.vv_debug_screen_rect.argtypes = [i, i, C.POINTER(camera_params), C.POINTER(vv_ray_source), C.POINTER(C.c_double * 4)]
    lib.vv_reread_env.argtypes = [vp]
    lib.vv_prepare_layouts.argtypes = [vp, i, vp]
    lib.vv_device_bytes.argtypes = [vp, vp]
    lib.vv_set_layout_policy.argtypes = [vp, C.c_ulonglong, i]
    lib.vv_layout_state.argtypes = [vp, vp]
    lib.vv_volume_dims.argtypes = [vp, C.POINTER(i * 3), C.POINTER(i)]
    for name in EXPORTS:
        if path is not None and name in _NEWER_EXPORTS and not hasattr(lib, name):
            continue
        fn = getattr(lib, name)
        if name not in ("vv_last_error", "vv_last_frame_ms", "vv_last_sample_count"):
            fn.restype = i
    if path is None:
        _lib = lib
    else:
        _libs[path] = lib
    return lib


class VolvizError(RuntimeError):
    def __init__(self, code: int, msg: str):
        super().__init__(f"volviz error {code}: {msg}")
        self.code = code


def transfer_preset(preset: int) -> np.ndarray:
    tf = np.zeros(1024, np.float32)
    rc = load_library().vv_transfer_preset(preset, tf.ctypes.data)
    if rc:
        raise VolvizError(rc, "bad preset")
    return tf


def dataset_preset(path: str):
    tfp = C.c_int(-1)
    sc = (C.c_float * 3)(0, 0, 0)
    rc = load_library().vv_dataset_preset(path.encode(), C.byref(tfp), sc)
    if rc < 0:
        raise VolvizError(rc, "bad argument")
    return (tfp.value, (sc[0], sc[1], sc[2])) if rc == 1 else None


@dataclass
class Camera:
    origin: Sequence[float] = (0.0, 0.0, -4.0)
    look_at: Sequence[float] = (0.0, 0.0, 0.0)
    up: Sequence[float] = (0.0, 1.0, 0.0)
    fov_y: float = 45.0
    scale: Sequence[float] = (1.0, 1.0, 1.0)

    def params(self, width: int, height: int) -> camera_params:
        aspect = np.float32(width) / np.float32(height)
        cp = camera_params()
        cp.origin[:] = [float(v) for v in self.origin]
        cp.fovY = float(self.fov_y)
        cp.fovX = float(np.float32(self.fov_y) * aspect)
        cp.scale[:] = [float(v) for v in self.scale]
        return cp

    def look(self):
        return [float(np.float32(t) - np.float32(o)) for t, o in zip(self.look_at, self.origin)]

    @staticmethod
    def orbit(r: float, theta: float, phi: float, **kw) -> "Camera":
        return Camera(origin=(r * np.sin(theta) * np.cos(phi), r * np.cos(theta),
                              r * np.sin(theta) * np.sin(phi)), **kw)


def screen_rect(cam: "Camera", width: int, height: int):
    out = (C.c_double * 4)()
    cp = cam.params(width, height); rs = analytic_rays(cam)
    rc = load_library().vv_debug_screen_rect(width, height, C.byref(cp), C.byref(rs), C.byref(out))
    if rc < 0:
        raise VolvizError(rc, "vv_debug_screen_rect")
    return tuple(out) if rc == 1 else None


def analytic_rays(cam: Camera, quantize8: bool = False, aspect: float = 0.0) -> vv_ray_source:
    rs = vv_ray_source()
    rs.mode = RAYS_ANALYTIC
    rs.look[:] = cam.look()
    rs.up[:] = [float(v) for v in cam.up]
    rs.aspect = aspect
    rs.quantize8 = int(quantize8)
    return rs


def _hint(rs: vv_ray_source, cam: Optional["Camera"], aspect: float) -> vv_ray_source:
    if cam is not None:
        rs.look[:] = cam.look()
        rs.up[:] = [float(v) for v in cam.up]
# ... 160 lines not shown
                   rays: Optional[vv_ray_source] = None, options: Optional[vv_render_options] = None,
                   fill: int = 0, return_index: bool = False, return_hit: bool = False):
        ptrs, res = self._host_images(width, height, fill, (return_index, (), np.uint8), (return_hit, (16,), np.float32))
        self._chk(self.lib.vv_render_iso(self.h, width, height, *self._frame_args(width, height, cam, slice, rays, options), int(level), *ptrs, 0, None))
        return res

    def render_iso_device(self, width: int, height: int, cam: Camera, level: int, rgba_ptr: int = 0, index_ptr: int = 0, hit_ptr: int = 0, *,
                          slice=None, rays=None, options=None, stream: int = 0):
        self._chk(self.lib.vv_render_iso(self.h, width, height, *self._frame_args(width, height, cam, slice, rays, options), int(level),
                                         rgba_ptr or None, index_ptr or None, hit_ptr or None, 1, stream))

    def render_projection(self, width: int, height: int, cam: Camera, mode: int, *, slice: Optional[slice_params] = None,
                          rays: Optional[vv_ray_source] = None, options: Optional[vv_render_options] = None,
                          fill: int = 0, return_index: bool = False, return_stat: bool = False):
        ptrs, res = self._host_images(width, height, fill, (return_index, (), np.uint8), (return_stat, (8,), np.uint32))
        self._chk(self.lib.vv_render_projection(self.h, width, height, *self._frame_args(width, height, cam, slice, rays, options), int(mode), *ptrs, 0, None))
        return res

    def render_projection_device(self, width: int, height: int, cam: Camera, mode: int, rgba_ptr: int = 0, index_ptr: int = 0, stat_ptr: int = 0, *,
                                 slice=None, rays=None, options=None, stream: int = 0):
        self._chk(self.lib.vv_render_projection(self.h, width, height, *self._frame_args(width, height, cam, slice, rays, options), int(mode),
                                                rgba_ptr or None, index_ptr or None, stat_ptr or None, 1, stream))

    def classify_indices(self, index: np.ndarray, tf: Optional[np.ndarray] = None) -> np.ndarray:
        index = np.ascontiguousarray(index, np.uint8)
        out = np.zeros(index.shape + (4,), np.uint8)
        t = None if tf is None else np.ascontiguousarray(tf, np.float32).reshape(1024)
        self._chk(self.lib.vv_classify_indices(self.h, index.ctypes.data, index.size, None if t is None else t.ctypes.data,
                                               out.ctypes.data, 0, None))
        return out

    def classify_indices_device(self, index_ptr: int, n: int, rgba_ptr: int, tf: Optional[np.ndarray] = None, stream: int = 0):
        t = None if tf is None else np.ascontiguousarray(tf, np.float32).reshape(1024)
        self._chk(self.lib.vv_classify_indices(self.h, index_ptr, n, None if t is None else t.ctypes.data, rgba_ptr, 1, stream))

    def first_pass(self, img_w: int, img_h: int, cam: Camera):
        front = np.zeros((img_h, img_w, 4), np.uint8); back = np.zeros((img_h, img_w, 4), np.uint8)
        cp = cam.params(img_w, img_h); rs = analytic_rays(cam)
        self._chk(self.lib.vv_first_pass(self.h, img_w, img_h, C.byref(cp), C.byref(rs), front.ctypes.data, back.ctypes.data, 0, None))
        return front, back

    def first_pass_device(self, img_w: int, img_h: int, cam: Camera, front_ptr: int, back_ptr: int, stream: int = 0):
        cp = cam.params(img_w, img_h); rs = analytic_rays(cam)
        self._chk(self.lib.vv_first_pass(self.h, img_w, img_h, C.byref(cp), C.byref(rs), front_ptr, back_ptr, 1, stream))

    def last_frame_ms(self) -> float:
        return float(self.lib.vv_last_frame_ms(self.h))

    def set_frame_timing(self, on: bool) -> None:
        self._chk(self.lib.vv_set_frame_timing(self.h, int(bool(on))))

    def debug_counters(self):
        out = np.zeros(16, np.uint64)
        self._chk(self.lib.vv_debug_counters(self.h, out.ctypes.data))
        return out

    def last_launch(self) -> dict:
        out = (C.c_int * 8)()
        self._chk(self.lib.vv_debug_last_launch(self.h, out))
        k = ("tile_log2w", "blk_log2w", "unroll", "lds_reserve", "layout", "view_known", "density_x1000", "phong")
        return dict(zip(k, list(out)))

    def reread_env(self):
        self._chk(self.lib.vv_reread_env(self.h))

    def last_sample_count(self) -> int:
        return int(self.lib.vv_last_sample_count(self.h))

    def prepare_layouts(self, which: int = 3, stream=None) -> int:
        rc = self.lib.vv_prepare_layouts(self.h, which, stream)
        if rc < 0:
            self._chk(rc)
        return rc

    def set_layout_policy(self, budget_bytes: int = 0, build_in_render: bool = True):
        self._chk(self.lib.vv_set_layout_policy(self.h, int(budget_bytes), int(build_in_render)))

    def layout_state(self) -> dict:
        out = np.zeros(8, np.uint64)
        self._chk(self.lib.vv_layout_state(self.h, out.ctypes.data))
        k = ("linear", "bricked", "zpair", "zfast", "xpair", "budget", "builds_in_render", "build_in_render")
        return dict(zip(k, (int(v) for v in out)))

    def device_bytes(self):
        out = np.zeros(4, np.uint64)
        self._chk(self.lib.vv_device_bytes(self.h, out.ctypes.data))
        return [int(v) for v in out]

    def slice(self, height: int, width: int, dx=0.0, dy=0.0, dz=0.0, orientation=SAGITTAL,
              scale=(1.0, 1.0, 1.0), legacy=False, filter=FILTER_TEX8, fill=0.0) -> np.ndarray:
        buf = np.full(height * width, fill, np.float32)
        sc = (C.c_float * 3)(*[float(v) for v in scale])
        self._chk(self.lib.vv_slice(self.h, buf.ctypes.data, height, width, dx, dy, dz, orientation,
                                    C.byref(sc), int(legacy), filter, 0, None))
        return buf

    def slice_advanced(self, height: int, width: int, trans: np.ndarray, scale=(1.0, 1.0, 1.0),
                       filter=FILTER_TEX8, fill=0.0) -> np.ndarray:
        buf = np.full(height * width, fill, np.float32)
        t = (C.c_float * 16)(*[float(v) for v in np.asarray(trans, np.float32).reshape(16)])
        sc = (C.c_float * 3)(*[float(v) for v in scale])
        self._chk(self.lib.vv_slice_advanced(self.h, buf.ctypes.data, height, width, C.byref(t), C.byref(sc),
                                             filter, 0, None))
        return buf

    def slice_slab(self, height: int, width: int, dx=0.0, dy=0.0, dz=0.0, orientation=SAGITTAL, *, mode=SLAB_MAX, samples=1,
                   thickness=0.0, scale=(1.0, 1.0, 1.0), filter=FILTER_TEX8, fill=0.0, return_aux=False, aux_fill=-7):
        buf = np.full(height * width, fill, np.float32)
        aux = np.full(height * width, aux_fill, np.int32) if return_aux else None
        self.slice_slab_device(height, width, dx, dy, dz, orientation, buf.ctypes.data, aux.ctypes.data if return_aux else 0,
                               mode=mode, samples=samples, thickness=thickness, scale=scale, filter=filter, stream=None, on_device=False)
        return (buf, aux) if return_aux else buf

    def slice_advanced_slab(self, height: int, width: int, trans: np.ndarray, *, mode=SLAB_MAX, samples=1, thickness=0.0,
                            scale=(1.0, 1.0, 1.0), filter=FILTER_TEX8, fill=0.0, return_aux=False, aux_fill=-7):
        buf = np.full(height * width, fill, np.float32)
        aux = np.full(height * width, aux_fill, np.int32) if return_aux else None
        self.slice_advanced_slab_device(height, width, trans, buf.ctypes.data, aux.ctypes.data if return_aux else 0,
                                        mode=mode, samples=samples, thickness=thickness, scale=scale, filter=filter, stream=None, on_device=False)
        return (buf, aux) if return_aux else buf

    def slice_slab_device(self, height: int, width: int, dx, dy, dz, orientation, buffer_ptr: int, aux_ptr: int = 0, *, mode=SLAB_MAX,
                          samples=1, thickness=0.0, scale=(1.0, 1.0, 1.0), filter=FILTER_TEX8, stream=0, on_device=True):
        sc = (C.c_float * 3)(*[float(v) for v in scale])
        sl = vv_slab(int(mode), int(samples), float(thickness))
        self._chk(self.lib.vv_slice_slab(self.h, buffer_ptr or None, aux_ptr or None, height, width, dx, dy, dz, orientation, C.byref(sc),
                                         filter, C.byref(sl), int(on_device), stream or None))

    def slice_advanced_slab_device(self, height: int, width: int, trans, buffer_ptr: int, aux_ptr: int = 0, *, mode=SLAB_MAX, samples=1,
                                   thickness=0.0, scale=(1.0, 1.0, 1.0), filter=FILTER_TEX8, stream=0, on_device=True):
        t = (C.c_float * 16)(*[float(v) for v in np.asarray(trans, np.float32).reshape(16)])
        sc = (C.c_float * 3)(*[float(v) for v in scale])
        sl = vv_slab(int(mode), int(samples), float(thickness))
        self._chk(self.lib.vv_slice_advanced_slab(self.h, buffer_ptr or None, aux_ptr or None, height, width, C.byref(t), C.byref(sc),
                                                  filter, C.byref(sl), int(on_device), stream or None))

    @staticmethod
    def _box(box):
        if box is None:
            return None, None
        (x0, y0, z0), (x1, y1, z1) = box
        return C.byref((C.c_int * 3)(int(x0), int(y0), int(z0))), C.byref((C.c_int * 3)(int(x1), int(y1), int(z1)))

    def histogram(self, box=None, prefill: int = 0) -> Histogram:
        out = vv_histogram()
        C.memset(C.byref(out), prefill, C.sizeof(out))
        lo, hi = self._box(box)
        self._chk(self.lib.vv_volume_histogram(self.h, lo, hi, C.addressof(out), 0, None))
        return Histogram.from_bytes(out)

    def histogram_device(self, out_ptr: int, box=None, stream: int = 0):
        lo, hi = self._box(box)
        self._chk(self.lib.vv_volume_histogram(self.h, lo, hi, out_ptr or None, 1, stream or None))

    def histogram_indices(self, index: np.ndarray) -> np.ndarray:
        index = np.ascontiguousarray(index, np.uint8)
        counts = np.full(256, 0xA5A5A5A5A5A5A5A5, np.uint64)
        self._chk(self.lib.vv_histogram_indices(self.h, index.ctypes.data if index.size else None, index.size, counts.ctypes.data, 0, None))
        return counts

    def histogram_indices_device(self, index_ptr: int, n: int, counts_ptr: int, stream: int = 0):
        self._chk(self.lib.vv_histogram_indices(self.h, index_ptr or None, n, counts_ptr or None, 1, stream or None))

    def generate_ellipsoids(self, nx: int, ny: int, nz: int, centers, axes, colors) -> np.ndarray:
        centers = np.ascontiguousarray(centers, np.float32).reshape(-1, 3)
        axes = np.ascontiguousarray(axes, np.float32).reshape(-1, 3)
# ... 110 lines not shown
```

Baseline: 218,900.

## Add lossless 16-bit quantised volume copy for f32 data on a uniform grid

Adds a detection pass that checks whether every f32 voxel lies exactly on one of several k/D grids. When one fits, it builds a packed uint16 copy of the volume, and the composite march kernel reads it, dequantising with an exact fma split. This halves the bytes fetched per trilinear sample on large f32 volumes. It costs an extra device copy, a larger layout budget, a one-time detect and pack pass, and a lower LDS reserve. It only applies to composite, non-Phong frames that use neither the bricked nor the zfast layout.

```diff
diff --git a/include/volviz.h b/include/volviz.h
--- a/include/volviz.h
+++ b/include/volviz.h
@@ -226,10 +226,11 @@
 int  vv_t3d_read (const char *path, int header, uint8_t *dst, size_t capacity);
 int  vv_t3d_write(const char *path, int header, const uint8_t *src, int nx, int ny, int nz);
 
-enum { VV_LAYOUT_BRICKED = 1, VV_LAYOUT_ZPAIR = 2, VV_LAYOUT_ZFAST = 4, VV_LAYOUT_POLICY = 256 };
+enum { VV_LAYOUT_BRICKED = 1, VV_LAYOUT_ZPAIR = 2, VV_LAYOUT_ZFAST = 4, VV_LAYOUT_Q16 = 16, VV_LAYOUT_POLICY = 256 };
 int  vv_prepare_layouts(vv_context *ctx, int which, void *stream);
 int  vv_set_layout_policy(vv_context *ctx, unsigned long long budget_bytes , int build_in_render );
 int  vv_layout_state(const vv_context *ctx, unsigned long long out[8]);
+int  vv_debug_voxel_storage(const vv_context *ctx, unsigned long long out[4]);
 int  vv_device_bytes(const vv_context *ctx, unsigned long long out[4]);
 
 float              vv_last_frame_ms(const vv_context *ctx);
diff --git a/volume-viz_amd/csrc/vv_api.cpp b/volume-viz_amd/csrc/vv_api.cpp
--- a/volume-viz_amd/csrc/vv_api.cpp
+++ b/volume-viz_amd/csrc/vv_api.cpp
@@ -17,7 +17,7 @@
 
 struct vv_knobs {
     int tile_log2w = -1, xcd_band = -1, unroll = -1, lds_reserve = -1, lds_reserve_phong = -1;
-    int bricked = -1, zpair = -1, zfast = -1, force_big = 0;
+    int bricked = -1, zpair = -1, zfast = -1, q16 = -1, force_big = 0;
     int block_w = -1, tail = -1, rect = -1, lpt = -1, lpt_run = -1, phong_bricks = -1;
     int hist_blocks = -1;
     static int geti(const char *name, int dflt) { const char *e = getenv(name); return e ? atoi(e) : dflt; }
@@ -27,18 +27,19 @@
         lds_reserve = geti("VV_LDS_RESERVE", -1); lds_reserve_phong = geti("VV_LDS_RESERVE_PHONG", -1);
         bricked = geti("VV_BRICKED", -1); zpair = geti("VV_ZPAIR", -1);
         block_w = geti("VV_BLOCK_W", -1); tail = geti("VV_TAIL", -1);
-        zfast = geti("VV_ZFAST", -1); force_big = getenv("VV_FORCE_BIG") != nullptr;
+        zfast = geti("VV_ZFAST", -1); q16 = geti("VV_Q16", -1); force_big = getenv("VV_FORCE_BIG") != nullptr;
         rect = geti("VV_RECT", -1); lpt = geti("VV_LPT", -1); lpt_run = geti("VV_LPT_RUN", -1); phong_bricks = geti("VV_PHONG_BRICKS", -1);
         hist_blocks = geti("VV_HIST_BLOCKS", -1);
     }
 };
 
-enum { CP_BRICKS = 0, CP_ZPAIR = 1, CP_ZFAST = 2, CP_XPAIR = 3, CP_N = 4 };
+enum { CP_BRICKS = 0, CP_ZPAIR = 1, CP_ZFAST = 2, CP_XPAIR = 3, CP_STATE_N = 4, CP_Q16 = 4, CP_N = 5 };
 struct layout_copy {
     void *ptr = nullptr; size_t bytes = 0;
     bool valid = false, failed = false;
     unsigned long long last_used = 0;
     uint32_t row = 0; uint64_t slab = 0;
+    Q16Grid grid = {0, 0.f, 0.f};
 };
 
 struct vv_context {
@@ -71,6 +72,7 @@
     bool view_key_valid = false, view_est_ok = false; float view_side[3] = {0, 0, 0}, view_px_cube = 0.f;
     std::vector<uint8_t> row_buf;
     int last_launch[8] = {0, 0, 0, 0, 0, 0, 0, 0};
+    int last_storage = 0;
     unsigned long long *d_counter = nullptr;
     unsigned long long *d_hist = nullptr;
     int n_cu = 0;
@@ -110,7 +112,7 @@
         if (cp.ptr) (void)hipFree(cp.ptr);
         cp = layout_copy();
     }
-    c->builds_in_render = 0;
+    c->builds_in_render = 0; c->last_storage = 0;
     c->view_key_valid = false;
 }
 
@@ -173,7 +175,7 @@
 static size_t layout_budget(const vv_context *c)
 {
     if (c->layout_budget_bytes) return c->layout_budget_bytes;
-    return std::max<size_t>((size_t)8 << 30, c->alloc_bytes / 2 * 5);
+    return std::max<size_t>((size_t)8 << 30, c->alloc_bytes / 4 * 11);
 }
 static size_t copy_bytes(const vv_context *c, int k) { return c->copies[k].valid ? c->copies[k].bytes : 0; }
 static void copy_drop(vv_context *c, int k)
@@ -282,13 +284,43 @@
         launch_build_xpair(c->vtype, zf.ptr, zf.row, zf.slab, p, c->nx, c->ny, c->nz, st); });
 }
 
-static bool (*const ensure_copy[CP_N])(vv_context *, hipStream_t) = {ensure_bricks, ensure_zpair, ensure_zfast, ensure_xpair};
+static bool ensure_q16(vv_context *c, hipStream_t st)
+{
+    layout_copy &cp = c->copies[CP_Q16];
+    if (cp.valid || cp.failed) return cp.valid;
+    if (c->vtype != VV_VOXEL_F32) return copy_refused(c, CP_Q16);
+    size_t row = ((size_t)c->nx * 2 + 3) & ~(size_t)3, rows = (size_t)c->ny;
+    if (row % 1024 == 0) { row += 32; if ((rows * row) % 4096 == 0) rows += 1; }
+    const size_t slice = rows * row, bytes = slice * ((size_t)c->nz + 1) + row + 16;
+    const bool big = c->slice_pitch * (size_t)c->nz > (1ull << 32) || c->slice_pitch >= (1u << 24) || c->knobs.force_big;
+    if ((size_t)c->ny * c->nz >= (1ull << 32) || row >= (1u << 24) || slice > 0xFFFFFFF0ull || (!big && (slice >= (1u << 24) || bytes >= (1ull << 32)))) return copy_refused(c, CP_Q16);
+    uint32_t *d_off = nullptr, off = ~0u;
+    if (hipMalloc((void **)&d_off, sizeof off) != hipSuccess) { (void)hipGetLastError(); return copy_refused(c, CP_Q16); }
+    bool ok = hipMemsetAsync(d_off, 0, sizeof off, st) == hipSuccess;
+    if (ok) launch_q16_detect(c->d_vol, c->row_pitch, c->slice_pitch, c->nx, c->ny, c->nz, kQ16Grids, d_off, st);
+    ok = ok && hipGetLastError() == hipSuccess && hipMemcpyAsync(&off, d_off, sizeof off, hipMemcpyDeviceToHost, st) == hipSuccess && hipStreamSynchronize(st) == hipSuccess;
+    (void)hipFree(d_off);
+    int g = 0;
+    while (g < kQ16Grids.n && (off >> g & 1u)) ++g;
+    if (!ok || g == kQ16Grids.n) { (void)hipGetLastError(); return copy_refused(c, CP_Q16); }
+    cp.row = (uint32_t)row; cp.slab = slice; cp.grid = kQ16Grids.g[g];
+    return build_copy(c, CP_Q16, bytes, 0, 0, 0, st, [&](void *p) {
+        launch_q16_pack(c->d_vol, c->row_pitch, c->slice_pitch, c->nx, c->ny, c->nz, cp.grid, p, row, slice, st); });
+}
+
+static bool (*const ensure_copy[CP_N])(vv_context *, hipStream_t) = {ensure_bricks, ensure_zpair, ensure_zfast, ensure_xpair, ensure_q16};
 
 static bool take_copy(vv_context *c, int k, hipStream_t st)
 {
     if (!(c->build_in_render ? ensure_copy[k](c, st) : c->copies[k].valid)) return false;
     c->copies[k].last_used = c->frame_no;
     return true;
+}
+
+static bool q16_policy(const vv_context *c)
+{
+    if (c->vtype != VV_VOXEL_F32 || c->knobs.q16 == 0) return false;
+    return c->knobs.q16 > 0 || c->vol_bytes > (1ull << 30);
 }
 
 extern "C" {
@@ -422,17 +454,19 @@
 {
     if (!c) return fail(nullptr, VV_ERR_INVALID, "vv_prepare_layouts: NULL context");
     if (!c->d_vol) return fail(c, VV_ERR_NO_VOLUME, "vv_prepare_layouts: no volume loaded");
-    if (which & ~(VV_LAYOUT_BRICKED | VV_LAYOUT_ZPAIR | VV_LAYOUT_ZFAST | VV_LAYOUT_POLICY)) return fail(c, VV_ERR_INVALID, "vv_prepare_layouts: unknown layout bit");
+    if (which & ~(VV_LAYOUT_BRICKED | VV_LAYOUT_ZPAIR | VV_LAYOUT_ZFAST | VV_LAYOUT_Q16 | VV_LAYOUT_POLICY)) return fail(c, VV_ERR_INVALID, "vv_prepare_layouts: unknown layout bit");
     HIPCHK(c, hipSetDevice(c->device));
     hipStream_t st = pick_stream(c, stream);
     const bool pair_ok = c->vtype == VV_VOXEL_U8 || c->vol_bytes <= (512ull << 20);
     if (which & VV_LAYOUT_POLICY) {
         if ((size_t)c->nx * c->ny * c->nz >= (1ull << 21)) which |= VV_LAYOUT_BRICKED | VV_LAYOUT_ZFAST;
         if (pair_ok) which |= VV_LAYOUT_ZPAIR;
+        if (q16_policy(c)) which |= VV_LAYOUT_Q16;
     }
     int built = 0;
     if (which & VV_LAYOUT_BRICKED) c->copies[CP_BRICKS].failed = false;
     if (which & VV_LAYOUT_ZFAST) c->copies[CP_ZFAST].failed = c->copies[CP_XPAIR].failed = false;
+    if (which & VV_LAYOUT_Q16) c->copies[CP_Q16].failed = false;
     auto prepare = [&](int k) {
         if (!ensure_copy[k](c, st)) return false;
         c->copies[k].last_used = ++c->frame_no;
@@ -443,6 +477,7 @@
         built |= VV_LAYOUT_ZFAST;
         if (pair_ok) prepare(CP_XPAIR);
     }
+    if ((which & VV_LAYOUT_Q16) && prepare(CP_Q16)) built |= VV_LAYOUT_Q16;
     if ((which & VV_LAYOUT_ZPAIR) && prepare(CP_ZPAIR)) built |= VV_LAYOUT_ZPAIR;
     return built;
 }
@@ -466,10 +501,21 @@
 {
     if (!c || !out) return VV_ERR_INVALID;
     out[0] = c->d_vol ? c->alloc_bytes : 0;
-    for (int k = 0; k < CP_N; ++k) out[1 + k] = copy_bytes(c, k);
+    for (int k = 0; k < CP_STATE_N; ++k) out[1 + k] = copy_bytes(c, k);
     out[5] = c->d_vol ? layout_budget(c) : c->layout_budget_bytes;
     out[6] = c->builds_in_render;
     out[7] = c->build_in_render ? 1 : 0;
+    return VV_OK;
+}
+
+int vv_debug_voxel_storage(const vv_context *c, unsigned long long out[4])
+{
+    if (!c || !out) return VV_ERR_INVALID;
+    const layout_copy &cp = c->copies[CP_Q16];
+    out[0] = (unsigned long long)c->last_storage;
+    out[1] = cp.valid ? cp.grid.D : 0;
+    out[2] = copy_bytes(c, CP_Q16);
+    out[3] = cp.valid ? 1 : (cp.failed ? 2 : 0);
     return VV_OK;
 }
 
@@ -709,7 +755,7 @@
 
 }
 
-static bool choose_launch(vv_context *c, MarchArgs &A, const camera_params *cam, const vv_ray_source *rays, const shading_params *shading,
+static bool choose_launch(vv_context *c, MarchArgs &A, FrameKind kind, const camera_params *cam, const vv_ray_source *rays, const shading_params *shading,
                           bool have_basis, float density, int H, hipStream_t st)
 {
     FrameParams &P = A.P;
@@ -780,14 +826,23 @@
                      (c->vtype == VV_VOXEL_U8 || c->vol_bytes <= (512ull << 20));
     if (K.zpair >= 0) use_zpair = K.zpair != 0 && !use_bricks;
     if (use_zfast) use_zpair = false;
+    const bool want_q16 = kind == FRAME_COMPOSITE && !shading->phongShading && !use_zfast && !use_bricks && q16_policy(c) && (K.q16 > 0 || density > 3.5f);
+    if (want_q16 && K.q16 > 0) use_zpair = false;
     if (use_zpair) use_zpair = take_copy(c, CP_ZPAIR, st);
     const bool use_xpair = use_zfast && !shading->phongShading && K.zpair != 0 && (c->vtype == VV_VOXEL_U8 || c->vol_bytes <= (512ull << 20)) &&
                            take_copy(c, CP_XPAIR, st);
+    const bool use_q16 = want_q16 && !use_zpair && take_copy(c, CP_Q16, st);
     const int valid_after = copies_valid();
     if (valid_after > valid_before) c->builds_in_render += valid_after - valid_before;
     A.build = use_xpair ? MB_XPAIR : use_zfast ? MB_ZFAST : use_bricks ? (beyond_caches ? MB_BRICKED : MB_BRICKED_CACHED) : use_zpair ? MB_ZPAIR :
               (view_of(c, MB_LINEAR).big || (shading->phongShading && beyond_caches)) ? MB_LINEAR_BIG : MB_LINEAR;
     A.V = view_of(c, A.build);
+    if (use_q16) {
+        const layout_copy &q = c->copies[CP_Q16];
+        A.V_type = VV_VOXEL_Q16; A.V.data = q.ptr; A.V.row_bytes = q.row; A.V.slice_bytes = (uint32_t)q.slab; A.V.q_hi = q.grid.hi; A.V.q_lo = q.grid.lo;
+    }
+    if (use_q16 && !k_reserve && A.lds_reserve == 76000) A.lds_reserve = 49000;
+    c->last_storage = use_q16 ? 1 : 0;
     A.lds_reserve_phong = c->vol_bytes > (8ull << 30) ? 40000 : ((beyond_caches && density > 3.5f && !use_bricks) ? 30000 : 13000);
     if (K.lds_reserve_phong >= 0 && K.lds_reserve_phong <= 146 * 1024) A.lds_reserve_phong = K.lds_reserve_phong;
     c->last_density = density;
@@ -1118,7 +1173,7 @@
     hipStream_t st = F.st;
     if ((rc = frame_params(c, F, slice, cam, rays, opts)) != VV_OK) return rc;
     if ((rc = view_knowledge(c, F, cam, rays, stream)) != VV_OK) return rc;
-    F.beyond_caches = choose_launch(c, A, cam, rays, shading, F.have_basis, F.density, H, st);
+    F.beyond_caches = choose_launch(c, A, kind, cam, rays, shading, F.have_basis, F.density, H, st);
     F.density = c->last_density;
     A.gray = c->tf_gray; A.phong = shading->phongShading;
     tiles_under_rect(c, F, rays);
diff --git a/volume-viz_amd/csrc/vv_aux.hip b/volume-viz_amd/csrc/vv_aux.hip
--- a/volume-viz_amd/csrc/vv_aux.hip
+++ b/volume-viz_amd/csrc/vv_aux.hip
@@ -637,6 +637,53 @@
     hipLaunchKernelGGL(repitch_kernel, dim3((unsigned)blocks), dim3(256), 0, s, (const uint4 *)dense, (char *)pitched, row16, ny, row_pitch, slice_pitch, total);
 }
 
+__device__ __forceinline__ bool on_grid16(float v, Q16Grid g, uint32_t &q)
+{
+    q = (uint32_t)rintf(v * (float)g.D);
+    return q <= g.D && __float_as_uint(dequant16((float)q, g.hi, g.lo)) == __float_as_uint(v);
+}
+__global__ __launch_bounds__(256) void q16_detect_kernel(const char *__restrict__ in, size_t row_pitch, size_t slice_pitch, uint32_t nx, uint32_t ny, uint32_t n_rows,
+                                                         Q16Grids G, uint32_t *__restrict__ off_grid)
+{
+    uint32_t bad = 0;
+    for (uint32_t r = blockIdx.x; r < n_rows; r += gridDim.x) {
+        const float *row = (const float *)(in + (size_t)(r / ny) * slice_pitch + (size_t)(r % ny) * row_pitch);
+        for (uint32_t x = threadIdx.x; x < nx; x += blockDim.x) {
+            const float v = row[x];
+            uint32_t q;
+            for (int g = 0; g < G.n; ++g) if (!(bad >> g & 1u)) bad |= on_grid16(v, G.g[g], q) ? 0u : 1u << g;
+        }
+    }
+    uint32_t block_bad = 0;
+    for (int g = 0; g < G.n; ++g) if (__syncthreads_or((int)(bad >> g & 1u))) block_bad |= 1u << g;
+    if (threadIdx.x == 0 && block_bad) atomicOr(off_grid, block_bad);
+}
+__global__ __launch_bounds__(256) void q16_pack_kernel(const char *__restrict__ in, size_t row_pitch, size_t slice_pitch, uint32_t nx, uint32_t ny, uint32_t n_rows,
+                                                       Q16Grid g, char *__restrict__ out, size_t q_row, size_t q_slice)
+{
+    for (uint32_t r = blockIdx.x; r < n_rows; r += gridDim.x) {
+        const size_t z = r / ny, y = r % ny;
+        const float *row = (const float *)(in + z * slice_pitch + y * row_pitch);
+        uint16_t *dst = (uint16_t *)(out + z * q_slice + y * q_row);
+        for (uint32_t x = threadIdx.x; x < nx; x += blockDim.x) {
+            uint32_t q;
+            (void)on_grid16(row[x], g, q);
+            dst[x] = (uint16_t)min(q, 65535u);
+        }
+    }
+}
+static unsigned q16_blocks(size_t n_rows) { return (unsigned)(n_rows > 256 * 64 ? 256 * 64 : n_rows); }
+void launch_q16_detect(const void *vol, size_t row_pitch, size_t slice_pitch, int nx, int ny, int nz, const Q16Grids &G, uint32_t *off_grid, hipStream_t s)
+{
+    const size_t n_rows = (size_t)ny * nz;
+    hipLaunchKernelGGL(q16_detect_kernel, dim3(q16_blocks(n_rows)), dim3(256), 0, s, (const char *)vol, row_pitch, slice_pitch, (uint32_t)nx, (uint32_t)ny, (uint32_t)n_rows, G, off_grid);
+}
+void launch_q16_pack(const void *vol, size_t row_pitch, size_t slice_pitch, int nx, int ny, int nz, const Q16Grid &g, void *out, size_t q_row, size_t q_slice, hipStream_t s)
+{
+    const size_t n_rows = (size_t)ny * nz;
+    hipLaunchKernelGGL(q16_pack_kernel, dim3(q16_blocks(n_rows)), dim3(256), 0, s, (const char *)vol, row_pitch, slice_pitch, (uint32_t)nx, (uint32_t)ny, (uint32_t)n_rows, g, (char *)out, q_row, q_slice);
+}
+
 size_t zpair_copy_bytes(int vtype, int nx, int ny, int nz, uint32_t *row_bytes, uint32_t *slab_bytes)
 {
     const size_t rec = vtype == VV_VOXEL_F32 ? 8 : 2;
diff --git a/volume-viz_amd/csrc/vv_device.h b/volume-viz_amd/csrc/vv_device.h
--- a/volume-viz_amd/csrc/vv_device.h
+++ b/volume-viz_amd/csrc/vv_device.h
@@ -22,8 +22,13 @@
     uint32_t slice_bytes;
     int big;
     const void *bricks;
-    uint32_t b_sy;
-    uint32_t b_sz64;
+    union {
+        struct {
+            uint32_t b_sy;
+            uint32_t b_sz64;
+        };
+        struct { float q_hi, q_lo; };
+    };
     const void *zpair;
     uint32_t zp_row_bytes;
     uint32_t zp_slab_bytes;
@@ -68,6 +73,7 @@
     }
 }
 template <> struct BrickGeom<VV_VOXEL_U8>  { static constexpr uint32_t xlog2 = 2, bx = 4, halo = 1, row = 8, zlog2 = 2, bz = 4, rows = 16, brick = 128; };
+enum { VV_VOXEL_Q16 = 2 };
 enum { LAYOUT_LINEAR = 0, LAYOUT_LINEAR_BIG = 1, LAYOUT_BRICKED = 2, LAYOUT_ZPAIR = 3, LAYOUT_ZFAST = 4 };
 
 struct FrameParams {
@@ -254,6 +260,15 @@
 template <int VOXEL> struct Corners;
 template <> struct Corners<VV_VOXEL_F32> { float2u a, b, c, d; float wx, wy, wz; };
 template <> struct Corners<VV_VOXEL_U8>  { uint32_t a0, a1, b0, b1, c0, c1, d0, d1, sh; float wx, wy, wz; };
+template <> struct Corners<VV_VOXEL_Q16> { uint32_t a, b, c, d, a1, b1, c1, d1, sh; float wx, wy, wz, hi, lo; };
+typedef uint32_t __attribute__((ext_vector_type(2), aligned(4))) uint2q;
+typedef uint32_t __attribute__((aligned(2))) uint32_a2;
+
+__device__ __forceinline__ float dequant16(float b, float hi, float lo)
+{
+#pragma clang fp contract(off)
+    return __builtin_fmaf(b, hi, b * lo);
+}
 
 template <int VOXEL>
 __device__ __forceinline__ void load_rows(const char *b00, uint32_t row_bytes, uint32_t slice_bytes, uint32_t ix,
@@ -266,6 +281,10 @@
         const uint32_t off = ix * 4u + yz;
         C.a = *(const float2u *)(b00 + off); C.b = *(const float2u *)(b10 + off);
         C.c = *(const float2u *)(b01 + off); C.d = *(const float2u *)(b11 + off);
+    } else if constexpr (VOXEL == VV_VOXEL_Q16) {
+        const uint32_t off = ix * 2u + yz;
+        const uint2q ra = *(const uint2q *)(b00 + off), rb = *(const uint2q *)(b10 + off), rc = *(const uint2q *)(b01 + off), rd = *(const uint2q *)(b11 + off);
+        C.a = ra.x; C.a1 = ra.y; C.b = rb.x; C.b1 = rb.y; C.c = rc.x; C.c1 = rc.y; C.d = rd.x; C.d1 = rd.y;
     } else {
         const uint32_t off = (ix & ~3u) + yz;
         C.sh = ix & 3u;
@@ -283,13 +302,15 @@
     C.wx = axis_coord<TEX8>(px, (float)V.nx, (float)(V.nx - 1), ix);
     C.wy = axis_coord<TEX8>(py, (float)V.ny, (float)(V.ny - 1), iy);
     C.wz = axis_coord<TEX8>(pz, (float)V.nz, (float)(V.nz - 1), iz);
+    if constexpr (VOXEL == VV_VOXEL_Q16) { C.hi = V.q_hi; C.lo = V.q_lo; }
+    if constexpr (VOXEL == VV_VOXEL_Q16) { C.sh = (ix & 1u) << 1; ix &= ~1u; }
     if constexpr (LAYOUT == LAYOUT_LINEAR) {
         load_rows<VOXEL>((const char *)V.data, V.row_bytes, V.slice_bytes, ix,
                          __umul24(iy, V.row_bytes) + __umul24(iz, V.slice_bytes), C);
     } else if constexpr (LAYOUT == LAYOUT_LINEAR_BIG) {
-        const uint32_t vsz = VOXEL == VV_VOXEL_F32 ? 4u : 1u;
+        const uint32_t vsz = VOXEL == VV_VOXEL_F32 ? 4u : (VOXEL == VV_VOXEL_Q16 ? 2u : 1u);
         const char *zb = (const char *)V.data + (uint64_t)iz * V.slice_bytes + (__umul24(iy, V.row_bytes) + ix * vsz);
-        if constexpr (VOXEL == VV_VOXEL_F32) load_rows<VOXEL>(zb, V.row_bytes, V.slice_bytes, 0u, 0u, C);
+        if constexpr (VOXEL != VV_VOXEL_U8) load_rows<VOXEL>(zb, V.row_bytes, V.slice_bytes, 0u, 0u, C);
         else {
             const char *zr = (const char *)V.data + (uint64_t)iz * V.slice_bytes;
             load_rows<VOXEL>(zr, V.row_bytes, V.slice_bytes, ix, __umul24(iy, V.row_bytes), C);
@@ -367,7 +388,6 @@
 }
 
 struct CornersZ8 { float wx; uint32_t r0; float wy; uint32_t r1; float wz; };
-typedef uint32_t __attribute__((aligned(2))) uint32_a2;
 
 template <bool TEX8>
 __device__ __forceinline__ void fetch_corners_zpair(const VolumeView &V, float px, float py, float pz, CornersZ8 &C)
@@ -420,6 +440,13 @@
     float c000, c100, c010, c110, c001, c101, c011, c111;
     if constexpr (VOXEL == VV_VOXEL_F32) {
         c000 = C.a.x; c100 = C.a.y; c010 = C.b.x; c110 = C.b.y; c001 = C.c.x; c101 = C.c.y; c011 = C.d.x; c111 = C.d.y;
+    } else if constexpr (VOXEL == VV_VOXEL_Q16) {
+        const uint32_t a = __builtin_amdgcn_alignbyte(C.a1, C.a, C.sh), b = __builtin_amdgcn_alignbyte(C.b1, C.b, C.sh);
+        const uint32_t c = __builtin_amdgcn_alignbyte(C.c1, C.c, C.sh), d = __builtin_amdgcn_alignbyte(C.d1, C.d, C.sh);
+        c000 = dequant16((float)(a & 0xffffu), C.hi, C.lo); c100 = dequant16((float)(a >> 16), C.hi, C.lo);
+        c010 = dequant16((float)(b & 0xffffu), C.hi, C.lo); c110 = dequant16((float)(b >> 16), C.hi, C.lo);
+        c001 = dequant16((float)(c & 0xffffu), C.hi, C.lo); c101 = dequant16((float)(c >> 16), C.hi, C.lo);
+        c011 = dequant16((float)(d & 0xffffu), C.hi, C.lo); c111 = dequant16((float)(d >> 16), C.hi, C.lo);
     } else {
         const uint32_t a = __builtin_amdgcn_alignbyte(C.a1, C.a0, C.sh), b = __builtin_amdgcn_alignbyte(C.b1, C.b0, C.sh);
         const uint32_t c = __builtin_amdgcn_alignbyte(C.c1, C.c0, C.sh), d = __builtin_amdgcn_alignbyte(C.d1, C.d0, C.sh);
@@ -461,7 +488,7 @@
 template <int VOXEL>
 __device__ __forceinline__ uint32_t index_of(float L)
 {
-    float s = (VOXEL == VV_VOXEL_F32) ? L * 255.0f : L;
+    float s = (VOXEL != VV_VOXEL_U8) ? L * 255.0f : L;
     return min((uint32_t)s, 255u);
 }
 template <int VOXEL, class CT>
diff --git a/volume-viz_amd/csrc/vv_kernels.h b/volume-viz_amd/csrc/vv_kernels.h
--- a/volume-viz_amd/csrc/vv_kernels.h
+++ b/volume-viz_amd/csrc/vv_kernels.h
@@ -76,6 +76,11 @@
 void launch_build_zpair(int vtype, const void *linear, size_t row_pitch, size_t slice_pitch, void *zpair, int nx, int ny, int nz, hipStream_t s);
 void launch_repitch(const void *dense, void *pitched, size_t row_bytes , size_t ny, size_t nz,
                     size_t row_pitch, size_t slice_pitch, hipStream_t s);
+struct Q16Grid { uint32_t D; float hi, lo; };
+struct Q16Grids { int n; Q16Grid g[4]; };
+constexpr Q16Grids kQ16Grids = {2, {{65535u, 0x1.0001p-16f, 0x1.0001p-48f}, {4095u, 0x1.001002p-12f, -0x1.ffdffep-37f}}};
+void launch_q16_detect(const void *vol, size_t row_pitch, size_t slice_pitch, int nx, int ny, int nz, const Q16Grids &G, uint32_t *off_grid, hipStream_t s);
+void launch_q16_pack(const void *vol, size_t row_pitch, size_t slice_pitch, int nx, int ny, int nz, const Q16Grid &g, void *out, size_t q_row, size_t q_slice, hipStream_t s);
 size_t brick_copy_bytes(int vtype, int nx, int ny, int nz, uint32_t *sy, uint32_t *sz64);
 void launch_build_bricks(int vtype, const void *linear, size_t row_pitch, size_t slice_pitch, void *bricks, int nx, int ny, int nz, hipStream_t s);
 struct SliceArgs {
diff --git a/volume-viz_amd/csrc/vv_layout.h b/volume-viz_amd/csrc/vv_layout.h
--- a/volume-viz_amd/csrc/vv_layout.h
+++ b/volume-viz_amd/csrc/vv_layout.h
@@ -70,9 +70,11 @@
     mark_line_range(I, off, bytes); mark_line_range(I, off + V.zp_row_bytes, bytes);
 #else
     if constexpr (kLayout == LAYOUT_LINEAR || kLayout == LAYOUT_LINEAR_BIG) {
-        const uint64_t o = (uint64_t)iz * V.slice_bytes + (uint64_t)iy * V.row_bytes + (F ? ix * 4u : (ix & ~3u));
-        mark_line_range(I, o, 8); mark_line_range(I, o + V.row_bytes, 8);
-        mark_line_range(I, o + V.slice_bytes, 8); mark_line_range(I, o + V.slice_bytes + V.row_bytes, 8);
+        constexpr bool Q = VOXEL == VV_VOXEL_Q16;
+        constexpr uint32_t bytes = 8u;
+        const uint64_t o = (uint64_t)iz * V.slice_bytes + (uint64_t)iy * V.row_bytes + (F ? ix * 4u : (Q ? (ix & ~1u) * 2u : (ix & ~3u)));
+        mark_line_range(I, o, bytes); mark_line_range(I, o + V.row_bytes, bytes);
+        mark_line_range(I, o + V.slice_bytes, bytes); mark_line_range(I, o + V.slice_bytes + V.row_bytes, bytes);
     } else if constexpr (kLayout == LAYOUT_ZFAST) {
         const uint64_t o = (uint64_t)ix * V.zf_slice_bytes + (uint64_t)iy * V.zf_row_bytes + (F ? iz * 4u : (iz & ~3u));
         mark_line_range(I, o, 8); mark_line_range(I, o + V.zf_row_bytes, 8);
diff --git a/volume-viz_amd/csrc/vv_raymarch.hip b/volume-viz_amd/csrc/vv_raymarch.hip
--- a/volume-viz_amd/csrc/vv_raymarch.hip
+++ b/volume-viz_amd/csrc/vv_raymarch.hip
@@ -1,3 +1,5 @@
+#include <cstdio>
+#include <cstdlib>
 #include "vv_device.h"
 #include "vv_kernels.h"
 
@@ -545,19 +547,28 @@
 }
 
 template <int SLICE, int VOXEL, bool TEX8>
+static void dispatch_march(const MarchArgs &a, hipStream_t s)
+{
+    const bool gray = a.gray && SLICE != SLICE_PLANE;
+    if (gray) { if (a.instr) launch_march<SLICE, VOXEL, TEX8, true, true>(a, s); else launch_march<SLICE, VOXEL, TEX8, true, false>(a, s); }
+    else      { if (a.instr) launch_march<SLICE, VOXEL, TEX8, false, true>(a, s); else launch_march<SLICE, VOXEL, TEX8, false, false>(a, s); }
+}
+template <int SLICE, int VOXEL, bool TEX8>
 static void dispatch3(const MarchArgs &a, hipStream_t s)
 {
     if (a.phong) {
         if (a.instr) launch_phong<SLICE, VOXEL, TEX8, true>(a, s); else launch_phong<SLICE, VOXEL, TEX8, false>(a, s);
         return;
     }
-    const bool gray = a.gray && SLICE != SLICE_PLANE;
-    if (gray) { if (a.instr) launch_march<SLICE, VOXEL, TEX8, true, true>(a, s); else launch_march<SLICE, VOXEL, TEX8, true, false>(a, s); }
-    else      { if (a.instr) launch_march<SLICE, VOXEL, TEX8, false, true>(a, s); else launch_march<SLICE, VOXEL, TEX8, false, false>(a, s); }
+    dispatch_march<SLICE, VOXEL, TEX8>(a, s);
 }
 template <int SLICE>
 static void dispatch2(const MarchArgs &a, hipStream_t s)
 {
+#if defined(VV_BUILD_LINEAR) || defined(VV_BIG_VOLUME)
+    if (a.V_type == VV_VOXEL_Q16 && !a.phong) { if (a.tex8) dispatch_march<SLICE, VV_VOXEL_Q16, true>(a, s); else dispatch_march<SLICE, VV_VOXEL_Q16, false>(a, s); return; }
+#endif
+    if (a.V_type == VV_VOXEL_Q16) { fprintf(stderr, "volviz: the quantised storage has no kernel in this build\n"); abort(); }
     if (a.V_type == VV_VOXEL_F32) { if (a.tex8) dispatch3<SLICE, VV_VOXEL_F32, true>(a, s); else dispatch3<SLICE, VV_VOXEL_F32, false>(a, s); }
     else                          { if (a.tex8) dispatch3<SLICE, VV_VOXEL_U8,  true>(a, s); else dispatch3<SLICE, VV_VOXEL_U8,  false>(a, s); }
 }
diff --git a/volume-viz_amd/host/device_math_check.hip b/volume-viz_amd/host/device_math_check.hip
--- a/volume-viz_amd/host/device_math_check.hip
+++ b/volume-viz_amd/host/device_math_check.hip
@@ -8,6 +8,7 @@
 #include <vector>
 #include "../csrc/vv_device.h"
 #include "../csrc/vv_gate.h"
+#include "../csrc/vv_kernels.h"
 
 using namespace vv;
 
@@ -265,8 +266,25 @@
     tally(R, bad);
 }
 
-static const char *kNames[] = {"div", "sqrt", "axis", "bounds", "convert", "chunks"};
-constexpr int kSweeps = 6;
+static unsigned long long dequant_count() { unsigned long long n = 0; for (int g = 0; g < kQ16Grids.n; ++g) n += kQ16Grids.g[g].D + 1ull; return n; }
+template <int TWIN>
+__global__ __launch_bounds__(256) void dequant_kernel(Q16Grids G, unsigned long long total, Record *R)
+{
+    unsigned long long bad = 0;
+    for (unsigned long long idx = thread_index(); idx < total; idx += (unsigned long long)gridDim.x * blockDim.x) {
+        int g = 0;
+        unsigned long long q = idx;
+        while (q > G.g[g].D) { q -= G.g[g].D + 1ull; ++g; }
+        const float b = (float)(uint32_t)q;
+        const float got = TWIN ? b * G.g[g].hi : dequant16(b, G.g[g].hi, G.g[g].lo);
+        const float want = (float)(wide(b) / (double)G.g[g].D);
+        if (__float_as_uint(got) != __float_as_uint(want)) { ++bad; note(R, G.g[g].D, (uint32_t)q, __float_as_uint(got), __float_as_uint(want)); }
+    }
+    tally(R, bad);
+}
+
+static const char *kNames[] = {"div", "sqrt", "axis", "bounds", "convert", "chunks", "dequant"};
+constexpr int kSweeps = 7, kListed = 6;
 
 struct Result { unsigned long long visited = 0; Record rec = {}; float seconds = 0.f; };
 
@@ -376,6 +394,16 @@
     return out;
 }
 
+template <int TWIN> static Result run_dequant()
+{
+    const unsigned long long n = dequant_count();
+    Record *R = new_record(); Result out; Timer t;
+    dequant_kernel<TWIN><<<blocks_for(n), 256>>>(kQ16Grids, n, R);
+    HIP_OK(hipGetLastError());
+    out.seconds = t.stop(); out.rec = take(R); out.visited = n;
+    return out;
+}
+
 static std::string first_json(const Record &r)
 {
     std::string s = "[";
@@ -392,16 +420,16 @@
 {
     bool self_test = false, want[kSweeps] = {}, any = false;
     for (int a = 1; a < argc; ++a) {
-        if (!strcmp(argv[a], "--list")) { for (const char *n : kNames) printf("%s\n", n); return 0; }
+        if (!strcmp(argv[a], "--list")) { for (int k = 0; k < kListed; ++k) printf("%s\n", kNames[k]); return 0; }
         if (!strcmp(argv[a], "--self-test")) { self_test = true; continue; }
         int k = 0;
         while (k < kSweeps && strcmp(argv[a], kNames[k])) ++k;
-        if (k == kSweeps) { fprintf(stderr, "usage: device_math_check [--list] [--self-test] [div|sqrt|axis|bounds|convert|chunks ...]\n"); return 2; }
+        if (k == kSweeps) { fprintf(stderr, "usage: device_math_check [--list] [--self-test] [div|sqrt|axis|bounds|convert|chunks|dequant ...]\n"); return 2; }
         want[k] = any = true;
     }
     int rc = 0;
     for (int k = 0; k < kSweeps; ++k) {
-        if (any && !want[k]) continue;
+        if (any ? !want[k] : k >= kListed) continue;
         Result r, inv, twin, twin2;
         std::string extra;
         char buf[256];
@@ -439,7 +467,13 @@
             extra = ", \"disagreeing_patterns\": " + set + "]";
             break; }
         case 4: r = run_convert<0>(); if (self_test) twin = run_convert<1>(); clean = r.rec.mismatches == 0; break;
-        default: r = run_chunks<0>(); if (self_test) twin = run_chunks<1>(); clean = r.rec.mismatches == 0; break;
+        case 5: r = run_chunks<0>(); if (self_test) twin = run_chunks<1>(); clean = r.rec.mismatches == 0; break;
+        default: {
+            r = run_dequant<0>(); if (self_test) twin = run_dequant<1>();
+            extra = ", \"grids\": [";
+            for (int g = 0; g < kQ16Grids.n; ++g) { snprintf(buf, sizeof buf, "%s%u", g ? ", " : "", kQ16Grids.g[g].D); extra += buf; }
+            extra += "]";
+            clean = r.rec.mismatches == 0; break; }
         }
         if (!clean) rc = 1;
         std::string st;
diff --git a/volume-viz_amd/python/volviz_amd/__init__.py b/volume-viz_amd/python/volviz_amd/__init__.py
--- a/volume-viz_amd/python/volviz_amd/__init__.py
+++ b/volume-viz_amd/python/volviz_amd/__init__.py
@@ -16,6 +16,7 @@
 HORIZONTAL, SAGITTAL, CORONAL, FREE_FORM = 0, 1, 2, 4
 VOXEL_U8, VOXEL_F32 = 0, 1
 LAYOUT_BRICKED, LAYOUT_ZPAIR, LAYOUT_ZFAST, LAYOUT_POLICY = 1, 2, 4, 256
+LAYOUT_Q16 = 16
 FILTER_TEX8, FILTER_EXACT = 0, 1
 ERT_REFERENCE, ERT_TRUE = 0, 1
 SLAB_MAX, SLAB_MIN, SLAB_MEAN = 0, 1, 2
@@ -98,10 +99,10 @@
     "vv_load_volume_stream_begin", "vv_load_volume_stream_slices", "vv_load_volume_stream_end", "vv_load_volume_t3d",
     "vv_load_volume_stream_slices_async", "vv_load_volume_stream_wait_source", "vv_dataset_preset", "vv_debug_last_launch", "vv_set_frame_timing", "vv_debug_screen_rect",
     "vv_render_mip", "vv_classify_indices", "vv_render_iso", "vv_slice_slab", "vv_slice_advanced_slab",
-    "vv_volume_histogram", "vv_histogram_indices", "vv_render_projection",
+    "vv_volume_histogram", "vv_histogram_indices", "vv_render_projection", "vv_debug_voxel_storage",
 ]
 _NEWER_EXPORTS = ("vv_render_mip", "vv_classify_indices", "vv_render_iso", "vv_slice_slab", "vv_slice_advanced_slab",
-                  "vv_volume_histogram", "vv_histogram_indices", "vv_render_projection")
+                  "vv_volume_histogram", "vv_histogram_indices", "vv_render_projection", "vv_debug_voxel_storage")
 
 _lib = None
 _libs = {}
@@ -184,9 +185,11 @@
     lib.vv_device_bytes.argtypes = [vp, vp]
     lib.vv_set_layout_policy.argtypes = [vp, C.c_ulonglong, i]
     lib.vv_layout_state.argtypes = [vp, vp]
+    if hasattr(lib, "vv_debug_voxel_storage"):
+        lib.vv_debug_voxel_storage.argtypes = [vp, vp]
     lib.vv_volume_dims.argtypes = [vp, C.POINTER(i * 3), C.POINTER(i)]
     for name in EXPORTS:
-        if path is not None and name in _NEWER_EXPORTS and not hasattr(lib, name):
+        if (path is not None or "VV_LIB" in os.environ) and name in _NEWER_EXPORTS and not hasattr(lib, name):
             continue
         fn = getattr(lib, name)
         if name not in ("vv_last_error", "vv_last_frame_ms", "vv_last_sample_count"):
@@ -513,6 +516,11 @@
         k = ("linear", "bricked", "zpair", "zfast", "xpair", "budget", "builds_in_render", "build_in_render")
         return dict(zip(k, (int(v) for v in out)))
 
+    def voxel_storage(self) -> dict:
+        out = np.zeros(4, np.uint64)
+        self._chk(self.lib.vv_debug_voxel_storage(self.h, out.ctypes.data))
+        return dict(zip(("storage", "grid", "bytes", "state"), (int(v) for v in out)))
+
     def device_bytes(self):
         out = np.zeros(4, np.uint64)
         self._chk(self.lib.vv_device_bytes(self.h, out.ctypes.data))
```

Measured after the change: 275,400, median of 6. 25.8% higher.
